# avishkarsaha/learning-adaptive-neighborhoods-for-gnns

Measured on AMD Instinct MI355X. Metric: DGG adj-build+SpMM fwd/bwd edges/sec & achieved HBM GB/s, N=100k d=128 k=32, higher is better.
Workload: dtype f32; 1 GPU; synthetic all-pairs DGG N=100000 d=128 h=64 k~32.3 K=64, u-v-dist/x/k_times_edge_prob, Gumbel(0,0.3) perturbation, + normalize + GCNConv(128,64), fwd+bwd; nodes=100000, feat=128, latent=64, parallelism=row-shard x1, rows_per_rank=100000, hipgraph=True, noise=ranked

## Files before the change

### include/dgg_hip.h

```cpp
#ifndef DGG_HIP_H
#define DGG_HIP_H
#include <stddef.h>
#include <stdint.h>

#ifdef __cplusplus
extern "C" {
#endif

#define DGG_OK 0
#define DGG_ERR_ARG 1
#define DGG_ERR_UNSUPPORTED 2
#define DGG_ERR_HIP 3

#define DGG_NOISE_NONE 0
#define DGG_NOISE_EXPLICIT 1
#define DGG_NOISE_HASH 2
#define DGG_NOISE_HASH_SYM 3
#define DGG_NOISE_RANKED 4
#define DGG_NOISE_RANKED_SYM 5

#define DGG_ACT_NONE 0
#define DGG_ACT_LEAKY 1
#define DGG_ACT_RELU 2

#define DGG_MODE_K_TIMES_EDGE_PROB 0
#define DGG_MODE_K_ONLY 1

const char *dgg_last_error(void);
int dgg_abi_version(void);

int dgg_linear_fwd(const float *x, int64_t N, int d, const float *W, const float *b, int out, int w_layout, int act,
                   float *y, void *stream);
size_t dgg_linear_bwd_ws_floats(int64_t N, int d, int out);
int dgg_linear_bwd(const float *x, int64_t N, int d, const float *W, int out, int w_layout, int act, const float *y,
                   const float *dy, float *dx, float *dW, float *db, float *ws, void *stream);
int dgg_linear_pack_weights(int nseg, const float *const *W, const float *const *b, const int *seg_out, const int *seg_layout, int d,
                            float *Wcat, float *bcat, void *stream);
int dgg_linear_fwd_multi(const float *x, int64_t N, int d, const float *Wcat, const float *bcat, int nseg, const int *seg_out,
                         const int *seg_act, float *const *y, void *stream);
size_t dgg_gemm_tn_multi_ws_floats(int64_t N, int M1_total, int M2);
int dgg_gemm_tn_multi(int nseg, const float *const *A, const int *M1, const float *const *Y, const int *act, const float *B,
                      int64_t N, int M2, float *const *C, const int *c_layout, float *const *colsum, float *ws, void *stream);
int dgg_gemm_tn_pairs(int npair, const float *const *A, const int *M1, const float *const *B, const int *M2, int64_t N, float *const *C,
                      float *const *colsum, float *ws, void *stream);
size_t dgg_gemm_tn_ws_floats(int64_t N, int M1, int M2);
int dgg_gemm_tn_acc(const float *A, const float *B, int64_t N, int M1, int M2, float *C, int c_layout, float *colsum,
                    float *ws, void *stream);

int dgg_degree_stats(const float *deg, int64_t N, float *mu_sd, void *ws, void *stream);
size_t dgg_degree_stats_ws_bytes(void);
int dgg_knet_x_fwd(const float *xk, int64_t N, int h, const float *deg, const float *mu_sd, const float *W1,
                   const float *b1, int h2, const float *Wmu, const float *bmu, int h4, const float *Wp, const float *bp,
                   float *k, float *z_save, float *u_save, float *feat_save, void *stream);
int dgg_knet_x_fwd_mfma(const float *xk, int64_t N, int h, const float *deg, const float *mu_sd, const float *W1, const float *b1,
                        const float *Wmu, const float *bmu, const float *Wp, const float *bp, float *k, float *u_save, void *stream);
size_t dgg_knet_x_bwd_ws_bytes(int64_t N, int h);
int dgg_knet_x_bwd_reg(const float *xk, int64_t N, int h, const float *deg, const float *mu_sd, const float *W1, const float *b1,
                       const float *Wmu, const float *bmu, const float *Wp, const float *u, const float *dk, float *dxk, float *gW1,
                       float *gb1, float *gWmu, float *gbmu, float *gWp, float *gbp, int out_act, void *ws, void *stream);
int dgg_knet_x_bwd_nodes(int64_t N, int h, const float *mu_sd, const float *W1, int h2, const float *Wmu, int h4,
                         const float *Wp, const float *bmu, const float *z, const float *u, const float *dk, float *dkp,
                         float *dm, float *dpre1, float *dxk, float *m_out, void *stream);
int dgg_knet_deg_fwd(const float *deg, int64_t N, const float *mu_sd, float dmean, float dstd, float eps, const float *Wd,
                     const float *bd, const float *Wmu, const float *bmu, int h4, const float *Wp, const float *bp, float *k,
                     float *u_save, void *stream);
int dgg_knet_feat(const float *xk, const float *deg, const float *mu_sd, int64_t N, int h, float *feat, void *stream);
int dgg_knet_out_fwd(const float *kp, const float *mu_sd, int64_t N, float *k, float *u, void *stream);
int dgg_knet_out_bwd(const float *u, const float *dk, const float *mu_sd, int64_t N, float *dkp, void *stream);
int dgg_knet_deg_bwd_sums(const float *deg, int64_t N, const float *mu_sd, float dmean, float dstd, float eps, const float *u,
                          const float *dk, float *S, void *stream);
int dgg_knet_input_deg_fwd(const float *deg, int64_t N, float dmean, float dstd, const float *Wd, const float *bd,
                           const float *Wmu, const float *bmu, int h4, const float *Wp, const float *bp, float *k,
                           void *stream);

int dgg_allpairs_topk(const float *xp, int64_t N, int h, int64_t row0, int64_t row1, float t, int noise_mode,
                      const float *G, int64_t ldG, uint32_t s0, uint32_t s1, int K, int32_t *idx, float *val,
                      const float *k_limit, int algo, void *workspace, size_t ws_bytes, void *stream);
int dgg_allpairs_ranked_probe(const float *xp, int64_t N, int h, int64_t row0, int64_t row1, float t, uint32_t s0, uint32_t s1,
                              const float *k_limit, int stride, int max_blocks, unsigned long long *probe, const float *lpub, void *stream);
int dgg_allpairs_topk_ranked_softk(const float *xp, int64_t N, int h, int64_t row0, int64_t row1, float t, uint32_t s0, uint32_t s1,
                                   const float *k, int mode, int32_t *idx, float *val, float *w, float *rs, void *stream);
int dgg_allpairs_topk_ranked_softk_dseed(const float *xp, int64_t N, int h, int64_t row0, int64_t row1, float t, const uint32_t *seed_dev,
                                         const float *k, int mode, int32_t *idx, float *val, float *w, float *rs, void *stream);
int dgg_allpairs_topk_ranked_softk_lp(const float *xp, int64_t N, int h, int64_t row0, int64_t row1, float t, uint32_t s0, uint32_t s1,
                                      const uint32_t *seed_dev, const float *lpub, const float *k, int mode, int32_t *idx, float *val, float *w,
                                      float *rs, void *stream);
int dgg_chunk_layout(const float *k, int64_t rows, int maxm, int64_t ccap, int32_t *cptr, int32_t *cnode, int32_t *meta, int32_t *sticky,
                     void *stream);
int dgg_allpairs_topk_ranked_wide(const float *xp, int64_t N, int h, int64_t row0, int64_t row1, float t, uint32_t s0, uint32_t s1,
                                  const uint32_t *seed_dev, const float *k, int mode, int maxm, const int32_t *cptr, int64_t ccap, int32_t *idx,
                                  float *val, float *w, float *rs, const float *lpub, void *stream);
size_t dgg_allpairs_anywide_ws_bytes(int64_t ccap, int64_t rows, int64_t N, int h);
int dgg_allpairs_topk_anywide(const float *xp, int64_t N, int h, int64_t row0, int64_t row1, float t, int noise_mode, uint32_t s0, uint32_t s1,
                              const uint32_t *seed_dev, const float *k, int mode, int maxm, int min_m, const int32_t *cptr, int64_t ccap,
                              int32_t *idx, float *val, float *w, float *rs, const float *lpub, void *workspace, size_t ws_bytes, void *stream);
size_t dgg_allpairs_rowmin_ws_bytes(int64_t rows, int64_t N, int h);
int dgg_allpairs_rowmin_bound(const float *xp, int64_t N, int h, int64_t row0, int64_t row1, float t, float *lpub, void *workspace, size_t ws_bytes,
                              void *stream);
size_t dgg_allpairs_workspace_bytes(int64_t N, int h, int noise_mode, int K);
size_t dgg_allpairs_sweep_ctl_offset_bytes(int64_t rows, int64_t N, int h);
size_t dgg_allpairs_rsym_ctl_offset_bytes(int64_t rows, int64_t N);
int dgg_literal_hard_fwd(const float *xp, int64_t N, int h, const int64_t *rowptr, const int32_t *col, float t, int noise_mode,
                         const float *G, int64_t ldG, uint32_t s0, uint32_t s1, const int32_t *idx, const float *w, int K, float threshold,
                         int32_t *hidx, float *hval, int32_t *hsrc, void *stream);
int dgg_literal_hard_bwd(const int32_t *hsrc, const float *g, int64_t N, int K, float *dw, void *stream);
int dgg_edgelist_topk(const float *xp, int64_t N, int h, const int64_t *rowptr, const int32_t *col, float t,
                      int noise_mode, const float *G, int64_t ldG, uint32_t s0, uint32_t s1, int K, int32_t *idx,
                      float *val, void *stream);
int dgg_edgelist_topk_softk(const float *xp, int64_t N, int h, const int64_t *rowptr, const int32_t *col, float t,
                            int noise_mode, const float *G, int64_t ldG, uint32_t s0, uint32_t s1, int K, const float *k,
                            int mode, int32_t *idx, float *val, float *w, float *rs, int32_t *overflow, void *stream);
int dgg_edgelist_topk_softk_rows(const float *xp, int64_t N, int h, int64_t row0, int64_t row1, const int64_t *rowptr, const int32_t *col,
                                 float t, int noise_mode, const float *G, int64_t ldG, uint32_t s0, uint32_t s1, int K, const float *k,
                                 int mode, int32_t *idx, float *val, float *w, float *rs, int32_t *overflow, void *stream);

int dgg_edge_mlp_fwd(const float *AB, const float *xp, int64_t N, int h, int hw, const int32_t *erow, const int32_t *col,
                     int64_t E, const float *deg, const float *ex_in, int ex_mode, float t_ex, const float *wdu,
                     const float *wdv, const float *wex, const float *b1, const float *w2, const float *b2, int act,
                     float *p_edge, float *ex_out, void *stream);
int dgg_edgelist_topk_p(const float *p_edge, int64_t N, const int64_t *rowptr, const int32_t *col, int noise_mode,
                        const float *G, int64_t ldG, uint32_t s0, uint32_t s1, int K, int32_t *idx, float *val, int32_t *eid,
                        void *stream);
int dgg_edgelist_topk_p_rows(const float *p_edge, int64_t N, int64_t row0, int64_t row1, const int64_t *rowptr, const int32_t *col,
                             int noise_mode, const float *G, int64_t ldG, uint32_t s0, uint32_t s1, int K, int32_t *idx, float *val,
                             int32_t *eid, void *stream);
// ... 193 lines not shown
```

### learning-adaptive-neighborhoods-for-gnns_amd/_lib.py

```python
import ctypes as C
import os

_HERE = os.path.dirname(os.path.abspath(__file__))
SO_PATH = os.environ.get("DGG_HIP_SO", os.path.join(_HERE, "libdgg_hip.so"))

_vp, _i64, _i32, _u32, _f32, _sz = C.c_void_p, C.c_int64, C.c_int, C.c_uint32, C.c_float, C.c_size_t

PROTOTYPES = {
    "dgg_linear_fwd": [_vp, _i64, _i32, _vp, _vp, _i32, _i32, _i32, _vp, _vp],
    "dgg_linear_bwd": [_vp, _i64, _i32, _vp, _i32, _i32, _i32, _vp, _vp, _vp, _vp, _vp, _vp, _vp],
    "dgg_gemm_tn_acc": [_vp, _vp, _i64, _i32, _i32, _vp, _i32, _vp, _vp, _vp],
    "dgg_gemm_tn_ws_floats": [_i64, _i32, _i32],
    "dgg_linear_pack_weights": [_i32, _vp, _vp, _vp, _vp, _i32, _vp, _vp, _vp],
    "dgg_linear_fwd_multi": [_vp, _i64, _i32, _vp, _vp, _i32, _vp, _vp, _vp, _vp],
    "dgg_gemm_tn_multi": [_i32, _vp, _vp, _vp, _vp, _vp, _i64, _i32, _vp, _vp, _vp, _vp, _vp],
    "dgg_gemm_tn_multi_ws_floats": [_i64, _i32, _i32],
    "dgg_gemm_tn_pairs": [_i32, _vp, _vp, _vp, _vp, _i64, _vp, _vp, _vp, _vp],
    "dgg_linear_bwd_ws_floats": [_i64, _i32, _i32],
    "dgg_degree_stats": [_vp, _i64, _vp, _vp, _vp],
    "dgg_degree_stats_ws_bytes": [],
    "dgg_knet_x_fwd": [_vp, _i64, _i32, _vp, _vp, _vp, _vp, _i32, _vp, _vp, _i32, _vp, _vp, _vp, _vp, _vp, _vp, _vp],
    "dgg_knet_x_fwd_mfma": [_vp, _i64, _i32] + [_vp] * 10 + [_vp],
    "dgg_knet_x_bwd_reg": [_vp, _i64, _i32] + [_vp] * 16 + [_i32, _vp, _vp],
    "dgg_knet_x_bwd_ws_bytes": [_i64, _i32],
    "dgg_knet_x_bwd_nodes": [_i64, _i32, _vp, _vp, _i32, _vp, _i32, _vp, _vp, _vp, _vp, _vp, _vp, _vp, _vp, _vp, _vp, _vp],
    "dgg_knet_input_deg_fwd": [_vp, _i64, _f32, _f32, _vp, _vp, _vp, _vp, _i32, _vp, _vp, _vp, _vp],
    "dgg_knet_feat": [_vp, _vp, _vp, _i64, _i32, _vp, _vp],
    "dgg_knet_out_fwd": [_vp, _vp, _i64, _vp, _vp, _vp],
    "dgg_knet_out_bwd": [_vp, _vp, _vp, _i64, _vp, _vp],
    "dgg_knet_deg_fwd": [_vp, _i64, _vp, _f32, _f32, _f32, _vp, _vp, _vp, _vp, _i32, _vp, _vp, _vp, _vp, _vp],
    "dgg_knet_deg_bwd_sums": [_vp, _i64, _vp, _f32, _f32, _f32, _vp, _vp, _vp, _vp],
    "dgg_allpairs_topk": [_vp, _i64, _i32, _i64, _i64, _f32, _i32, _vp, _i64, _u32, _u32, _i32, _vp, _vp, _vp, _i32, _vp, _sz, _vp],
    "dgg_allpairs_workspace_bytes": [_i64, _i32, _i32, _i32],
    "dgg_allpairs_sweep_ctl_offset_bytes": [_i64, _i64, _i32],
    "dgg_allpairs_rsym_ctl_offset_bytes": [_i64, _i64],
    "dgg_allpairs_ranked_probe": [_vp, _i64, _i32, _i64, _i64, _f32, _u32, _u32, _vp, _i32, _i32, _vp, _vp, _vp],
    "dgg_allpairs_topk_ranked_softk_lp": [_vp, _i64, _i32, _i64, _i64, _f32, _u32, _u32, _vp, _vp, _vp, _i32, _vp, _vp, _vp, _vp, _vp],
    "dgg_allpairs_topk_ranked_softk": [_vp, _i64, _i32, _i64, _i64, _f32, _u32, _u32, _vp, _i32, _vp, _vp, _vp, _vp, _vp],
    "dgg_literal_hard_fwd": [_vp, _i64, _i32, _vp, _vp, _f32, _i32, _vp, _i64, _u32, _u32, _vp, _vp, _i32, _f32, _vp, _vp, _vp, _vp],
    "dgg_literal_hard_bwd": [_vp, _vp, _i64, _i32, _vp, _vp],
    "dgg_allpairs_topk_ranked_softk_dseed": [_vp, _i64, _i32, _i64, _i64, _f32, _vp, _vp, _i32, _vp, _vp, _vp, _vp, _vp],
    "dgg_chunk_layout": [_vp, _i64, _i32, _i64, _vp, _vp, _vp, _vp, _vp],
    "dgg_allpairs_anywide_ws_bytes": [_i64, _i64, _i64, _i32],
    "dgg_allpairs_rowmin_ws_bytes": [_i64, _i64, _i32],
    "dgg_allpairs_rowmin_bound": [_vp, _i64, _i32, _i64, _i64, _f32, _vp, _vp, _sz, _vp],
    "dgg_allpairs_topk_anywide": [_vp, _i64, _i32, _i64, _i64, _f32, _i32, _u32, _u32, _vp, _vp, _i32, _i32, _i32, _vp, _i64, _vp, _vp, _vp, _vp, _vp,
                                  _vp, _sz, _vp],
    "dgg_allpairs_topk_ranked_wide": [_vp, _i64, _i32, _i64, _i64, _f32, _u32, _u32, _vp, _vp, _i32, _i32, _vp, _i64, _vp, _vp, _vp, _vp, _vp, _vp],
    "dgg_partp_build_chunked": [_vp, _vp, _vp, _vp, _i64, _vp, _i64, _vp, _vp, _vp, _i32, _vp],
    "dgg_ell_spmm_act_fwd_chunked": [_vp, _vp, _vp, _i64, _vp, _i32, _i32, _vp, _vp],
    "dgg_ell_conv_bwd_partp_chunked": [_vp, _vp, _i64, _i32, _vp, _i64, _vp, _vp, _vp, _vp, _vp, _vp, _vp],
    "dgg_softk_edge_bwd_partp_chunked": [_vp, _i64, _vp, _i64, _i32, _vp, _vp, _vp, _vp, _vp, _vp, _vp, _vp, _i64, _f32, _i32, _i32, _i32, _vp,
                                         _i64, _vp, _vp, _vp, _i32, _i32, _vp],
    "dgg_partp_gather_rec": [_vp, _i64, _i64, _vp, _vp, _vp],
    "dgg_edgelist_topk": [_vp, _i64, _i32, _vp, _vp, _f32, _i32, _vp, _i64, _u32, _u32, _i32, _vp, _vp, _vp],
    "dgg_edgelist_topk_softk": [_vp, _i64, _i32, _vp, _vp, _f32, _i32, _vp, _i64, _u32, _u32, _i32, _vp, _i32, _vp, _vp, _vp, _vp, _vp, _vp],
    "dgg_edgelist_topk_softk_rows": [_vp, _i64, _i32, _i64, _i64, _vp, _vp, _f32, _i32, _vp, _i64, _u32, _u32, _i32, _vp, _i32, _vp, _vp, _vp, _vp, _vp, _vp],
    "dgg_edge_mlp_fwd": [_vp, _vp, _i64, _i32, _i32, _vp, _vp, _i64, _vp, _vp, _i32, _f32, _vp, _vp, _vp, _vp, _vp, _vp, _i32, _vp, _vp, _vp],
    "dgg_edgelist_topk_p": [_vp, _i64, _vp, _vp, _i32, _vp, _i64, _u32, _u32, _i32, _vp, _vp, _vp, _vp],
    "dgg_edgelist_topk_p_rows": [_vp, _i64, _i64, _i64, _vp, _vp, _i32, _vp, _i64, _u32, _u32, _i32, _vp, _vp, _vp, _vp],
    "dgg_edge_mlp_bwd": [_vp, _i64, _i32, _vp, _vp, _vp, _vp, _vp, _i32, _vp, _vp, _vp, _vp, _vp, _vp, _vp, _vp, _i32, _i32, _vp, _vp, _vp, _vp],
    "dgg_edge_mlp_bwd_rows": [_vp, _i64, _i32, _i64, _i64, _vp, _vp, _vp, _vp, _vp, _i32, _vp, _vp, _vp, _vp, _vp, _vp, _vp, _vp, _i32, _i32, _vp, _vp, _vp, _vp],
    "dgg_edge_mlp_bwd_partp": [_vp, _i64, _i32, _vp, _vp, _vp, _vp, _vp, _i32, _vp, _vp, _vp, _vp, _vp, _vp, _vp, _vp, _i32, _i32, _vp, _i64, _vp, _i64, _vp, _vp, _vp, _vp],
    "dgg_edge_mlp_bwd_partp_rows": [_vp, _i64, _i32, _i64, _i64, _vp, _vp, _vp, _vp, _vp, _i32, _vp, _vp, _vp, _vp, _vp, _vp, _vp, _vp, _i32, _i32, _vp, _vp, _i64, _vp, _vp, _vp, _vp],
    "dgg_csr_softk_fwd": [_vp, _vp, _vp, _i64, _vp, _i32, _vp, _i64, _u32, _u32, _i32, _vp, _vp, _vp, _vp],
    "dgg_csr_softk_bwd": [_vp, _vp, _vp, _i64, _vp, _vp, _i32, _i32, _vp, _vp, _vp, _vp],
    "dgg_csr_softk_fwd_rows": [_vp, _vp, _vp, _i64, _i64, _i64, _vp, _i32, _u32, _u32, _i32, _vp, _vp, _vp, _vp],
    "dgg_csr_rank_ramp_fwd": [_vp, _vp, _vp, _i64, _vp, _vp, _vp, _vp, _vp, _vp, _vp],
    "dgg_csr_rank_ramp_bwd": [_vp, _vp, _i64, _vp, _vp, _vp, _vp, _vp, _vp, _vp, _vp, _vp],
    "dgg_csr_noisy_sigmoid_fwd": [_vp, _vp, _i64, _vp, _vp],
    "dgg_csr_noisy_sigmoid_bwd": [_vp, _vp, _i64, _vp, _vp],
    "dgg_csr_rank_cut_fwd": [_vp, _vp, _vp, _i64, _i32, _vp, _vp, _vp],
    "dgg_csr_rank_cut_bwd": [_vp, _vp, _i64, _i32, _vp, _vp],
    "dgg_dense_rows_fwd": [_vp, _i32, _i64, _i32, _vp, _f32, _i32, _vp, _i32, _f32, _f32, _i32, _vp, _vp, _vp, _vp],
    "dgg_dense_rows_bwd": [_vp, _i32, _i64, _i32, _vp, _f32, _i32, _vp, _f32, _f32, _vp, _vp, _vp, _vp, _vp, _vp, _vp],
    "dgg_dense_pairs_dx": [_vp, _i32, _i64, _i32, _vp, _vp, _vp],
    "dgg_feat_softmax_fwd": [_vp, _i64, _i32, _vp, _vp],
    "dgg_feat_softmax_bwd": [_vp, _vp, _i64, _i32, _vp, _vp],
    "dgg_csr_uvdist_fwd": [_vp, _vp, _vp, _i64, _i32, _f32, _vp, _vp],
    "dgg_csr_uvdist_bwd": [_vp, _vp, _vp, _i64, _i32, _f32, _vp, _vp, _vp, _vp],
    "dgg_csr_uvdist_fwd_rows": [_vp, _vp, _vp, _i64, _i64, _i64, _i32, _f32, _vp, _vp],
    "dgg_csr_uvdist_bwd_rows": [_vp, _vp, _vp, _i64, _i64, _i64, _i32, _f32, _vp, _vp, _vp, _vp],
    "dgg_csr_perturb_fwd": [_vp, _vp, _vp, _i64, _i64, _i32, _vp, _i64, _u32, _u32, _vp, _vp],
    "dgg_csr_perturb_bwd": [_vp, _vp, _vp, _i64, _vp, _vp],
    "dgg_csr_row_sum": [_vp, _vp, _i64, _vp, _vp],
    "dgg_csr_normalize_fwd": [_vp, _vp, _vp, _vp, _i64, _vp, _vp],
    "dgg_csr_norm_bwd": [_vp, _vp, _vp, _vp, _vp, _i64, _vp, _vp, _vp],
    "dgg_csr_normalize_fwd_rows": [_vp, _vp, _vp, _vp, _i64, _i64, _i64, _vp, _vp],
    "dgg_csr_norm_bwd_acc_rows": [_vp, _vp, _vp, _vp, _vp, _i64, _i64, _i64, _vp, _vp],
    "dgg_csr_norm_bwd_apply_rows": [_vp, _vp, _vp, _vp, _vp, _i64, _i64, _i64, _vp, _vp],
    "dgg_csr_spmm_fwd": [_vp, _vp, _vp, _vp, _i64, _i32, _vp, _vp],
    "dgg_csr_bg_softmax_fwd": [_vp, _vp, _i64, _vp, _vp, _vp],
    "dgg_csr_bg_softmax_bwd": [_vp, _vp, _vp, _i64, _vp, _vp, _vp, _vp],
    "dgg_masked_dense_sum": [_vp, _i64, _i32, _f32, _u32, _u32, _i32, _vp, _vp],
    "dgg_pair_keep": [_vp, _vp, _i64, _f32, _u32, _u32, _vp, _vp],
    "dgg_csr_spmm_bwd": [_vp, _vp, _vp, _vp, _vp, _i64, _i32, _vp, _vp, _vp],
    "dgg_select_scores": [_vp, _i64, _i64, _i32, _vp, _vp, _vp],
    "dgg_softk_fwd": [_vp, _vp, _vp, _i64, _i32, _i32, _vp, _vp, _vp],
# ... 89 lines not shown
```

### learning-adaptive-neighborhoods-for-gnns_amd/csrc/dgg_linear.hip

```cpp
#include "dgg_common.h"
#include "dgg_api_internal.h"

#include <cstdlib>

typedef float f32x16 __attribute__((ext_vector_type(16)));

namespace {

constexpr int LIN_BK(int nacc) { return 32; }

__device__ __forceinline__ float act_apply(float v, int act) {
    if (act == 1) return v > 0.0f ? v : __fmul_rn(0.01f, v);
    if (act == 2) return v > 0.0f ? v : 0.0f;
    return v;
}

struct LinSegs {
    float *y[8];
    int ld[8];
    int act[8];
};

template <int NACC, int WAVES, bool MULTI = false>
__global__ __launch_bounds__(64 * WAVES, NACC <= 2 ? 4 : 2) void linear_fwd_mfma(const float *__restrict__ x, int64_t N, int d,
                                                       const float *__restrict__ W, const float *__restrict__ b,
                                                       int out, int w_layout, int act, float *__restrict__ y, LinSegs segs) {
    constexpr int BN = 32 * NACC, BM = 32 * WAVES, NT = 64 * WAVES;
    constexpr int BK = LIN_BK(NACC), LDP = BK + 1, F4R = BK / 4;
    __shared__ float xs[BM * LDP];
    __shared__ float ws[BN * LDP];
    const int tid = threadIdx.x, lane = tid & 63, wave = dgg::wave_id();
    const int64_t m0 = (int64_t)blockIdx.x * BM;
    const int n0 = blockIdx.y * BN;
    f32x16 acc[NACC];
#pragma unroll
    for (int a = 0; a < NACC; a++)
#pragma unroll
        for (int r = 0; r < 16; r++) acc[a][r] = 0.0f;
    const int li = lane & 31, hh = lane >> 5;
    const bool vec4 = (d % 4 == 0) && ((reinterpret_cast<uintptr_t>(x) & 15) == 0);
    constexpr int XQ = BM * BK / 4 / NT;
    constexpr int WQ = BN * BK / NT;
    float4 xr[XQ];
    float wr[WQ];
    unsigned xm[XQ];
    auto load_block = [&](int k0) {
        if (vec4) {
#pragma unroll
            for (int q = 0; q < XQ; q++) {
                const int e = tid + q * NT, r = e / F4R, c4 = (e % F4R) * 4;
                const int64_t gi = m0 + r;
                const bool ok = gi < N && k0 + c4 < d;
                const int64_t gic = gi < N ? gi : N - 1;
                const int kc = k0 + c4 < d ? k0 + c4 : d - 4;
                xr[q] = *reinterpret_cast<const float4 *>(x + gic * d + kc);
                xm[q] = ok ? 15u : 0u;
            }
        } else {
#pragma unroll
            for (int q = 0; q < XQ; q++) {
                const int e = tid + q * NT, r = e / F4R, c4 = (e % F4R) * 4;
                const int64_t gi = m0 + r;
                const int64_t gic = gi < N ? gi : N - 1;
                float t[4];
                unsigned bits = 0;
#pragma unroll
                for (int u = 0; u < 4; u++) {
                    const int kk = k0 + c4 + u;
                    t[u] = x[gic * d + (kk < d ? kk : d - 1)];
                    bits |= (gi < N && kk < d) ? (1u << u) : 0u;
                }
                xr[q] = make_float4(t[0], t[1], t[2], t[3]);
                xm[q] = bits;
            }
        }
#pragma unroll
        for (int q = 0; q < WQ; q++) {
            const int e = tid + q * NT;
            const int j = w_layout == 0 ? e / BK : e % BN, c = w_layout == 0 ? e % BK : e / BN;
            const int gj = n0 + j, gk = k0 + c;
            const int gjc = gj < out ? gj : out - 1, gkc = gk < d ? gk : d - 1;
            wr[q] = W[w_layout == 0 ? (int64_t)gjc * d + gkc : (int64_t)gkc * out + gjc];
        }
    };
    float bj[NACC];
#pragma unroll
    for (int a = 0; a < NACC; a++) {
        const int gj = n0 + a * 32 + li;
        bj[a] = b ? b[gj < out ? gj : out - 1] : 0.0f;
    }
    load_block(0);
    for (int k0 = 0; k0 < d; k0 += BK) {
        __syncthreads();
#pragma unroll
        for (int q = 0; q < XQ; q++) {
            const int e = tid + q * NT, r = e / F4R, c4 = (e % F4R) * 4;
            float *dst = xs + r * LDP + c4;
            dst[0] = (xm[q] & 1u) ? xr[q].x : 0.0f; dst[1] = (xm[q] & 2u) ? xr[q].y : 0.0f;
            dst[2] = (xm[q] & 4u) ? xr[q].z : 0.0f; dst[3] = (xm[q] & 8u) ? xr[q].w : 0.0f;
        }
#pragma unroll
        for (int q = 0; q < WQ; q++) {
            const int e = tid + q * NT;
            const int j = w_layout == 0 ? e / BK : e % BN, c = w_layout == 0 ? e % BK : e / BN;
            ws[j * LDP + c] = (n0 + j < out && k0 + c < d) ? wr[q] : 0.0f;
        }
        __syncthreads();
        if (k0 + BK < d) load_block(k0 + BK);
        const float *xa = xs + (wave * 32 + li) * LDP + hh;
#pragma unroll
        for (int s = 0; s < BK / 2; s++) {
            float av = xa[2 * s];
#pragma unroll
            for (int a = 0; a < NACC; a++) {
                float bv = ws[(a * 32 + li) * LDP + 2 * s + hh];
                acc[a] = __builtin_amdgcn_mfma_f32_32x32x2f32(av, bv, acc[a], 0, 0, 0);
            }
        }
    }
    const bool hasb = b != nullptr;
    auto finish_act = [&](float v, float bias, int actv) {
        const float vb = __fadd_rn(v, bias);
        v = hasb ? vb : v;
        const float lk = v > 0.0f ? v : __fmul_rn(0.01f, v), rl = v > 0.0f ? v : 0.0f;
        return actv == 1 ? lk : (actv == 2 ? rl : v);
    };
    auto finish = [&](float v, float bias) { return finish_act(v, bias, act); };
    if constexpr (MULTI) {
        const bool full = m0 + BM <= N;
#pragma unroll
        for (int a = 0; a < NACC; a++) {
            const int cb = n0 / 32 + a;
            float *yb = segs.y[cb] + (m0 + wave * 32 + 4 * hh) * (int64_t)segs.ld[cb] + li;
            const int av = segs.act[cb];
#pragma unroll
            for (int r = 0; r < 16; r++) {
                const int row = (r & 3) + 8 * (r >> 2);
                if (full || m0 + wave * 32 + 4 * hh + row < N) yb[(int64_t)row * segs.ld[cb]] = finish_act(acc[a][r], bj[a], av);
            }
        }
        return;
    }
    if (m0 + BM <= N && n0 + BN <= out) {
        float *yb = y + (m0 + wave * 32 + 4 * hh) * out + n0 + li;
#pragma unroll
        for (int a = 0; a < NACC; a++)
#pragma unroll
            for (int r = 0; r < 16; r++) yb[(int64_t)((r & 3) + 8 * (r >> 2)) * out + a * 32] = finish(acc[a][r], bj[a]);
        return;
    }
#pragma unroll
    for (int a = 0; a < NACC; a++) {
        const int gj = n0 + a * 32 + li;
#pragma unroll
        for (int r = 0; r < 16; r++) {
            const int row = (r & 3) + 8 * (r >> 2) + 4 * hh;
            const int64_t gi = m0 + wave * 32 + row;
            const float v = finish(acc[a][r], bj[a]);
            if (gi < N && gj < out) y[gi * out + gj] = v;
        }
    }
}

template <int D, int NACC>
__global__ __launch_bounds__(256, 1) void linear_fwd_reg(const float *__restrict__ x, int64_t N, const float *__restrict__ W,
                                                         const float *__restrict__ b, LinSegs segs, int64_t nrb) {
    constexpr int S = D / 2, XR = D / 2;
    __shared__ float wsf[S * NACC * 64];
    const int tid = threadIdx.x, lane = tid & 63, wave = dgg::wave_id(), li = lane & 31, hh = lane >> 5;
    const int64_t nw = (int64_t)gridDim.x * 4, slot = (int64_t)blockIdx.x * 4 + wave;
    const int64_t nrbf = N / 32;
    const int64_t nmain = nrbf - nrbf % nw, nfull = nmain / nw;
    const int64_t R = nrb - nmain, nunits = nfull + (slot < R * NACC ? (R * NACC - slot + nw - 1) / nw : 0);
    auto unit_rb = [&](int64_t t) {
        if (t < nfull) return slot + t * nw;
        const int64_t u = slot + (t - nfull) * nw;
        return nmain + u % (R > 0 ? R : 1);
    };
    float xc[XR], xn[XR];
    auto load_rows = [&](int64_t rb, float(&dst)[XR]) {
        int64_t row = rb * 32 + li;
        row = row < N ? row : N - 1;
        const float4 *p = reinterpret_cast<const float4 *>(x + row * D + hh * (D / 2));
#pragma unroll
        for (int q = 0; q < XR / 4; q++) {
            const float4 v = p[q];
            dst[4 * q] = v.x; dst[4 * q + 1] = v.y; dst[4 * q + 2] = v.z; dst[4 * q + 3] = v.w;
        }
    };
    if (nunits > 0) load_rows(unit_rb(0), xc);
#pragma unroll
    for (int it = 0; it < NACC * 32 * (D / 4) / 256; it++) {
        const int e = tid + it * 256;
        const int j = e % (NACC * 32), q = e / (NACC * 32);
        const float4 v = *reinterpret_cast<const float4 *>(W + (int64_t)j * D + 4 * q);
        float *dst = wsf + ((2 * q) * NACC + (j >> 5)) * 64 + (j & 31);
        dst[0] = v.x; dst[32] = v.y; dst[NACC * 64] = v.z; dst[NACC * 64 + 32] = v.w;
    }
    const bool hasb = b != nullptr;
    float bj[NACC];
    int actv[NACC];
#pragma unroll
    for (int a = 0; a < NACC; a++) {
        bj[a] = hasb ? b[a * 32 + li] : 0.0f;
        actv[a] = segs.act[a];
    }
    __syncthreads();
    auto swap_rows = [&]() {
#pragma unroll
        for (int t = 0; t < XR / 2; t++) {
            const auto r = __builtin_amdgcn_permlane32_swap(__float_as_uint(xc[2 * t]), __float_as_uint(xc[2 * t + 1]), false, false);
            xc[2 * t] = __uint_as_float(r[0]);
            xc[2 * t + 1] = __uint_as_float(r[1]);
        }
    };
    auto act4 = [&](float4 v, int av) {
        if (av == 1) {
            v.x = fmaxf(v.x, __fmul_rn(0.01f, v.x)); v.y = fmaxf(v.y, __fmul_rn(0.01f, v.y));
            v.z = fmaxf(v.z, __fmul_rn(0.01f, v.z)); v.w = fmaxf(v.w, __fmul_rn(0.01f, v.w));
        } else if (av == 2) {
            v.x = fmaxf(v.x, 0.0f); v.y = fmaxf(v.y, 0.0f); v.z = fmaxf(v.z, 0.0f); v.w = fmaxf(v.w, 0.0f);
        }
        return v;
    };
    auto store_block = [&](const f32x16 &acc, int a, int64_t rb) {
        const int64_t n = rb * 32 + li;
        if (n >= N) return;
        const int av = actv[a];
        float *yb = segs.y[a] + n * (int64_t)segs.ld[a] + 4 * hh;
#pragma unroll
        for (int q = 0; q < 4; q++)
            *reinterpret_cast<float4 *>(yb + 8 * q) = act4(make_float4(acc[4 * q], acc[4 * q + 1], acc[4 * q + 2], acc[4 * q + 3]), av);
    };
    const float one_or_zero = hh == 0 ? 1.0f : 0.0f;
    auto main_block = [&](int64_t rb) {
        f32x16 acc[NACC];
#pragma unroll
        for (int a = 0; a < NACC; a++)
#pragma unroll
            for (int r = 0; r < 16; r++) acc[a][r] = 0.0f;
        constexpr int PD = NACC >= 4 ? 1 : (NACC >= 2 ? 2 : 4), RING = PD + 1;
        float bw[RING][NACC];
#pragma unroll
        for (int s = 0; s < PD; s++)
#pragma unroll
            for (int a = 0; a < NACC; a++) bw[s][a] = wsf[(s * NACC + a) * 64 + lane];
#pragma unroll
        for (int s = 0; s < S; s++) {
            if (s + PD < S) {
#pragma unroll
                for (int a = 0; a < NACC; a++) bw[(s + PD) % RING][a] = wsf[((s + PD) * NACC + a) * 64 + lane];
            }
            __builtin_amdgcn_sched_barrier(0);
            const float av = s < S / 2 ? xc[2 * s] : xc[2 * (s - S / 2) + 1];
#pragma unroll
            for (int a = 0; a < NACC; a++) acc[a] = __builtin_amdgcn_mfma_f32_32x32x2f32(bw[s % RING][a], av, acc[a], 0, 0, 0);
            __builtin_amdgcn_sched_barrier(0);
        }
        if (hasb) {
#pragma unroll
            for (int a = 0; a < NACC; a++) acc[a] = __builtin_amdgcn_mfma_f32_32x32x2f32(bj[a] * one_or_zero, one_or_zero, acc[a], 0, 0, 0);
        }
#pragma unroll
        for (int a = 0; a < NACC; a++) store_block(acc[a], a, rb);
    };
    int64_t t = 0;
    for (; t < nfull; t++) {
        load_rows(unit_rb(t + 1 < nunits ? t + 1 : t), xn);
        asm volatile("" ::: "memory");
        swap_rows();
        main_block(unit_rb(t));
#pragma unroll
        for (int q = 0; q < XR; q++) xc[q] = xn[q];
    }
    for (; t < nunits; t++) {
        const int64_t rb = unit_rb(t);
        load_rows(unit_rb(t + 1 < nunits ? t + 1 : t), xn);
        asm volatile("" ::: "memory");
        swap_rows();
        const int a = (int)((slot + (t - nfull) * nw) / R);
        f32x16 acc;
#pragma unroll
        for (int r = 0; r < 16; r++) acc[r] = 0.0f;
        const float *wa = wsf + a * 64 + lane;
#pragma unroll
        for (int s = 0; s < S; s++) {
            const float av = s < S / 2 ? xc[2 * s] : xc[2 * (s - S / 2) + 1];
            acc = __builtin_amdgcn_mfma_f32_32x32x2f32(wa[s * NACC * 64], av, acc, 0, 0, 0);
        }
        if (hasb) acc = __builtin_amdgcn_mfma_f32_32x32x2f32(b[a * 32 + li] * one_or_zero, one_or_zero, acc, 0, 0, 0);
        store_block(acc, a, rb);
#pragma unroll
        for (int q = 0; q < XR; q++) xc[q] = xn[q];
    }
}

__global__ void act_bwd_kernel(const float *__restrict__ y, const float *__restrict__ dy, int64_t n, int act,
                               float *__restrict__ dp) {
    int64_t i = (int64_t)blockIdx.x * blockDim.x + threadIdx.x;
    int64_t stride = (int64_t)gridDim.x * blockDim.x;
    for (; i < n; i += stride) {
        float g = dy[i], v = y[i];
        if (act == 1) g = v > 0.0f ? g : 0.01f * g;
        else if (act == 2) g = v > 0.0f ? g : 0.0f;
        dp[i] = g;
    }
}

constexpr int GT_GRID = 256, GT_PF = 8;
template <int MB, int NB, int PFK, bool ACT>
__global__ __launch_bounds__(256) void gemm_tn_persist(const float *__restrict__ A, const float *__restrict__ B, int64_t N,
                                                       int M1, int M2, int M1p, int M2p, float *__restrict__ slab,
                                                       float *__restrict__ cs_slab, const float *__restrict__ Yact, int act) {
    extern __shared__ float red[];
    const int lane = threadIdx.x & 63, wave = dgg::wave_id(), li = lane & 31, hh = lane >> 5;
    const int o0 = blockIdx.y * 32 * MB, c0 = blockIdx.z * 32 * NB;
    int64_t acol[MB], bcol[NB];
#pragma unroll
    for (int m = 0; m < MB; m++) acol[m] = o0 + m * 32 + li < M1 ? o0 + m * 32 + li : M1 - 1;
#pragma unroll
    for (int a = 0; a < NB; a++) bcol[a] = c0 + a * 32 + li < M2 ? c0 + a * 32 + li : M2 - 1;
    f32x16 acc[MB][NB];
#pragma unroll
    for (int m = 0; m < MB; m++)
#pragma unroll
        for (int a = 0; a < NB; a++)
#pragma unroll
            for (int r = 0; r < 16; r++) acc[m][a][r] = 0.0f;
    float csum[MB];
#pragma unroll
    for (int m = 0; m < MB; m++) csum[m] = 0.0f;
    constexpr int PF = PFK;
    const int64_t step = (int64_t)gridDim.x * 4 * 2 * PF;
    float av[2][PF][MB], bv[2][PF][NB], rmask[2][PF], yv[2][PF][MB];
    auto load = [&](int buf, int64_t base) {
#pragma unroll
        for (int u = 0; u < PF; u++) {
            const int64_t n = base + 2 * u + hh;
            const int64_t nc = n < N ? n : N - 1;
            rmask[buf][u] = n < N ? 1.0f : 0.0f;
#pragma unroll
            for (int m = 0; m < MB; m++) {
                av[buf][u][m] = A[nc * M1 + acol[m]];
                if (ACT) yv[buf][u][m] = Yact[nc * M1 + acol[m]];
            }
#pragma unroll
            for (int a = 0; a < NB; a++) bv[buf][u][a] = B[nc * M2 + bcol[a]];
        }
    };
    auto mma = [&](int buf) {
#pragma unroll
        for (int u = 0; u < PF; u++) {
#pragma unroll
            for (int m = 0; m < MB; m++) {
                float am = rmask[buf][u];
                if (ACT && act == 1) am = yv[buf][u][m] > 0.0f ? am : 0.01f * am;
                else if (ACT && act == 2) am = yv[buf][u][m] > 0.0f ? am : 0.0f;
                av[buf][u][m] *= am;
                csum[m] += av[buf][u][m];
#pragma unroll
                for (int a = 0; a < NB; a++)
                    acc[m][a] = __builtin_amdgcn_mfma_f32_32x32x2f32(av[buf][u][m], bv[buf][u][a], acc[m][a], 0, 0, 0);
            }
        }
    };
    int64_t base = ((int64_t)blockIdx.x * 4 + wave) * 2 * PF;
    if (base < N) load(0, base);
    while (base < N) {
        if (base + step < N) load(1, base + step);
        mma(0);
        base += step;
        if (base >= N) break;
        if (base + step < N) load(0, base + step);
// ... 263 lines not shown
                acc[m][a] = __builtin_amdgcn_mfma_f32_32x32x16_bf16(al[m], bh[a], acc[m][a], 0, 0, 0);
                acc[m][a] = __builtin_amdgcn_mfma_f32_32x32x16_bf16(ah[m], bl[a], acc[m][a], 0, 0, 0);
                acc[m][a] = __builtin_amdgcn_mfma_f32_32x32x16_bf16(ah[m], bh[a], acc[m][a], 0, 0, 0);
            }
    }
}

template <int PF, bool B3 = false, bool HASACT = true>
__global__ __launch_bounds__(256, 2) void gemm_tn_wide(TnSegs segs, const float *__restrict__ B, int64_t N, int G, int M2, int M2p, int ntile,
                                                       float *__restrict__ slab, float *__restrict__ cs_slab) {
    extern __shared__ float red[];
    const int lane = threadIdx.x & 63, wave = dgg::wave_id(), li = lane & 31, hh = lane >> 5;
    const int npair = segs.nyb / 2, nblk = npair * ntile;
    const int bid = blockIdx.x, tt = bid / (8 * nblk), rem = bid % (8 * nblk);
    const int yb = 2 * ((rem / 8) % npair), tile = (rem / 8) / npair;
    const int g = tt * 8 + (rem % 8);
    if (g >= G) return;
    const int col0 = tile * 128 + 4 * li, bcol = col0 + 4 <= M2 ? col0 : M2 - 4;
    const float *__restrict__ A = segs.A[yb];
    const float *__restrict__ Yact = segs.Y[yb];
    const int M1 = segs.ld[yb], act = Yact ? segs.act[yb] : 0, acol = segs.o0[yb] + 2 * li;
    f32x16 acc[2][4];
#pragma unroll
    for (int m = 0; m < 2; m++)
#pragma unroll
        for (int a = 0; a < 4; a++)
#pragma unroll
            for (int r = 0; r < 16; r++) acc[m][a][r] = 0.0f;
    float csum[2] = {0.0f, 0.0f};
    if constexpr (B3) {
        const int64_t base = ((int64_t)g * 4 + wave) * 16, stride = (int64_t)G * 4 * 16;
        if (HASACT && act != 0) tn_wide_stream_b3<true>(A, Yact, act, B, N, M1, acol, M2, bcol, hh, base, stride, acc, csum);
        else tn_wide_stream_b3<false>(A, Yact, act, B, N, M1, acol, M2, bcol, hh, base, stride, acc, csum);
    } else {
        const int64_t base = ((int64_t)g * 4 + wave) * 2 * PF, stride = (int64_t)G * 4 * 2 * PF;
        if (act != 0) tn_wide_stream<PF, true>(A, Yact, act, B, N, M1, acol, M2, bcol, hh, base, stride, acc, csum);
        else tn_wide_stream<PF, false>(A, Yact, act, B, N, M1, acol, M2, bcol, hh, base, stride, acc, csum);
    }
    float *cred = red + 8 * 16 * 64;
    for (int w = 1; w < 4; w++) {
        if (wave == w) {
#pragma unroll
            for (int q = 0; q < 8; q++)
#pragma unroll
                for (int r = 0; r < 16; r++) red[(q * 16 + r) * 64 + lane] = acc[q >> 2][q & 3][r];
            cred[lane] = csum[0];
            cred[64 + lane] = csum[1];
        }
        __syncthreads();
        if (wave == 0) {
#pragma unroll
            for (int q = 0; q < 8; q++)
#pragma unroll
                for (int r = 0; r < 16; r++) acc[q >> 2][q & 3][r] += red[(q * 16 + r) * 64 + lane];
            csum[0] += cred[lane];
            csum[1] += cred[64 + lane];
        }
        __syncthreads();
    }
    if (wave != 0) return;
    const int M1tp = segs.nyb * 32;
    float *sl = slab + ((int64_t)g * M1tp + yb * 32) * M2p + col0;
    if (col0 < M2p) {
#pragma unroll
        for (int m = 0; m < 2; m++)
#pragma unroll
            for (int r = 0; r < 16; r++) {
                const int go = (r & 3) + 8 * (r >> 2) + 4 * hh;
                *reinterpret_cast<float4 *>(sl + (int64_t)(2 * go + m) * M2p) = make_float4(acc[m][0][r], acc[m][1][r], acc[m][2][r], acc[m][3][r]);
            }
    }
    if (tile != 0) return;
#pragma unroll
    for (int m = 0; m < 2; m++) {
        const float t = csum[m] + __uint_as_float(dgg::xor_shfl<32>(__float_as_uint(csum[m]), lane));
        if (hh == 0) cs_slab[(int64_t)g * M1tp + yb * 32 + 2 * li + m] = t;
    }
}

struct RedSegs {
    float *C[8];
    float *colsum[8];
    int M1[8], M2[8], M1p[8], rowbase[8], c_layout[8];
};
__global__ __launch_bounds__(1024) void gemm_tn_reduce_multi(const float *__restrict__ slab, const float *__restrict__ cs_slab, int nchunks,
                                                             int M2p, int64_t chunk_stride, int64_t cs_stride, RedSegs rs) {
    __shared__ float part[16][64];
    const int sgi = blockIdx.z;
    const int M1 = rs.M1[sgi], M2 = rs.M2[sgi], M1p = rs.M1p[sgi];
    const int lane = threadIdx.x & 63, pw = threadIdx.x >> 6;
    const int e = blockIdx.x * 64 + lane;
    if (blockIdx.x * 64 >= M1p * M2p) return;
    auto total = [&](const float *base, int64_t stride, bool ok) {
        float acc[8];
#pragma unroll
        for (int j = 0; j < 8; j++) acc[j] = 0.0f;
        for (int k0 = pw; k0 < nchunks; k0 += 128) {
#pragma unroll
            for (int j = 0; j < 8; j++) {
                const int k = k0 + 16 * j;
                acc[j] += (ok && k < nchunks) ? base[(int64_t)k * stride] : 0.0f;
            }
        }
        part[pw][lane] = ((acc[0] + acc[1]) + (acc[2] + acc[3])) + ((acc[4] + acc[5]) + (acc[6] + acc[7]));
        __syncthreads();
        float v = 0.0f;
#pragma unroll
        for (int j = 0; j < 16; j++) v += part[j][lane];
        __syncthreads();
        return v;
    };
    const int o = e / M2p, c = e % M2p;
    const bool ok = e < M1p * M2p && o < M1 && c < M2;
    const float v = total(slab + (int64_t)rs.rowbase[sgi] * M2p + e, chunk_stride, ok);
    if (ok && pw == 0) {
        float *dst = rs.c_layout[sgi] == 0 ? rs.C[sgi] + (int64_t)o * M2 + c : rs.C[sgi] + (int64_t)c * M1 + o;
        *dst += v;
    }
    if (rs.colsum[sgi] && blockIdx.x * 64 < M1) {
        const bool okc = e < M1;
        const float cv = total(cs_slab + rs.rowbase[sgi] + e, cs_stride, okc);
        if (okc && pw == 0) rs.colsum[sgi][e] += cv;
    }
}

constexpr int GT_SPLIT = 32;
__global__ __launch_bounds__(256) void gemm_tn_reduce(const float *__restrict__ slab, const float *__restrict__ cs_slab,
                                                      int nchunks, int M1, int M2, int M1p, int M2p,
                                                      float *__restrict__ Cout, int c_layout, float *__restrict__ colsum,
                                                      int64_t chunk_stride, int64_t cs_stride) {
    const int e = blockIdx.x * 256 + threadIdx.x;
    const int per = (nchunks + (int)gridDim.y - 1) / (int)gridDim.y;
    const int k0 = blockIdx.y * per, k1 = k0 + per < nchunks ? k0 + per : nchunks;
    if (k0 >= k1) return;
    if (e < M1p * M2p) {
        const int o = e / M2p, c = e % M2p;
        if (o < M1 && c < M2) {
            float s = 0.0f;
            for (int k = k0; k < k1; k++) s += slab[(int64_t)k * chunk_stride + e];
            float *dst = c_layout == 0 ? Cout + (int64_t)o * M2 + c : Cout + (int64_t)c * M1 + o;
            atomicAdd(dst, s);
        }
    }
    if (colsum && cs_slab && e < M1) {
        float s = 0.0f;
        for (int k = k0; k < k1; k++) s += cs_slab[(int64_t)k * cs_stride + e];
        atomicAdd(colsum + e, s);
    }
}

template <int NACC>
void launch_linear_fwd_n(const float *x, int64_t N, int d, const float *W, const float *b, int out, int w_layout, int act, float *y,
                         hipStream_t st) {
    const unsigned gy = (unsigned)((out + 32 * NACC - 1) / (32 * NACC));
    hipLaunchKernelGGL((linear_fwd_mfma<NACC, 4>), dim3((unsigned)((N + 127) / 128), gy), dim3(256), 0, st, x, N, d, W, b, out, w_layout, act, y, LinSegs{});
}

int launch_linear_fwd(const float *x, int64_t N, int d, const float *W, const float *b, int out, int w_layout, int act,
                      float *y, hipStream_t st) {
    static const int nacc_env = [] { const char *e = getenv("DGG_LIN_NACC1"); return e ? atoi(e) : 0; }();
    const int64_t wg4 = ((N + 127) / 128) * ((out + 127) / 128);
    if (out <= 32) launch_linear_fwd_n<1>(x, N, d, W, b, out, w_layout, act, y, st);
    else if (out <= 64 || nacc_env == 2 || (nacc_env == 0 && wg4 < 256)) launch_linear_fwd_n<2>(x, N, d, W, b, out, w_layout, act, y, st);
    else launch_linear_fwd_n<4>(x, N, d, W, b, out, w_layout, act, y, st);
    return dgg_check_launch("linear_fwd");
}

template <int NACC>
void launch_linear_fwd_multi_n(const float *x, int64_t N, int d, const float *W, const float *b, int out, const LinSegs &segs, hipStream_t st) {
    hipLaunchKernelGGL((linear_fwd_mfma<NACC, 4, true>), dim3((unsigned)((N + 127) / 128), (unsigned)(out / (32 * NACC))), dim3(256), 0, st, x, N,
                       d, W, b, out, 0, 0, nullptr, segs);
}

inline void gemm_tn_shape(int M1p, int M2p, int &mb, int &nb) {
    mb = M1p / 32 >= 2 ? 2 : 1;
    nb = M2p / 32 >= 3 ? 4 : M2p / 32;
}
inline int gemm_tn_grid(int64_t N, int M1p, int M2p) {
    int mb, nb;
    gemm_tn_shape(M1p, M2p, mb, nb);
    const int64_t blocks = (int64_t)((M1p / 32 + mb - 1) / mb) * ((M2p / 32 + nb - 1) / nb);
    int64_t g = (4 * GT_GRID + blocks - 1) / blocks;
    if (g > GT_GRID) g = GT_GRID;
    const int64_t need = (N + 4 * 2 * GT_PF - 1) / (4 * 2 * GT_PF);
    if (g > need) g = need;
    int64_t cap = N * (int64_t)(M1p + M2p) / (4 * (int64_t)M1p * M2p);
    if (cap < 8) cap = 8;
    if (g > cap) g = cap;
    if (g > need) g = need;
    return (int)(g < 1 ? 1 : g);
}
size_t gemm_tn_ws_floats(int64_t N, int M1, int M2) {
    const size_t M1p = (size_t)(M1 + 31) / 32 * 32, M2p = (size_t)(M2 + 31) / 32 * 32;
    const size_t g = (size_t)gemm_tn_grid(N, (int)M1p, (int)M2p);
    return g * M1p * M2p + g * M1p;
}

template <int MB, int NB>
void launch_gemm_tn_persist(const float *A, const float *B, int64_t N, int M1, int M2, int M1p, int M2p, float *slab,
                            float *cs_slab, int g, const float *Yact, int act, hipStream_t st) {
    const unsigned gy = (unsigned)((M1p / 32 + MB - 1) / MB), gz = (unsigned)((M2p / 32 + NB - 1) / NB);
    const size_t lds = (size_t)(MB * NB * 16 * 64 + MB * 64) * sizeof(float);
    if (Yact)
        hipLaunchKernelGGL((gemm_tn_persist<MB, NB, GT_PF / 2, true>), dim3(g, gy, gz), dim3(256), lds, st, A, B, N, M1, M2, M1p, M2p, slab,
                           cs_slab, Yact, act);
    else
        hipLaunchKernelGGL((gemm_tn_persist<MB, NB, GT_PF, false>), dim3(g, gy, gz), dim3(256), lds, st, A, B, N, M1, M2, M1p, M2p, slab,
                           cs_slab, Yact, act);
}

int launch_gemm_tn(const float *A, const float *B, int64_t N, int M1, int M2, float *C, int c_layout, float *colsum,
                   float *ws, hipStream_t st, const float *Yact = nullptr, int act = 0) {
    if (!ws) return dgg_set_error(DGG_ERR_ARG, "gemm_tn: workspace is NULL (dgg_gemm_tn_ws_floats)");
    const int M1p = (M1 + 31) / 32 * 32, M2p = (M2 + 31) / 32 * 32;
    const int g = gemm_tn_grid(N, M1p, M2p);
    float *slab = ws, *cs_slab = ws + (size_t)g * M1p * M2p;
    float *csl = colsum ? cs_slab : nullptr;
    int mb, nb;
    gemm_tn_shape(M1p, M2p, mb, nb);
    if (Yact) mb = 1;
    if (mb == 2 && nb == 4) launch_gemm_tn_persist<2, 4>(A, B, N, M1, M2, M1p, M2p, slab, csl, g, Yact, act, st);
    else if (mb == 2 && nb == 2) launch_gemm_tn_persist<2, 2>(A, B, N, M1, M2, M1p, M2p, slab, csl, g, Yact, act, st);
    else if (mb == 2) launch_gemm_tn_persist<2, 1>(A, B, N, M1, M2, M1p, M2p, slab, csl, g, Yact, act, st);
    else if (nb == 4) launch_gemm_tn_persist<1, 4>(A, B, N, M1, M2, M1p, M2p, slab, csl, g, Yact, act, st);
    else if (nb == 2) launch_gemm_tn_persist<1, 2>(A, B, N, M1, M2, M1p, M2p, slab, csl, g, Yact, act, st);
    else launch_gemm_tn_persist<1, 1>(A, B, N, M1, M2, M1p, M2p, slab, csl, g, Yact, act, st);
    int split = (M1p * M2p >= 16384) ? (g + 7) / 8 : g;
    split = split < 1 ? 1 : (split > GT_SPLIT ? GT_SPLIT : split);
    hipLaunchKernelGGL(gemm_tn_reduce, dim3((unsigned)((M1p * M2p + 255) / 256), (unsigned)split), dim3(256), 0, st, slab, csl, g, M1,
                       M2, M1p, M2p, C, c_layout, colsum, (int64_t)M1p * M2p, (int64_t)M1p);
    return dgg_check_launch("gemm_tn");
}

}

extern "C" {

int dgg_linear_fwd(const float *x, int64_t N, int d, const float *W, const float *b, int out, int w_layout, int act,
                   float *y, void *stream) {
    if (N < 0 || d < 1 || out < 1) return dgg_set_error(DGG_ERR_ARG, "linear_fwd: bad shape");
    if (N == 0) return 0;
    return launch_linear_fwd(x, N, d, W, b, out, w_layout, act, y, (hipStream_t)stream);
}

struct PackSegs {
    const float *W[8];
    const float *b[8];
    int out[8], layout[8], first[8];
};
__global__ __launch_bounds__(256) void pack_weights_kernel(PackSegs sg, int nseg, int d, int total, float *__restrict__ Wcat,
                                                           float *__restrict__ bcat) {
    const int e = blockIdx.x * 256 + threadIdx.x;
    if (e >= total * (d + 1)) return;
    const int c = e / (d + 1), k = e % (d + 1);
    int s = 0;
#pragma unroll
    for (int q = 1; q < 8; q++)
        if (q < nseg && c >= sg.first[q]) s = q;
    const int lc = c - sg.first[s];
    if (k == d) { bcat[c] = sg.b[s] ? sg.b[s][lc] : 0.0f; return; }
    Wcat[(int64_t)c * d + k] = sg.layout[s] == 0 ? sg.W[s][(int64_t)lc * d + k] : sg.W[s][(int64_t)k * sg.out[s] + lc];
}

extern "C" int dgg_linear_pack_weights(int nseg, const float *const *W, const float *const *b, const int *seg_out, const int *seg_layout,
                                       int d, float *Wcat, float *bcat, void *stream) {
    if (nseg < 1 || nseg > 8 || d < 1) return dgg_set_error(DGG_ERR_ARG, "linear_pack_weights: 1..8 layers");
    PackSegs sg{};
    int total = 0;
    for (int s = 0; s < nseg; s++) {
        sg.W[s] = W[s]; sg.b[s] = b ? b[s] : nullptr; sg.out[s] = seg_out[s]; sg.layout[s] = seg_layout[s]; sg.first[s] = total;
        total += seg_out[s];
    }
    hipLaunchKernelGGL(pack_weights_kernel, dim3((unsigned)((total * (d + 1) + 255) / 256)), dim3(256), 0, (hipStream_t)stream, sg, nseg, d, total,
                       Wcat, bcat);
    return dgg_check_launch("linear_pack_weights");
}

int dgg_linear_fwd_multi(const float *x, int64_t N, int d, const float *Wcat, const float *bcat, int nseg, const int *seg_out,
                         const int *seg_act, float *const *y, void *stream) {
    if (N < 0 || d < 1 || nseg < 1 || nseg > 8) return dgg_set_error(DGG_ERR_ARG, "linear_fwd_multi: bad shape");
    LinSegs segs{};
    int cb = 0;
    for (int sgi = 0; sgi < nseg; sgi++) {
        if (seg_out[sgi] < 32 || seg_out[sgi] % 32 != 0 || cb + seg_out[sgi] / 32 > 8)
            return dgg_set_error(DGG_ERR_UNSUPPORTED, "linear_fwd_multi: layer widths must be multiples of 32 with a total of at most 256");
        for (int q = 0; q < seg_out[sgi] / 32; q++, cb++) {
            segs.y[cb] = y[sgi] + q * 32;
            segs.ld[cb] = seg_out[sgi];
            segs.act[cb] = seg_act[sgi];
        }
    }
    if (cb == 7) return dgg_set_error(DGG_ERR_UNSUPPORTED, "linear_fwd_multi: 7 column blocks (224 outputs) are not tiled");
    if (N == 0) return 0;
    const int out = cb * 32;
    hipStream_t st = (hipStream_t)stream;
    static const int forced = [] { const char *e = getenv("DGG_LINEAR_REG"); return e ? atoi(e) : -1; }();
    const bool aligned = (reinterpret_cast<uintptr_t>(x) % 16 == 0) && (reinterpret_cast<uintptr_t>(Wcat) % 16 == 0);
    if (d == 128 && aligned && cb <= 6 && (forced >= 0 ? forced != 0 : N >= 32768)) {
        const int64_t nrb = (N + 31) / 32;
        const unsigned grid = (unsigned)std::min<int64_t>(256, (nrb + 3) / 4);
        switch (cb) {
#define DGG_LIN_REG(NA) case NA: hipLaunchKernelGGL((linear_fwd_reg<128, NA>), dim3(grid), dim3(256), 0, st, x, N, Wcat, bcat, segs, nrb); break
            DGG_LIN_REG(1); DGG_LIN_REG(2); DGG_LIN_REG(3); DGG_LIN_REG(4); DGG_LIN_REG(5); DGG_LIN_REG(6);
#undef DGG_LIN_REG
        }
        return dgg_check_launch("linear_fwd_multi");
    }
    static const int nacc_env = [] { const char *e = getenv("DGG_LIN_NACC"); return e ? atoi(e) : 0; }();
    int nacc_small = 0;
    if ((N + 127) / 128 < 256 && cb > 2) nacc_small = cb % 2 == 0 ? 2 : 1;
    if (cb > 1 && ((N + 127) / 128) * ((cb + 1) / 2) < 128) nacc_small = 1;
    if (nacc_env > 0 && cb % nacc_env == 0) nacc_small = nacc_env;
    if (nacc_small > 0) {
        switch (nacc_small) {
            case 1: launch_linear_fwd_multi_n<1>(x, N, d, Wcat, bcat, out, segs, st); break;
            case 2: launch_linear_fwd_multi_n<2>(x, N, d, Wcat, bcat, out, segs, st); break;
            case 3: launch_linear_fwd_multi_n<3>(x, N, d, Wcat, bcat, out, segs, st); break;
            default: launch_linear_fwd_multi_n<4>(x, N, d, Wcat, bcat, out, segs, st); break;
        }
        return dgg_check_launch("linear_fwd_multi");
    }
    switch (cb) {
        case 1: launch_linear_fwd_multi_n<1>(x, N, d, Wcat, bcat, out, segs, st); break;
        case 2: launch_linear_fwd_multi_n<2>(x, N, d, Wcat, bcat, out, segs, st); break;
        case 3: launch_linear_fwd_multi_n<3>(x, N, d, Wcat, bcat, out, segs, st); break;
        case 4: launch_linear_fwd_multi_n<4>(x, N, d, Wcat, bcat, out, segs, st); break;
        case 5: launch_linear_fwd_multi_n<5>(x, N, d, Wcat, bcat, out, segs, st); break;
        case 6: launch_linear_fwd_multi_n<6>(x, N, d, Wcat, bcat, out, segs, st); break;
        default: launch_linear_fwd_multi_n<4>(x, N, d, Wcat, bcat, out, segs, st); break;
    }
    return dgg_check_launch("linear_fwd_multi");
}

size_t dgg_linear_bwd_ws_floats(int64_t N, int d, int out) { return (size_t)N * out + gemm_tn_ws_floats(N, out, d); }
size_t dgg_gemm_tn_ws_floats(int64_t N, int M1, int M2) { return gemm_tn_ws_floats(N, M1, M2); }

int dgg_linear_bwd(const float *x, int64_t N, int d, const float *W, int out, int w_layout, int act, const float *y,
                   const float *dy, float *dx, float *dW, float *db, float *ws, void *stream) {
    hipStream_t st = (hipStream_t)stream;
    if (N == 0) return 0;
    if (!ws) return dgg_set_error(DGG_ERR_ARG, "linear_bwd: workspace is NULL (dgg_linear_bwd_ws_floats)");
    const float *dp = dy;
    if (act != 0 && !dx && dW)
        return launch_gemm_tn(dy, x, N, out, d, dW, w_layout == 0 ? 0 : 1, db, ws + (size_t)N * out, st, y, act);
    if (act != 0) {
        int64_t n = N * out;
        unsigned blocks = (unsigned)((n + 255) / 256 < 4096 ? (n + 255) / 256 : 4096);
        hipLaunchKernelGGL(act_bwd_kernel, dim3(blocks), dim3(256), 0, st, y, dy, n, act, ws);
        dp = ws;
    }
    if (dx) {
        int rc = launch_linear_fwd(dp, N, out, W, nullptr, d, w_layout == 0 ? 1 : 0, 0, dx, st);
        if (rc != 0) return rc;
    }
    if (dW) return launch_gemm_tn(dp, x, N, out, d, dW, w_layout == 0 ? 0 : 1, db, ws + (size_t)N * out, st);
    return dgg_check_launch("linear_bwd");
}

int dgg_act_bwd(const float *y, const float *dy, int64_t n, int act, float *dp, void *stream) {
    if (n == 0) return 0;
    const unsigned blocks = (unsigned)((n + 255) / 256 < 8192 ? (n + 255) / 256 : 8192);
    hipLaunchKernelGGL(act_bwd_kernel, dim3(blocks), dim3(256), 0, (hipStream_t)stream, y, dy, n, act, dp);
    return dgg_check_launch("act_bwd");
}

size_t dgg_gemm_tn_multi_ws_floats(int64_t N, int M1_total, int M2) {
    const size_t M2p = (size_t)(M2 + 31) / 32 * 32;
    return (size_t)256 * ((size_t)M1_total * M2p + (size_t)M1_total);
}
int dgg_gemm_tn_multi(int nseg, const float *const *A, const int *M1, const float *const *Y, const int *act, const float *B, int64_t N,
                      int M2, float *const *C, const int *c_layout, float *const *colsum, float *ws, void *stream) {
    if (nseg < 1 || nseg > 8 || M2 < 1) return dgg_set_error(DGG_ERR_UNSUPPORTED, "gemm_tn_multi: 1..8 operands");
    if (!ws) return dgg_set_error(DGG_ERR_ARG, "gemm_tn_multi: workspace is NULL (dgg_gemm_tn_multi_ws_floats)");
    TnSegs segs{};
    int yb = 0;
    for (int sgi = 0; sgi < nseg; sgi++) {
        if (M1[sgi] < 32 || M1[sgi] % 32 != 0 || yb + M1[sgi] / 32 > 8)
            return dgg_set_error(DGG_ERR_UNSUPPORTED, "gemm_tn_multi: operand widths must be multiples of 32 with a total of at most 256");
        for (int q = 0; q < M1[sgi] / 32; q++, yb++) {
            segs.A[yb] = A[sgi];
            segs.Y[yb] = Y ? Y[sgi] : nullptr;
            segs.ld[yb] = M1[sgi];
            segs.o0[yb] = q * 32;
            segs.act[yb] = act ? act[sgi] : 0;
        }
    }
    segs.nyb = yb;
    if (N == 0) return 0;
    hipStream_t st = (hipStream_t)stream;
    const int M2p = (M2 + 31) / 32 * 32, M1tp = yb * 32;
    constexpr int PF = 4;
    int G = 128;
    const int64_t need = (N + 4 * 2 * PF - 1) / (4 * 2 * PF);
    while (G > 8 && G / 2 >= need) G /= 2;
    bool wide = (M2 == 128 || (M2 > 128 && M2 % 4 == 0)) && (N >= 4096 || M2 > 128) && reinterpret_cast<uintptr_t>(B) % 16 == 0;
    for (int sgi = 0; sgi < nseg; sgi++)
        wide = wide && M1[sgi] % 64 == 0 && reinterpret_cast<uintptr_t>(A[sgi]) % 8 == 0 && (!Y || !Y[sgi] || reinterpret_cast<uintptr_t>(Y[sgi]) % 8 == 0);
    static const int force_wide = [] { const char *e = getenv("DGG_TN_WIDE"); return e ? atoi(e) : -1; }();
    if (force_wide == 0 && M2 <= 128) wide = false;
    if (M2 > 128 && !wide)
        return dgg_set_error(DGG_ERR_UNSUPPORTED, "gemm_tn_multi: an input wider than 128 columns needs M2 % 4 == 0, operand widths in "
                                                  "multiples of 64 and 16-byte aligned rows");
    const int ntile = (M2 + 127) / 128;
    if (wide) {
        constexpr int PFW = 6;
        const int npair = yb / 2 * ntile;
        G = 512 / npair / 8 * 8;
        G = G < 8 ? 8 : G;
        G = G > 256 ? 256 : G;
        const int64_t needw = (N + 4 * 2 * PFW - 1) / (4 * 2 * PFW);
        while (G > 8 && G - 8 >= needw) G -= 8;
    }
    float *slab = ws, *cs_slab = ws + (size_t)G * M1tp * M2p;
    const unsigned grid = (unsigned)(G * yb);
    const int nb = M2p / 32 == 3 ? 4 : M2p / 32;
    const size_t lds = (size_t)(nb * 16 * 64 + 64) * sizeof(float);
    const size_t ldsw = (size_t)(8 * 16 * 64 + 128) * sizeof(float);
    const dim3 gridw((unsigned)(G * (yb / 2) * ntile));
    static const bool tn_b3 = [] { const char *e = getenv("DGG_TN_B3"); return !(e && atoi(e) == 0); }();
    bool hasact = false;
    for (int sgi = 0; sgi < nseg; sgi++) hasact = hasact || (Y && Y[sgi] && act && act[sgi] != 0);
    if (wide && tn_b3 && !hasact) hipLaunchKernelGGL((gemm_tn_wide<6, true, false>), gridw, dim3(256), ldsw, st, segs, B, N, G, M2, M2p, ntile, slab, cs_slab);
    else if (wide && tn_b3) hipLaunchKernelGGL((gemm_tn_wide<6, true, true>), gridw, dim3(256), ldsw, st, segs, B, N, G, M2, M2p, ntile, slab, cs_slab);
    else if (wide) hipLaunchKernelGGL((gemm_tn_wide<6>), gridw, dim3(256), ldsw, st, segs, B, N, G, M2, M2p, ntile, slab, cs_slab);
    else if (nb == 4) hipLaunchKernelGGL((gemm_tn_multi<4, PF>), dim3(grid), dim3(256), lds, st, segs, B, N, M2, M2p, G, slab, cs_slab);
    else if (nb == 2) hipLaunchKernelGGL((gemm_tn_multi<2, PF>), dim3(grid), dim3(256), lds, st, segs, B, N, M2, M2p, G, slab, cs_slab);
    else hipLaunchKernelGGL((gemm_tn_multi<1, PF>), dim3(grid), dim3(256), lds, st, segs, B, N, M2, M2p, G, slab, cs_slab);
    RedSegs rsg{};
    int rb = 0, m1max = 0;
    for (int sgi = 0; sgi < nseg; sgi++) {
        rsg.C[sgi] = C[sgi]; rsg.colsum[sgi] = colsum ? colsum[sgi] : nullptr; rsg.M1[sgi] = M1[sgi]; rsg.M2[sgi] = M2; rsg.M1p[sgi] = M1[sgi];
        rsg.rowbase[sgi] = rb; rsg.c_layout[sgi] = c_layout[sgi];
        rb += M1[sgi];
        m1max = M1[sgi] > m1max ? M1[sgi] : m1max;
    }
    hipLaunchKernelGGL(gemm_tn_reduce_multi, dim3((unsigned)((m1max * M2p + 63) / 64), 1, (unsigned)nseg), dim3(1024), 0, st,
                       slab, cs_slab, G, M2p, (int64_t)M1tp * M2p, (int64_t)M1tp, rsg);
    return dgg_check_launch("gemm_tn_multi");
}

int dgg_gemm_tn_pairs(int npair, const float *const *A, const int *M1, const float *const *B, const int *M2, int64_t N, float *const *C,
                      float *const *colsum, float *ws, void *stream) {
    if (npair < 1 || npair > 8) return dgg_set_error(DGG_ERR_UNSUPPORTED, "gemm_tn_pairs: 1..8 products");
    if (!ws) return dgg_set_error(DGG_ERR_ARG, "gemm_tn_pairs: workspace is NULL");
    TnSegs segs{};
    int yb = 0, rb[8], m2max = 1;
    for (int p = 0; p < npair; p++) {
        if (M1[p] < 1 || M2[p] < 1 || M2[p] > 128) return dgg_set_error(DGG_ERR_UNSUPPORTED, "gemm_tn_pairs: M2 <= 128");
        rb[p] = yb * 32;
        for (int q = 0; q < (M1[p] + 31) / 32; q++, yb++) {
            if (yb >= 8) return dgg_set_error(DGG_ERR_UNSUPPORTED, "gemm_tn_pairs: at most 256 (padded) rows of output in total");
            segs.A[yb] = A[p]; segs.Y[yb] = nullptr; segs.ld[yb] = M1[p]; segs.o0[yb] = q * 32; segs.act[yb] = 0;
            segs.Bp[yb] = B[p]; segs.m2[yb] = M2[p];
        }
        m2max = M2[p] > m2max ? M2[p] : m2max;
    }
    segs.nyb = yb;
    if (N == 0) return 0;
    hipStream_t st = (hipStream_t)stream;
    const int M2p = 128, M1tp = yb * 32;
    constexpr int PF = 4;
    int G = 256;
    const int64_t need = (N + 4 * 2 * PF - 1) / (4 * 2 * PF);
    while (G > 8 && G / 2 >= need) G /= 2;
    float *slab = ws, *cs_slab = ws + (size_t)G * M1tp * M2p;
    const size_t lds = (size_t)(4 * 16 * 64 + 64) * sizeof(float);
    hipLaunchKernelGGL((gemm_tn_multi<4, PF>), dim3((unsigned)(G * yb)), dim3(256), lds, st, segs, A[0], N, m2max, M2p, G, slab, cs_slab);
    RedSegs rsg{};
    int m1pmax = 0;
    for (int p = 0; p < npair; p++) {
        rsg.C[p] = C[p]; rsg.colsum[p] = colsum ? colsum[p] : nullptr; rsg.M1[p] = M1[p]; rsg.M2[p] = M2[p];
        rsg.M1p[p] = (M1[p] + 31) / 32 * 32; rsg.rowbase[p] = rb[p]; rsg.c_layout[p] = 0;
        m1pmax = rsg.M1p[p] > m1pmax ? rsg.M1p[p] : m1pmax;
    }
    hipLaunchKernelGGL(gemm_tn_reduce_multi, dim3((unsigned)((m1pmax * M2p + 63) / 64), 1, (unsigned)npair), dim3(1024), 0, st,
                       slab, cs_slab, G, M2p, (int64_t)M1tp * M2p, (int64_t)M1tp, rsg);
    return dgg_check_launch("gemm_tn_pairs");
}

int dgg_gemm_tn_acc(const float *A, const float *B, int64_t N, int M1, int M2, float *C, int c_layout, float *colsum,
                    float *ws, void *stream) {
    if (N == 0) return 0;
    return launch_gemm_tn(A, B, N, M1, M2, C, c_layout, colsum, ws, (hipStream_t)stream);
}

}
```

### learning-adaptive-neighborhoods-for-gnns_amd/csrc/dgg_scatter.hip

```cpp
#include "dgg_common.h"
#include "dgg_api_internal.h"

using namespace dgg;

namespace {

constexpr int BS = 128;
constexpr int PR = 256;

struct PartHdr {
    int *bstart, *cursor;
    int2 *tmp;
    int *slot;
    int2 *recs;
    int *cstart;
};
__host__ __device__ inline size_t align256(size_t x) { return (x + 255) / 256 * 256; }
inline PartHdr part_layout(void *ws, int64_t nb, int64_t nrec) {
    char *w = reinterpret_cast<char *>(ws);
    PartHdr p;
    p.bstart = reinterpret_cast<int *>(w);
    p.cursor = reinterpret_cast<int *>(w + align256((size_t)(nb + 1) * 4));
    p.tmp = reinterpret_cast<int2 *>(w + align256((size_t)(nb + 1) * 4) + align256((size_t)nb * 4));
    p.slot = reinterpret_cast<int *>(reinterpret_cast<char *>(p.tmp) + align256((size_t)nrec * sizeof(int2)));
// ... 59 lines not shown
            if (jj[u] >= 0) {
                const int b = jj[u] / BS;
                const int slot = base[b] + atomicAdd(&hist[b], 1);
                recs[slot] = make_int2((int)(i * 64 + lane), jj[u]);
            } else if (jj[u] == -1) {
                slotmap[i * K + lane] = -1;
            }
        }
    }
}

__global__ __launch_bounds__(1024) void part_sort(const int *__restrict__ bstart, const int2 *__restrict__ tmp, int K,
                                                 int2 *__restrict__ recs, int *__restrict__ slotmap) {
    __shared__ int cnt[BS], base[BS];
    const int tid = threadIdx.x, b = blockIdx.x;
    const int e0 = bstart[b], e1 = bstart[b + 1];
    if (tid < BS) cnt[tid] = 0;
    __syncthreads();
    for (int e = e0 + tid; e < e1; e += 1024) atomicAdd(&cnt[tmp[e].y - b * BS], 1);
    __syncthreads();
    if (tid < 64) {
        const int c0 = cnt[2 * tid], c1 = cnt[2 * tid + 1];
        int incl = c0 + c1;
#pragma unroll
        for (int off = 1; off < 64; off <<= 1) {
            const int v = __shfl_up(incl, off, 64);
            if (tid >= off) incl += v;
        }
        base[2 * tid] = incl - c0 - c1;
        base[2 * tid + 1] = incl - c1;
    }
    __syncthreads();
    if (tid < BS) cnt[tid] = 0;
    __syncthreads();
    for (int e = e0 + tid; e < e1; e += 1024) {
        const int2 rec = tmp[e];
        const int jl = rec.y - b * BS;
        const int pos = e0 + base[jl] + atomicAdd(&cnt[jl], 1);
        recs[pos] = rec;
        slotmap[(int64_t)(rec.x >> 6) * K + (rec.x & 63)] = pos;
    }
}

__global__ void part_chunk_starts(const int *__restrict__ bstart, int nb, const int2 *__restrict__ recs, int nchunks, int chunk,
                                  int *__restrict__ cstart) {
    const int c = blockIdx.x * blockDim.x + threadIdx.x;
    if (c > nchunks) return;
    const int nnz = bstart[nb];
    const int64_t x = (int64_t)c * chunk;
    int e = x < nnz ? (int)x : nnz;
    if (e > 0) {
        const int lim = e + 48 < nnz ? e + 48 : nnz;
        while (e < lim && recs[e].y == recs[e - 1].y) e++;
        if (e < nnz && recs[e].y == recs[e - 1].y) e = (int)x;
    }
    cstart[c] = e;
}

__global__ __launch_bounds__(1024) void part_scan(int *__restrict__ bstart, int *__restrict__ cursor, int nb) {
    __shared__ int part[1024];
    const int tid = threadIdx.x;
    const int per = (nb + 1023) / 1024;
    const int lo = tid * per, hi = lo + per < nb ? lo + per : nb;
    int s = 0;
    for (int b = lo; b < hi; b++) s += cursor[b];
    part[tid] = s;
    __syncthreads();
    for (int off = 1; off < 1024; off <<= 1) {
        int v = tid >= off ? part[tid - off] : 0;
        __syncthreads();
        part[tid] += v;
        __syncthreads();
    }
    int run = part[tid] - s;
    for (int b = lo; b < hi; b++) {
        const int c = cursor[b];
        bstart[b] = run;
        cursor[b] = run;
        run += c;
    }
    if (tid == 1023) bstart[nb] = part[1023];
}

struct SoftkArgs {
    const float *k, *rs, *dA, *da;
    int mode, normalized;
    float *dval_out, *dk;
    const float *ahat_rows;
    float4 *rowinfo;
    const int *recpos;
    const float *dA_rec;
};
template <int H, bool FUSE, bool PAY = false>
__global__ __launch_bounds__(256) void edge_bwd_rows(const float *__restrict__ xp, int64_t rows, const int32_t *__restrict__ idx,
                                                     const float *__restrict__ val, const float *__restrict__ dval, int K,
                                                     int64_t row0, float t, int perturb, const int *__restrict__ slotmap,
                                                     float *__restrict__ coef, float *__restrict__ dxp, SoftkArgs sk) {
    constexpr int LPR = H / 4;
    constexpr int NPI = 64 / LPR;
    const int lane = threadIdx.x & 63, c4 = lane % LPR, slot = lane / LPR;
    const int64_t i = (int64_t)blockIdx.x * 4 + dgg::wave_id();
    if (i >= rows) return;
    const int64_t gi = row0 + i;
    const int32_t jl = lane < K ? idx[i * K + lane] : -1;
    const float vl = lane < K ? val[i * K + lane] : 0.0f;
    float gl;
    if (FUSE) {
        const int lc = lane < K ? lane : K - 1;
        const bool viamap = PAY && sk.recpos != nullptr;
        float dw = viamap ? 0.0f : sk.dA[i * K + lc];
        const int rpos = viamap ? sk.recpos[i * 64 + lc] : 0;
        const bool live = lane < K && jl >= 0;
        if (sk.normalized) {
            const float rsi = sk.rs[gi];
            const float ai = __fdiv_rn(1.0f, c_sqrt(rsi)), aj = __fdiv_rn(1.0f, c_sqrt(sk.rs[jl >= 0 ? jl : gi]));
            float dai = sk.da[gi];
            if (sk.ahat_rows) {
                const float ah = lane < K ? sk.ahat_rows[i * K + lane] : 0.0f;
                if (viamap) dw = sk.dA_rec[ah != 0.0f ? rpos : 0];
                if (PAY && ah == 0.0f) dw = 0.0f;
                float rp = dw * ah;
                rp = wave_sum_dpp(rp, lane);
                dai += rp * sqrtf(rsi);
            }
            const float drs = -0.5f * dai * ai / rsi;
            dw = dw * ai * aj + drs;
            if (PAY && lane == 0) sk.rowinfo[i] = make_float4(ai, drs, sk.k[i], 0.0f);
        } else if (PAY && lane == 0) {
            sk.rowinfo[i] = make_float4(1.0f, 0.0f, sk.k[i], 0.0f);
        }
        const float th = c_tanh((float)lane - sk.k[i]);
        const float f = 1.0f - 0.5f * (1.0f + th);
        const float dfdk = 0.5f * (1.0f - th * th);
        gl = (live && sk.mode == 0) ? dw * f : 0.0f;
        float skp = live ? (sk.mode == 0 ? dw * vl * dfdk : dw * dfdk) : 0.0f;
#pragma unroll
        for (int off = 32; off >= 1; off >>= 1) skp += __shfl_xor(skp, off, 64);
        if (lane == 0) sk.dk[i] = skp;
        if (sk.dval_out && lane < K) sk.dval_out[i * K + lane] = gl;
    } else {
        gl = lane < K ? dval[i * K + lane] : 0.0f;
    }
    const float4 xi = *reinterpret_cast<const float4 *>(xp + gi * H + 4 * c4);
    float4 acc = make_float4(0.0f, 0.0f, 0.0f, 0.0f);
    float mycoef = 0.0f;
    constexpr int NBT = (32 / NPI) < 1 ? 1 : 32 / NPI;
    const bool myact = lane < K && jl >= 0 && gl != 0.0f;
    for (int r0 = 0; r0 < K; r0 += NBT * NPI) {
        const bool mine = lane >= r0 && lane < r0 + NBT * NPI;
        if (__ballot(mine && myact) == 0ull) continue;
        float4 xj[NBT];
#pragma unroll
        for (int b = 0; b < NBT; b++) {
            const int r = r0 + b * NPI + slot;
            const int rr = r < 64 ? r : 63;
            const int32_t jb = __shfl(jl, rr, 64);
            const bool ab = __shfl((int)myact, rr, 64) != 0 && r < K;
            xj[b] = *reinterpret_cast<const float4 *>(xp + (ab ? (int64_t)jb : gi) * H + 4 * c4);
        }
        float myd2 = 0.0f;
#pragma unroll
        for (int b = 0; b < NBT; b++) {
            const float4 d = make_float4(xi.x - xj[b].x, xi.y - xj[b].y, xi.z - xj[b].z, xi.w - xj[b].w);
            float d2 = d.x * d.x + d.y * d.y + d.z * d.z + d.w * d.w;
            if (LPR > 16) d2 += __uint_as_float(xor_shfl<16>(__float_as_uint(d2), lane));
            if (LPR > 8) d2 += __uint_as_float(xor_shfl<8>(__float_as_uint(d2), lane));
            if (LPR > 4) d2 += __uint_as_float(xor_shfl<4>(__float_as_uint(d2), lane));
            if (LPR > 2) d2 += __uint_as_float(xor_shfl<2>(__float_as_uint(d2), lane));
            d2 += __uint_as_float(xor_shfl<1>(__float_as_uint(d2), lane));
            const float tq = __shfl(d2, (lane % NPI) * LPR, 64);
            if ((lane - r0) / NPI == b && mine) myd2 = tq;
        }
        float mydd = 0.0f;
        if (mine && myact && myd2 != 0.0f) {
            const float dist = sqrtf(myd2);
            const float p = c_exp(t * dist);
            const float dp = perturb ? gl * vl / (p + 1e-8f) : gl;
            mydd = dp * t * p / dist;
        }
        if (!PAY && mine) mycoef = mydd;
#pragma unroll
        for (int b = 0; b < NBT; b++) {
            const int r = r0 + b * NPI + slot;
            const float dd = __shfl(mydd, r < 64 ? r : 63, 64);
            const float4 d = make_float4(xi.x - xj[b].x, xi.y - xj[b].y, xi.z - xj[b].z, xi.w - xj[b].w);
            acc.x += dd * d.x; acc.y += dd * d.y; acc.z += dd * d.z; acc.w += dd * d.w;
        }
    }
#pragma unroll
    for (int off = LPR; off < 64; off <<= 1) {
        acc.x += __shfl_xor(acc.x, off, 64); acc.y += __shfl_xor(acc.y, off, 64);
        acc.z += __shfl_xor(acc.z, off, 64); acc.w += __shfl_xor(acc.w, off, 64);
    }
    if (slot == 0) *reinterpret_cast<float4 *>(dxp + gi * H + 4 * c4) = acc;
    if (!PAY && lane < K) {
        const int sl = slotmap[i * K + lane];
        if (sl >= 0) coef[sl] = mycoef;
    }
}

template <int H>
__global__ __launch_bounds__(256) void edge_bwd_rows_chunked(const float *__restrict__ xp, int64_t rows, const int32_t *__restrict__ cptr,
                                                             const int32_t *__restrict__ idx, const float *__restrict__ val, int64_t row0,
                                                             float t, int perturb, float *__restrict__ dxp, SoftkArgs sk) {
    constexpr int LPR = H / 4;
    constexpr int NPI = 64 / LPR;
    constexpr int NBT = (32 / NPI) < 1 ? 1 : 32 / NPI;
    const int lane = threadIdx.x & 63, c4 = lane % LPR, slot = lane / LPR;
    const int64_t i = (int64_t)blockIdx.x * 4 + dgg::wave_id();
    if (i >= rows) return;
    const int64_t gi = row0 + i;
    const int cb = __builtin_amdgcn_readfirstlane(cptr[i]), ce = __builtin_amdgcn_readfirstlane(cptr[i + 1]);
    const float ki = sk.k[i];
    float ai = 1.0f, drs = 0.0f;
    if (sk.normalized) {
        const float rsi = sk.rs[gi];
        ai = __fdiv_rn(1.0f, c_sqrt(rsi));
        float dai = sk.da[gi];
        if (sk.ahat_rows) {
            float rp = 0.0f;
            for (int c = cb; c < ce; c++) {
                const float ah = sk.ahat_rows[(int64_t)c * 64 + lane];
                float dw = sk.dA[(int64_t)c * 64 + lane];
                if (ah == 0.0f) dw = 0.0f;
                rp += dw * ah;
            }
            rp = wave_sum_dpp(rp, lane);
            dai += rp * sqrtf(rsi);
        }
        drs = -0.5f * dai * ai / rsi;
    }
    const float4 xi = *reinterpret_cast<const float4 *>(xp + gi * H + 4 * c4);
    float4 acc = make_float4(0.0f, 0.0f, 0.0f, 0.0f);
    float skp = 0.0f;
    for (int c = cb; c < ce; c++) {
        const int64_t e = (int64_t)c * 64 + lane;
        const int32_t jl = idx[e];
        const float vl = val[e];
        const bool live = jl >= 0;
        float dw = sk.dA[e];
        const float kshift = ki - (float)(64 * (c - cb));
        if (sk.normalized) {
            const float aj = __fdiv_rn(1.0f, c_sqrt(sk.rs[live ? jl : gi]));
            if (sk.ahat_rows && sk.ahat_rows[e] == 0.0f) dw = 0.0f;
            dw = dw * ai * aj + drs;
        }
        if (lane == 0) sk.rowinfo[c] = make_float4(ai, drs, kshift, 0.0f);
        const float th = c_tanh((float)lane - kshift);
        const float f = 1.0f - 0.5f * (1.0f + th);
        const float dfdk = 0.5f * (1.0f - th * th);
        const float gl = (live && sk.mode == 0) ? dw * f : 0.0f;
        skp += live ? (sk.mode == 0 ? dw * vl * dfdk : dw * dfdk) : 0.0f;
        const bool myact = live && gl != 0.0f;
        if (__ballot(myact) == 0ull) continue;
        for (int r0 = 0; r0 < 64; r0 += NBT * NPI) {
            const bool mine = lane >= r0 && lane < r0 + NBT * NPI;
            if (__ballot(mine && myact) == 0ull) continue;
            float4 xj[NBT];
#pragma unroll
            for (int b = 0; b < NBT; b++) {
                const int r = r0 + b * NPI + slot;
                const int rr = r < 64 ? r : 63;
                const int32_t jb = __shfl(jl, rr, 64);
                const bool ab = __shfl((int)myact, rr, 64) != 0 && r < 64;
                xj[b] = *reinterpret_cast<const float4 *>(xp + (ab ? (int64_t)jb : gi) * H + 4 * c4);
            }
            float myd2 = 0.0f;
#pragma unroll
            for (int b = 0; b < NBT; b++) {
                const float4 d = make_float4(xi.x - xj[b].x, xi.y - xj[b].y, xi.z - xj[b].z, xi.w - xj[b].w);
                float d2 = d.x * d.x + d.y * d.y + d.z * d.z + d.w * d.w;
                if (LPR > 16) d2 += __uint_as_float(xor_shfl<16>(__float_as_uint(d2), lane));
                if (LPR > 8) d2 += __uint_as_float(xor_shfl<8>(__float_as_uint(d2), lane));
                if (LPR > 4) d2 += __uint_as_float(xor_shfl<4>(__float_as_uint(d2), lane));
                if (LPR > 2) d2 += __uint_as_float(xor_shfl<2>(__float_as_uint(d2), lane));
                d2 += __uint_as_float(xor_shfl<1>(__float_as_uint(d2), lane));
                const float tq = __shfl(d2, (lane % NPI) * LPR, 64);
                if ((lane - r0) / NPI == b && mine) myd2 = tq;
            }
            float mydd = 0.0f;
            if (mine && myact && myd2 != 0.0f) {
// ... 261 lines not shown
        float ext[NBT];
        if constexpr (EXT) {
#pragma unroll
            for (int b = 0; b < NBT; b++) ext[b] = src[b] >= 0 ? dA_ext[(int64_t)(src[b] >> 6) * K + (src[b] & 63)] : 0.0f;
        }
        float mydot = 0.0f;
#pragma unroll
        for (int b = 0; b < NBT; b++) {
            float dot = g[b].x * hj.x;
            dot = fmaf(g[b].y, hj.y, dot); dot = fmaf(g[b].z, hj.z, dot); dot = fmaf(g[b].w, hj.w, dot);
            if (LPR > 16) dot += __uint_as_float(xor_shfl<16>(__float_as_uint(dot), lane));
            if (LPR > 8) dot += __uint_as_float(xor_shfl<8>(__float_as_uint(dot), lane));
            if (LPR > 4) dot += __uint_as_float(xor_shfl<4>(__float_as_uint(dot), lane));
            dot += __uint_as_float(xor_shfl<2>(__float_as_uint(dot), lane));
            dot += __uint_as_float(xor_shfl<1>(__float_as_uint(dot), lane));
            if constexpr (EXT) dot += ext[b];
            if (dA && src[b] >= 0 && c4 == 0)
                __hip_atomic_store(&dA[(int64_t)(src[b] >> 6) * K + (src[b] & 63)], dot, __ATOMIC_RELAXED, __HIP_MEMORY_SCOPE_AGENT);
            if constexpr (ROWSHARE) {
                if (c4 == b) mydot = dot;
            } else {
                const float tq = __shfl(dot, (lane % NPI) * LPR, 64);
                if (lane / NPI == b) mydot = tq;
            }
            acc.x = fmaf(cf[b], g[b].x, acc.x); acc.y = fmaf(cf[b], g[b].y, acc.y);
            acc.z = fmaf(cf[b], g[b].z, acc.z); acc.w = fmaf(cf[b], g[b].w, acc.w);
            sda = fmaf(dot, cf[b], sda);
        }
        if (have) dA_rec[e0 + myq] = mydot;
    }
#pragma unroll
    for (int off = LPR; off < 64; off <<= 1) {
        acc.x += __shfl_xor(acc.x, off, 64); acc.y += __shfl_xor(acc.y, off, 64);
        acc.z += __shfl_xor(acc.z, off, 64); acc.w += __shfl_xor(acc.w, off, 64);
        sda += __shfl_xor(sda, off, 64);
    }
}

template <int F, bool EXT = false>
__global__ __launch_bounds__(256) void conv_bwd_node(const float *__restrict__ G, const float *__restrict__ Hm, int K, int64_t ncols,
                                                     const int *__restrict__ nodeptr, const int4 *__restrict__ recs,
                                                     const float *__restrict__ rs, float *__restrict__ dA, float *__restrict__ dA_rec,
                                                     float *__restrict__ dH, float *__restrict__ da, const float *__restrict__ dA_ext = nullptr,
                                                     unsigned nmain = 0, int wide = 0) {
    constexpr int LPR = F / 4, PER = 4 * (64 / LPR);
    __shared__ float4 part[4][LPR];
    __shared__ float parts[4];
    const int lane = threadIdx.x & 63, c4 = lane % LPR, slot = lane / LPR, wave = dgg::wave_id();
    const bool longmode = nmain != 0 && blockIdx.x >= nmain;
    const int64_t j = longmode ? (int64_t)(blockIdx.x - nmain) : (int64_t)blockIdx.x * 4 + wave;
    if (j >= ncols) return;
    const int p0 = nodeptr[j], p1 = nodeptr[j + 1];
    const bool islong = nmain != 0 && p1 - p0 > NODE_LONG;
    if (islong != longmode) return;
    const float4 hj = *reinterpret_cast<const float4 *>(Hm + j * F + 4 * c4);
    const float rsj = rs[j];
    const float aj = __fdiv_rn(1.0f, c_sqrt(rsj));
    float4 acc = make_float4(0.0f, 0.0f, 0.0f, 0.0f);
    float sda = 0.0f;
    if (!longmode) {
        conv_bwd_walk<F, EXT>(G, K, p0, p1, p1, recs, hj, aj, dA, dA_rec, dA_ext, lane, acc, sda, wide);
    } else {
        const int chunk = ((p1 - p0 + 4 * PER - 1) / (4 * PER)) * PER;
        const int pb = p0 + wave * chunk, pe = pb + chunk < p1 ? pb + chunk : p1;
        conv_bwd_walk<F, EXT>(G, K, pb < p1 ? pb : p1, pe, p1, recs, hj, aj, dA, dA_rec, dA_ext, lane, acc, sda, wide);
        if (slot == 0) part[wave][c4] = acc;
        if (lane == 0) parts[wave] = sda;
        __syncthreads();
        if (wave != 0) return;
        acc = part[0][c4];
        sda = parts[0];
#pragma unroll
        for (int w_ = 1; w_ < 4; w_++) {
            const float4 v = part[w_][c4];
            acc.x += v.x; acc.y += v.y; acc.z += v.z; acc.w += v.w;
            sda += parts[w_];
        }
    }
    if (slot == 0) *reinterpret_cast<float4 *>(dH + j * F + 4 * c4) = acc;
    if (da && lane == 0) da[j] = sda * sqrtf(rsj);
}

template <int H>
__device__ __forceinline__ void edge_bwd_walk(const float *__restrict__ xp, int64_t j, int pb, int pe, int p1, const int4 *__restrict__ recs,
                                              const float *__restrict__ dA_rec, const float4 *__restrict__ rowinfo, const float4 xj, const float aj,
                                              int64_t row0, float t, int perturb, int lane, float4 &acc, const int wide = 0) {
    constexpr int LPR = H / 4, NPI = 64 / LPR, NBT = (32 / NPI) < 1 ? 1 : 32 / NPI, PER = NBT * NPI;
    const int c4 = lane % LPR, slot = lane / LPR;
    for (int e0 = pb; e0 < pe; e0 += PER) {
        const bool have = lane < PER && e0 + lane < pe;
        const int ec = have ? e0 + lane : p1 - 1;
        int4 myrec = recs[ec];
        if (!have) myrec.y = -1;
        float mydval;
        {
            const float4 info = rowinfo[myrec.x >> 6];
            const float dw = dA_rec[ec] * info.x * aj + info.y;
            const float th = c_tanh((float)(myrec.x & 63) - info.z);
            mydval = have ? dw * (1.0f - 0.5f * (1.0f + th)) : 0.0f;
        }
        float4 xi[NBT];
#pragma unroll
        for (int b = 0; b < NBT; b++) {
            const int q = b * NPI + slot;
            const int src = __shfl(myrec.x, q, 64);
            const int dst = __shfl(myrec.y, q, 64);
            xi[b] = *reinterpret_cast<const float4 *>(xp + (dst >= 0 ? row0 + (wide ? dst : (src >> 6)) : j) * H + 4 * c4);
        }
        float myd2 = 0.0f;
#pragma unroll
        for (int b = 0; b < NBT; b++) {
            const float4 d = make_float4(xi[b].x - xj.x, xi[b].y - xj.y, xi[b].z - xj.z, xi[b].w - xj.w);
            float d2 = d.x * d.x + d.y * d.y + d.z * d.z + d.w * d.w;
            if (LPR > 16) d2 += __uint_as_float(xor_shfl<16>(__float_as_uint(d2), lane));
            if (LPR > 8) d2 += __uint_as_float(xor_shfl<8>(__float_as_uint(d2), lane));
            if (LPR > 4) d2 += __uint_as_float(xor_shfl<4>(__float_as_uint(d2), lane));
            d2 += __uint_as_float(xor_shfl<2>(__float_as_uint(d2), lane));
            d2 += __uint_as_float(xor_shfl<1>(__float_as_uint(d2), lane));
            const float tq = __shfl(d2, (lane % NPI) * LPR, 64);
            if (lane / NPI == b) myd2 = tq;
        }
        float mydd = 0.0f;
        if (mydval != 0.0f && myd2 != 0.0f) {
            const float dist = sqrtf(myd2);
            const float p = c_exp(t * dist);
            const float dp = perturb ? mydval * __int_as_float(myrec.w) / (p + 1e-8f) : mydval;
            mydd = dp * t * p / dist;
        }
#pragma unroll
        for (int b = 0; b < NBT; b++) {
            const float dd = __shfl(mydd, b * NPI + slot, 64);
            const float4 d = make_float4(xi[b].x - xj.x, xi[b].y - xj.y, xi[b].z - xj.z, xi[b].w - xj.w);
            acc.x -= dd * d.x; acc.y -= dd * d.y; acc.z -= dd * d.z; acc.w -= dd * d.w;
        }
    }
#pragma unroll
    for (int off = LPR; off < 64; off <<= 1) {
        acc.x += __shfl_xor(acc.x, off, 64); acc.y += __shfl_xor(acc.y, off, 64);
        acc.z += __shfl_xor(acc.z, off, 64); acc.w += __shfl_xor(acc.w, off, 64);
    }
}

template <int H>
__global__ __launch_bounds__(256) void edge_bwd_node(const float *__restrict__ xp, int64_t ncols, const int *__restrict__ nodeptr,
                                                     const int4 *__restrict__ recs, const float *__restrict__ dA_rec,
                                                     const float4 *__restrict__ rowinfo, const float *__restrict__ rs, int normalized,
                                                     int64_t row0, int64_t rows, float t, int perturb, float *__restrict__ dxp, int out_act,
                                                     unsigned nmain = 0, int wide = 0) {
    constexpr int LPR = H / 4, NPI = 64 / LPR, NBT = (32 / NPI) < 1 ? 1 : 32 / NPI, PER = NBT * NPI;
    __shared__ float4 part[4][LPR];
    const int lane = threadIdx.x & 63, c4 = lane % LPR, slot = lane / LPR, wave = dgg::wave_id();
    const bool longmode = nmain != 0 && blockIdx.x >= nmain;
    const int64_t j = longmode ? (int64_t)(blockIdx.x - nmain) : (int64_t)blockIdx.x * 4 + wave;
    if (j >= ncols) return;
    const int p0 = nodeptr[j], p1 = nodeptr[j + 1];
    const bool islong = nmain != 0 && p1 - p0 > NODE_LONG;
    if (islong != longmode) return;
    const float4 xj = *reinterpret_cast<const float4 *>(xp + j * H + 4 * c4);
    const float aj = normalized ? __fdiv_rn(1.0f, c_sqrt(rs[j])) : 1.0f;
    float4 acc = make_float4(0.0f, 0.0f, 0.0f, 0.0f);
    if (!longmode) {
        edge_bwd_walk<H>(xp, j, p0, p1, p1, recs, dA_rec, rowinfo, xj, aj, row0, t, perturb, lane, acc, wide);
    } else {
        const int chunk = ((p1 - p0 + 4 * PER - 1) / (4 * PER)) * PER;
        const int pb = p0 + wave * chunk, pe = pb + chunk < p1 ? pb + chunk : p1;
        edge_bwd_walk<H>(xp, j, pb < p1 ? pb : p1, pe, p1, recs, dA_rec, rowinfo, xj, aj, row0, t, perturb, lane, acc, wide);
        if (slot == 0) part[wave][c4] = acc;
        __syncthreads();
        if (wave != 0) return;
        acc = part[0][c4];
#pragma unroll
        for (int w_ = 1; w_ < 4; w_++) {
            const float4 v = part[w_][c4];
            acc.x += v.x; acc.y += v.y; acc.z += v.z; acc.w += v.w;
        }
    }
    if (slot == 0) {
        float4 *o = reinterpret_cast<float4 *>(dxp + j * H + 4 * c4);
        if (j >= row0 && j < row0 + rows) {
            float4 v = *o;
            acc.x += v.x; acc.y += v.y; acc.z += v.z; acc.w += v.w;
        }
        if (out_act == 1) {
            acc.x *= xj.x > 0.0f ? 1.0f : 0.01f; acc.y *= xj.y > 0.0f ? 1.0f : 0.01f;
            acc.z *= xj.z > 0.0f ? 1.0f : 0.01f; acc.w *= xj.w > 0.0f ? 1.0f : 0.01f;
        }
        *o = acc;
    }
}

template <int F, int NBT>
__global__ __launch_bounds__(256) void conv_bwd_nodeg(const float *__restrict__ G, const float *__restrict__ Hm, int K, int64_t ncols,
                                                      const int *__restrict__ nodeptr, const int4 *__restrict__ recs,
                                                      const float *__restrict__ rs, float *__restrict__ dA, float *__restrict__ dA_rec,
                                                      float *__restrict__ dH, float *__restrict__ da) {
    constexpr int LPR = F / 4, NPW = 64 / LPR;
    const int lane = threadIdx.x & 63, c4 = lane % LPR;
    const int64_t jraw = ((int64_t)blockIdx.x * 4 + dgg::wave_id()) * NPW + lane / LPR;
    const bool live = jraw < ncols;
    const int64_t j = live ? jraw : ncols - 1;
    const int p0 = nodeptr[j], p1 = live ? nodeptr[j + 1] : p0;
    const float4 hj = *reinterpret_cast<const float4 *>(Hm + j * F + 4 * c4);
    const float rsj = rs[j];
    const float aj = __fdiv_rn(1.0f, c_sqrt(rsj));
    float4 acc = make_float4(0.0f, 0.0f, 0.0f, 0.0f);
    float sda = 0.0f;
    int trips = (p1 - p0 + NBT - 1) / NBT;
#pragma unroll
    for (int off = LPR; off < 64; off <<= 1) trips = max(trips, __shfl_xor(trips, off, 64));
    for (int it = 0, e0 = p0; it < trips; it++, e0 += NBT) {
        int src[NBT];
        float cf[NBT];
        float4 g[NBT];
#pragma unroll
        for (int b = 0; b < NBT; b++) {
            const bool have = e0 + b < p1;
            const int4 r = recs[have ? e0 + b : (p1 > p0 ? p1 - 1 : 0)];
            src[b] = have ? r.x : -1;
            cf[b] = have ? __fmul_rn(__int_as_float(r.z), aj) : 0.0f;
            g[b] = *reinterpret_cast<const float4 *>(G + (int64_t)(have ? (r.x >> 6) : 0) * F + 4 * c4);
        }
#pragma unroll
        for (int b = 0; b < NBT; b++) {
            float dot = g[b].x * hj.x;
            dot = fmaf(g[b].y, hj.y, dot); dot = fmaf(g[b].z, hj.z, dot); dot = fmaf(g[b].w, hj.w, dot);
            if (LPR > 16) dot += __uint_as_float(xor_shfl<16>(__float_as_uint(dot), lane));
            if (LPR > 8) dot += __uint_as_float(xor_shfl<8>(__float_as_uint(dot), lane));
            if (LPR > 4) dot += __uint_as_float(xor_shfl<4>(__float_as_uint(dot), lane));
            dot += __uint_as_float(xor_shfl<2>(__float_as_uint(dot), lane));
            dot += __uint_as_float(xor_shfl<1>(__float_as_uint(dot), lane));
            if (src[b] >= 0 && c4 == (b % LPR)) {
                if (dA) __hip_atomic_store(&dA[(int64_t)(src[b] >> 6) * K + (src[b] & 63)], dot, __ATOMIC_RELAXED, __HIP_MEMORY_SCOPE_AGENT);
                dA_rec[e0 + b] = dot;
            }
            acc.x = fmaf(cf[b], g[b].x, acc.x); acc.y = fmaf(cf[b], g[b].y, acc.y);
            acc.z = fmaf(cf[b], g[b].z, acc.z); acc.w = fmaf(cf[b], g[b].w, acc.w);
            sda = fmaf(dot, cf[b], sda);
        }
    }
    if (!live) return;
    *reinterpret_cast<float4 *>(dH + j * F + 4 * c4) = acc;
    if (da && c4 == 0) da[j] = sda * sqrtf(rsj);
}

template <int H, int NBT>
__global__ __launch_bounds__(256) void edge_bwd_nodeg(const float *__restrict__ xp, int64_t ncols, const int *__restrict__ nodeptr,
                                                      const int4 *__restrict__ recs, const float *__restrict__ dA_rec,
                                                      const float4 *__restrict__ rowinfo, const float *__restrict__ rs, int normalized,
                                                      int64_t row0, int64_t rows, float t, int perturb, float *__restrict__ dxp, int out_act) {
// ... 74 lines not shown
    const int lane = threadIdx.x & 63;
    const int64_t i = (int64_t)blockIdx.x * 4 + dgg::wave_id();
    if (i >= rows) return;
    float rowpart = 0.0f, cf = 0.0f;
    if (lane < K) {
        const int32_t j = idx[i * K + lane];
        if (j >= 0) {
            const float g = dA[i * K + lane] * w[i * K + lane];
            if (g != 0.0f) {
                const float ai = 1.0f / sqrtf(rs[row0 + i]), aj = 1.0f / sqrtf(rs[j]);
                rowpart = g * aj;
                cf = g * ai;
            }
        }
        const int sl = slotmap[i * K + lane];
        if (sl >= 0) coef[sl] = cf;
    }
    rowpart = wave_sum_dpp(rowpart, lane);
    if (lane == 0) da[row0 + i] = rowpart;
}
__global__ __launch_bounds__(256) void norm_da_cols(int64_t ncols, const int *__restrict__ bstart, const int2 *__restrict__ recs,
                                                    const float *__restrict__ coef, float *__restrict__ da) {
    __shared__ float ssum[BS];
    const int tid = threadIdx.x, b = blockIdx.x;
    if (tid < BS) ssum[tid] = 0.0f;
    __syncthreads();
    const int e0 = bstart[b], e1 = bstart[b + 1], lane = tid & 63;
    for (int eb = e0 + (tid - lane); eb < e1; eb += 256) {
        const int e = eb + lane;
        const bool have = e < e1;
        const int dst = have ? recs[e].y : -1;
        float v = have ? coef[e] : 0.0f;
#pragma unroll
        for (int off = 1; off < 64; off <<= 1) {
            const float vo = __shfl_up(v, off, 64);
            const int dd = __shfl_up(dst, off, 64);
            if (lane >= off && dd == dst) v += vo;
        }
        const int dn = __shfl_down(dst, 1, 64);
        if (have && (lane == 63 || dn != dst) && v != 0.0f) atomicAdd(&ssum[dst - b * BS], v);
    }
    __syncthreads();
    if (tid < BS) {
        const int64_t j = (int64_t)b * BS + tid;
        if (j < ncols && ssum[tid] != 0.0f) da[j] += ssum[tid];
    }
}

inline int64_t nbuckets(int64_t ncols) { return (ncols + BS - 1) / BS; }

constexpr int PP_T = 1024;
constexpr int PP_RPT = 16;
constexpr int PP_UF = 8;
inline int pp_threads() {
    static const int t = [] { const char *e = getenv("DGG_PP_THREADS"); const int v = e ? atoi(e) : 0; return (v == 256 || v == 512 || v == 1024) ? v : 1024; }();
    return t;
}
inline int pp_width(int64_t rows, int K, int64_t ncols) {
    static const int forced = [] { const char *e = getenv("DGG_PP_WIDTH"); return e ? atoi(e) : 0; }();
    const double per_node = (double)rows * (0.7 * K) / (double)(ncols > 0 ? ncols : 1);
    int64_t wmax = (int64_t)(0.75 * PP_T * PP_RPT / (per_node > 1e-9 ? per_node : 1e-9));
    wmax = wmax < 32 ? 32 : (wmax > 4096 ? 4096 : wmax);
    int64_t w = wmax;
    for (int m = 1; m <= 16; m++) {
        const int64_t cand = (ncols + 256 * m - 1) / (256 * m);
        if (cand <= wmax) { w = cand < 32 ? 32 : cand; break; }
    }
    if (forced >= 32 && forced <= 4096) w = forced;
    while ((ncols + w - 1) / w > 4096) w *= 2;
    if ((double)ncols * (double)w >= 4.0e9) {
        int64_t p2 = 32;
        while (p2 < w) p2 *= 2;
        w = p2;
    }
    return (int)w;
}
inline uint32_t pp_recip(int width) { return (uint32_t)((((uint64_t)1 << 32) + (uint64_t)width - 1) / (uint64_t)width); }
__device__ __forceinline__ int pp_bucket(int j, uint32_t rcp) { return (int)__umulhi((uint32_t)j, rcp); }

struct PartP2 {
    int *bstart, *totals, *nodeptr, *T;
    int *recpos;
    float *ainv;
    int4 *tmp, *recs;
    int width;
    uint32_t rcp;
    int64_t nb, nwg;
};
static bool pp_builds_map(int64_t rows) {
    static const int forced = [] { const char *e = getenv("DGG_DA_MAP"); return e ? atoi(e) : -1; }();
    return forced >= 0 ? forced != 0 : rows * 64 * 4 <= (8 << 20);
}
inline size_t partp2_layout(PartP2 &p, void *ws, int64_t rows, int K, int64_t ncols) {
    p.width = pp_width(rows, K, ncols);
    p.rcp = pp_recip(p.width);
    p.nb = (ncols + p.width - 1) / p.width;
    p.nwg = (rows + pp_threads() / 4 - 1) / (pp_threads() / 4);
    char *w = reinterpret_cast<char *>(ws);
    size_t o = 0;
    p.bstart = reinterpret_cast<int *>(w + o); o += align256((size_t)(p.nb + 1) * 4);
    p.totals = reinterpret_cast<int *>(w + o); o += align256((size_t)p.nb * 4);
    p.nodeptr = reinterpret_cast<int *>(w + o); o += align256((size_t)(p.nb * p.width + 1) * 4);
    p.T = reinterpret_cast<int *>(w + o); o += align256((size_t)p.nwg * p.nb * 4);
    p.ainv = reinterpret_cast<float *>(w + o); o += align256((size_t)ncols * 4);
    p.tmp = reinterpret_cast<int4 *>(w + o); o += align256((size_t)rows * K * sizeof(int4));
    p.recs = reinterpret_cast<int4 *>(w + o); o += align256((size_t)rows * K * sizeof(int4));
    p.recpos = reinterpret_cast<int *>(w + o); o += (size_t)rows * 64 * sizeof(int);
    return o;
}

__device__ __forceinline__ void pp_load16(const int32_t *__restrict__ idx, const float *__restrict__ w, int64_t rows, int64_t r0, int lane,
                                          int4 (&ji)[4], float4 (&wv)[4]) {
#pragma unroll
    for (int u = 0; u < 4; u++) {
        const int64_t i = r0 + 4 * u + (lane >> 4);
        const int64_t e = (i < rows ? i : rows - 1) * 64 + 4 * (lane & 15);
        ji[u] = *reinterpret_cast<const int4 *>(idx + e);
        wv[u] = *reinterpret_cast<const float4 *>(w + e);
        if (i >= rows) ji[u] = make_int4(-1, -1, -1, -1);
    }
}
__device__ __forceinline__ int pp_get(const int4 &v, int c) { return c == 0 ? v.x : c == 1 ? v.y : c == 2 ? v.z : v.w; }
__device__ __forceinline__ float pp_getf(const float4 &v, int c) { return c == 0 ? v.x : c == 1 ? v.y : c == 2 ? v.z : v.w; }

template <int THREADS>
__global__ __launch_bounds__(THREADS) void pp_count(const int32_t *__restrict__ idx, const float *__restrict__ w, int64_t rows, int K, int nb,
                                                    uint32_t rcp, int *__restrict__ T, const float *__restrict__ rs_all, int64_t ncols,
                                                    float *__restrict__ ainv) {
    extern __shared__ int lds[];
    int *hist = lds;
    const int tid = threadIdx.x, lane = tid & 63, wave = dgg::wave_id();
    for (int b = tid; b < nb; b += THREADS) hist[b] = 0;
    if (rs_all) {
        const int64_t per = (ncols + gridDim.x - 1) / gridDim.x;
        const int64_t j1 = ((int64_t)blockIdx.x + 1) * per < ncols ? ((int64_t)blockIdx.x + 1) * per : ncols;
        for (int64_t j = (int64_t)blockIdx.x * per + tid; j < j1; j += THREADS) ainv[j] = __fdiv_rn(1.0f, c_sqrt(rs_all[j]));
    }
    __syncthreads();
    const int64_t r0 = (int64_t)blockIdx.x * (THREADS / 4) + wave * 16;
    if (K == 64) {
        int4 ji[4];
        float4 wv[4];
        pp_load16(idx, w, rows, r0, lane, ji, wv);
#pragma unroll
        for (int u = 0; u < 4; u++)
#pragma unroll
            for (int c = 0; c < 4; c++) {
                const int j = pp_get(ji[u], c);
                if (j >= 0 && pp_getf(wv[u], c) != 0.0f) atomicAdd(&hist[pp_bucket(j, rcp)], 1);
            }
    } else {
        for (int q = 0; q < 16; q++) {
            const int64_t i = r0 + q;
            if (i < rows && lane < K) {
                const int j = idx[i * K + lane];
                if (j >= 0 && w[i * K + lane] != 0.0f) atomicAdd(&hist[pp_bucket(j, rcp)], 1);
            }
        }
    }
    __syncthreads();
    int *row = T + (int64_t)blockIdx.x * nb;
    for (int b = tid; b < nb; b += THREADS) row[b] = hist[b];
}

__global__ __launch_bounds__(1024) void pp_scan(int *__restrict__ T, int nwg, int nb, int *__restrict__ totals) {
    __shared__ int part[32][33];
    const int c = threadIdx.x & 31, s = threadIdx.x >> 5;
    const int b = blockIdx.x * 32 + c;
    const int per = (nwg + 31) / 32;
    const int lo = s * per, hi = lo + per < nwg ? lo + per : nwg;
    constexpr int CHK = 16;
    int v[CHK];
    int sum = 0;
    for (int g0 = lo; g0 < hi; g0 += CHK) {
#pragma unroll
        for (int q = 0; q < CHK; q++) v[q] = (b < nb && g0 + q < hi) ? T[(int64_t)(g0 + q) * nb + b] : 0;
#pragma unroll
        for (int q = 0; q < CHK; q++) sum += v[q];
    }
    part[s][c] = sum;
    __syncthreads();
    int run = 0, tot = 0;
#pragma unroll
    for (int q = 0; q < 32; q++) {
        const int pv = part[q][c];
        if (q < s) run += pv;
        tot += pv;
    }
    if (b < nb && s == 0) totals[b] = tot;
    for (int g0 = lo; g0 < hi; g0 += CHK) {
        if (per > CHK) {
#pragma unroll
            for (int q = 0; q < CHK; q++) v[q] = (b < nb && g0 + q < hi) ? T[(int64_t)(g0 + q) * nb + b] : 0;
        }
#pragma unroll
        for (int q = 0; q < CHK; q++) {
            if (b < nb && g0 + q < hi) T[(int64_t)(g0 + q) * nb + b] = run;
            run += v[q];
        }
    }
}

template <int THREADS>
__device__ __forceinline__ int pp_block_scan(const int *__restrict__ in_g, int *__restrict__ out, int nb, int *__restrict__ scratch) {
    const int tid = threadIdx.x;
    const int per = (nb + THREADS - 1) / THREADS;
    const int lo = tid * per, hi = lo + per < nb ? lo + per : nb;
    int s = 0;
    for (int b = lo; b < hi; b++) s += in_g[b];
    int incl = s;
#pragma unroll
    for (int off = 1; off < 64; off <<= 1) {
        const int v = __shfl_up(incl, off, 64);
        if ((tid & 63) >= off) incl += v;
    }
// ... 273 lines not shown
                       static_cast<const void *>(dY), F, p.cstart, (int)ngroups, p.recs, a, K, dX);
    return dgg_check_launch("ell_spmm_t_part");
}
int dgg_ell_spmm_t_part_b16(const float *a, const void *dYb, int64_t rows, int K, int F, const void *part_ws, int64_t ncols, float *dX,
                            void *stream) {
    if (F % 64 != 0 || (reinterpret_cast<uintptr_t>(dYb) % 8) != 0)
        return dgg_set_error(DGG_ERR_UNSUPPORTED, "ell_spmm_t_part_b16: feature width must be a multiple of 64 (8-byte aligned rows)");
    if (rows == 0) return 0;
    const int64_t nb = nbuckets(ncols);
    PartHdr p = part_layout(const_cast<void *>(part_ws), nb, rows * K);
    const int64_t ngroups = (rows * K + CH - 1) / CH;
    hipLaunchKernelGGL(spmm_t_cols<true>, dim3((unsigned)((ngroups * 16 + 255) / 256), (unsigned)(F / 64)), dim3(256), 0, (hipStream_t)stream, dYb,
                       F, p.cstart, (int)ngroups, p.recs, a, K, dX);
    return dgg_check_launch("ell_spmm_t_part_b16");
}

int dgg_ell_conv_bwd_part(const float *G, const float *H, const float *ahat, int64_t rows, int K, int F, const void *part_ws,
                          int64_t ncols, const float *rs, float *dA, float *dH, float *da, void *stream) {
    if ((F != 16 && F != 32 && F != 64 && F != 128) || (reinterpret_cast<uintptr_t>(G) % 16) || (reinterpret_cast<uintptr_t>(H) % 16) ||
        (reinterpret_cast<uintptr_t>(dH) % 16))
        return dgg_set_error(DGG_ERR_UNSUPPORTED, "ell_conv_bwd_part: feature width must be 16, 32, 64 or 128 (16-byte aligned rows)");
    if (da && !rs) return dgg_set_error(DGG_ERR_ARG, "ell_conv_bwd_part: da needs the row sums");
    if (!dgg_part_slotmap(part_ws, rows, K, ncols)) return dgg_set_error(DGG_ERR_ARG, "ell_conv_bwd_part: no partition");
    if (rows == 0) return 0;
    const int64_t nb = nbuckets(ncols);
    PartHdr p = part_layout(const_cast<void *>(part_ws), nb, rows * K);
    const int64_t ngroups = (rows * K + CH - 1) / CH;
    hipStream_t st = (hipStream_t)stream;
#define DGG_CONV_COLS(FF)                                                                                                  \
    hipLaunchKernelGGL(conv_bwd_cols<FF>, dim3((unsigned)((ngroups * (FF / 4) + 255) / 256)), dim3(256), 0, st, G, H, ahat, K, \
                       p.bstart, (int)nb, p.recs, rs, dA, dH, da)
    switch (F) {
        case 16: DGG_CONV_COLS(16); break;
        case 32: DGG_CONV_COLS(32); break;
        case 64: DGG_CONV_COLS(64); break;
        default: DGG_CONV_COLS(128); break;
    }
#undef DGG_CONV_COLS
    return dgg_check_launch("ell_conv_bwd_part");
}

int dgg_partp_build_norm(const int32_t *idx, const float *w, const float *val, const float *rs_rows, int64_t rows, int K, int64_t ncols,
                         const float *rs_all, float *ahat, void *ws, void *stream);
int dgg_partp_build_phase(const int32_t *idx, const float *w, const float *val, const float *rs_rows, int64_t rows, int K, int64_t ncols,
                          const float *rs_all, float *ahat, void *ws, int phase, void *stream);
size_t dgg_partp_ws_bytes(int64_t rows, int K, int64_t ncols) {
    if (K > 64 || K < 1 || rows * 64 >= ((int64_t)1 << 31) || ncols < 1) return 0;
    PartP2 p;
    const size_t bytes = partp2_layout(p, nullptr, rows, K, ncols);
    if (p.nb > 4096 || p.width > 4096) return 0;
    return bytes;
}

int dgg_partp_build(const int32_t *idx, const float *w, const float *val, const float *rs_rows, int64_t rows, int K, int64_t ncols,
                    void *ws, void *stream) {
    return dgg_partp_build_norm(idx, w, val, rs_rows, rows, K, ncols, nullptr, nullptr, ws, stream);
}

int dgg_partp_build_norm(const int32_t *idx, const float *w, const float *val, const float *rs_rows, int64_t rows, int K, int64_t ncols,
                         const float *rs_all, float *ahat, void *ws, void *stream) {
    return dgg_partp_build_phase(idx, w, val, rs_rows, rows, K, ncols, rs_all, ahat, ws, 0, stream);
}

int dgg_partp_build_phase(const int32_t *idx, const float *w, const float *val, const float *rs_rows, int64_t rows, int K, int64_t ncols,
                          const float *rs_all, float *ahat, void *ws, int phase, void *stream) {
    hipStream_t st = (hipStream_t)stream;
    if (phase < 0 || phase > 2) return dgg_set_error(DGG_ERR_ARG, "partp_build_phase: phase is 0 (all), 1 (count + fill) or 2 (sort)");
    if (dgg_partp_ws_bytes(rows, K, ncols) == 0 || !ws) return dgg_set_error(DGG_ERR_UNSUPPORTED, "partp_build: unsupported size or NULL workspace");
    if (!val || !rs_rows) return dgg_set_error(DGG_ERR_ARG, "partp_build: the payload needs the scores and the row sums");
    if ((rs_all == nullptr) != (ahat == nullptr)) return dgg_set_error(DGG_ERR_ARG, "partp_build_norm: rs_all and ahat go together");
    if (K == 64 && ((reinterpret_cast<uintptr_t>(idx) | reinterpret_cast<uintptr_t>(w) | reinterpret_cast<uintptr_t>(val) |
                     reinterpret_cast<uintptr_t>(ahat)) % 16))
        return dgg_set_error(DGG_ERR_ARG, "partp_build: idx / w / val / ahat must be 16-byte aligned");
    if (rows == 0) return 0;
    PartP2 p;
    partp2_layout(p, ws, rows, K, ncols);
    const int nb = (int)p.nb, nwg = (int)p.nwg, pbs = p.width;
    if (phase == 2) {
        hipLaunchKernelGGL(pp_sort<false>, dim3((unsigned)nb), dim3(PP_T), (size_t)(2 * pbs + 16) * 4, st, p.bstart, p.tmp, p.recs, p.nodeptr, pp_builds_map(rows) ? p.recpos : nullptr, nb, pbs, (const int32_t *)nullptr);
        return dgg_check_launch("partp_build");
    }
#define DGG_PP_PASS(TT)                                                                                                      \
    hipLaunchKernelGGL(pp_count<TT>, dim3((unsigned)nwg), dim3(TT), (size_t)nb * 4, st, idx, w, rows, K, nb, p.rcp, p.T, rs_all, ncols, \
                       p.ainv);                                                                                              \
    hipLaunchKernelGGL(pp_scan, dim3((unsigned)((nb + 31) / 32)), dim3(1024), 0, st, p.T, nwg, nb, p.totals);                \
    hipLaunchKernelGGL(pp_fill<TT>, dim3((unsigned)nwg), dim3(TT), (size_t)(2 * nb + 16) * 4, st, idx, w, val, rs_rows, rows, K, nb, p.rcp, \
                       p.T, p.totals, p.bstart, p.tmp, p.ainv, ahat)
    switch (pp_threads()) {
        case 256: DGG_PP_PASS(256); break;
        case 512: DGG_PP_PASS(512); break;
        default: DGG_PP_PASS(1024); break;
    }
#undef DGG_PP_PASS
    if (phase == 1) return dgg_check_launch("partp_build");
    hipLaunchKernelGGL(pp_sort<false>, dim3((unsigned)nb), dim3(PP_T), (size_t)(2 * pbs + 16) * 4, st, p.bstart, p.tmp, p.recs, p.nodeptr, pp_builds_map(rows) ? p.recpos : nullptr, nb, pbs, (const int32_t *)nullptr);
    return dgg_check_launch("partp_build");
}

int dgg_partp_has_map(int64_t rows) { return pp_builds_map(rows) ? 1 : 0; }

}
int dgg_partp_internal_ptrs(const void *partp_ws, int64_t rows, int K, int64_t ncols, const int **nodeptr, const int **recpos) {
    if (!partp_ws || dgg_partp_ws_bytes(rows, K, ncols) == 0 || !pp_builds_map(rows)) return 1;
    PartP2 p;
    partp2_layout(p, const_cast<void *>(partp_ws), rows, K, ncols);
    *nodeptr = p.nodeptr;
    *recpos = p.recpos;
    return 0;
}
extern "C" {
int dgg_partp_describe(int64_t rows, int K, int64_t ncols, int64_t *out6) {
    if (!out6 || dgg_partp_ws_bytes(rows, K, ncols) == 0) return dgg_set_error(DGG_ERR_UNSUPPORTED, "partp_describe: no payload partition for this shape");
    PartP2 p;
    partp2_layout(p, nullptr, rows, K, ncols);
    out6[0] = reinterpret_cast<char *>(p.bstart) - static_cast<char *>(nullptr);
    out6[1] = reinterpret_cast<char *>(p.nodeptr) - static_cast<char *>(nullptr);
    out6[2] = reinterpret_cast<char *>(p.recs) - static_cast<char *>(nullptr);
    out6[3] = p.nb;
    out6[4] = p.width;
    out6[5] = pp_threads() / 4;
    return 0;
}

static bool node_split(int64_t ncols) {
    static const int forced = [] { const char *e = getenv("DGG_NODE_SPLIT"); return e ? atoi(e) : -1; }();
    return forced >= 0 ? forced != 0 : ncols <= NODE_SPLIT_MAX;
}
static bool node_groups(int64_t nrec, int64_t ncols) {
    static const int forced = [] { const char *e = getenv("DGG_NODE_GROUPS"); return e ? atoi(e) : -1; }();
    return forced >= 0 ? forced != 0 : nrec < 16 * ncols;
}

int dgg_ell_conv_bwd_partp_ext(const float *G, const float *H, int64_t rows, int K, int F, const void *partp_ws, int64_t ncols,
                               const float *rs, const float *dA_ext, float *dA, float *dA_rec, float *dH, float *da, void *stream);
int dgg_ell_conv_bwd_partp(const float *G, const float *H, int64_t rows, int K, int F, const void *partp_ws, int64_t ncols,
                           const float *rs, float *dA, float *dA_rec, float *dH, float *da, void *stream) {
    return dgg_ell_conv_bwd_partp_ext(G, H, rows, K, F, partp_ws, ncols, rs, nullptr, dA, dA_rec, dH, da, stream);
}
int dgg_ell_conv_bwd_partp_ext(const float *G, const float *H, int64_t rows, int K, int F, const void *partp_ws, int64_t ncols,
                               const float *rs, const float *dA_ext, float *dA, float *dA_rec, float *dH, float *da, void *stream) {
    if ((F != 16 && F != 32 && F != 64 && F != 128) || (reinterpret_cast<uintptr_t>(G) % 16) || (reinterpret_cast<uintptr_t>(H) % 16) ||
        (reinterpret_cast<uintptr_t>(dH) % 16))
        return dgg_set_error(DGG_ERR_UNSUPPORTED, "ell_conv_bwd_partp: feature width must be 16, 32, 64 or 128 (16-byte aligned rows)");
    if (!rs || !partp_ws || !dA_rec || dgg_partp_ws_bytes(rows, K, ncols) == 0) return dgg_set_error(DGG_ERR_ARG, "ell_conv_bwd_partp: missing operand");
    if (rows == 0) return 0;
    PartP2 p;
    partp2_layout(p, const_cast<void *>(partp_ws), rows, K, ncols);
    hipStream_t st = (hipStream_t)stream;
    const bool grouped = !dA_ext && node_groups(rows * K, ncols);
    const unsigned nmain = (unsigned)((ncols + 3) / 4);
    const bool split = node_split(ncols);
    const dim3 gridn(split ? nmain + (unsigned)ncols : nmain);
#define DGG_CONV_COLS_P(FF)                                                                                                \
    if (dA_ext)                                                                                                            \
        hipLaunchKernelGGL((conv_bwd_node<FF, true>), gridn, dim3(256), 0, st, G, H, K, ncols, p.nodeptr, p.recs,          \
                           rs, dA, dA_rec, dH, da, dA_ext, split ? nmain : 0u);                                            \
    else if (grouped)                                                                                                      \
        hipLaunchKernelGGL((conv_bwd_nodeg<FF, 4>), dim3((unsigned)((ncols + 4 * (256 / FF) - 1) / (4 * (256 / FF)))), dim3(256), 0, st, G, H, K, \
                           ncols, p.nodeptr, p.recs, rs, dA, dA_rec, dH, da);                                              \
    else                                                                                                                   \
        hipLaunchKernelGGL((conv_bwd_node<FF, false>), gridn, dim3(256), 0, st, G, H, K, ncols, p.nodeptr, p.recs,         \
                           rs, dA, dA_rec, dH, da, (const float *)nullptr, split ? nmain : 0u)
    switch (F) {
        case 16: DGG_CONV_COLS_P(16); break;
        case 32: DGG_CONV_COLS_P(32); break;
        case 64: DGG_CONV_COLS_P(64); break;
        default: DGG_CONV_COLS_P(128); break;
    }
#undef DGG_CONV_COLS_P
    return dgg_check_launch("ell_conv_bwd_partp");
}

int dgg_softk_edge_bwd_partp_phase(const float *xp, int64_t rows, int h, const int32_t *idx, const float *val, const float *k, const float *rs,
                                   const float *dA, const float *dA_rec, const float *da, const float *ahat_rows, int K, int64_t row0, float t,
                                   int perturb, int mode, int normalized, const void *partp_ws, int64_t ncols, float *rowinfo_ws, float *dk,
                                   float *dxp, int out_act, int phase, void *stream);
int dgg_softk_edge_bwd_partp(const float *xp, int64_t rows, int h, const int32_t *idx, const float *val, const float *k, const float *rs,
                             const float *dA, const float *dA_rec, const float *da, const float *ahat_rows, int K, int64_t row0, float t,
                             int perturb, int mode, int normalized, const void *partp_ws, int64_t ncols, float *rowinfo_ws, float *dk,
                             float *dxp, int out_act, void *stream) {
    return dgg_softk_edge_bwd_partp_phase(xp, rows, h, idx, val, k, rs, dA, dA_rec, da, ahat_rows, K, row0, t, perturb, mode, normalized,
                                          partp_ws, ncols, rowinfo_ws, dk, dxp, out_act, 0, stream);
}

int dgg_softk_edge_bwd_partp_phase(const float *xp, int64_t rows, int h, const int32_t *idx, const float *val, const float *k, const float *rs,
                                   const float *dA, const float *dA_rec, const float *da, const float *ahat_rows, int K, int64_t row0, float t,
                                   int perturb, int mode, int normalized, const void *partp_ws, int64_t ncols, float *rowinfo_ws, float *dk,
                                   float *dxp, int out_act, int phase, void *stream) {
    if (phase < 0 || phase > 2) return dgg_set_error(DGG_ERR_ARG, "softk_edge_bwd_partp_phase: phase is 0 (all), 1 (rows) or 2 (nodes)");
    if (mode != 0 && mode != 1) return dgg_set_error(DGG_ERR_ARG, "softk_edge_bwd_partp: mode must be 0 (k_times) or 1 (k_only)");
    if (out_act != 0 && (out_act != 1 || mode != 0))
        return dgg_set_error(DGG_ERR_ARG, "softk_edge_bwd_partp: out_act is 0 or 1 (LeakyReLU), mode 0 only");
    if (!k || !dA_rec || !dk || !rowinfo_ws || (normalized && (!rs || !da))) return dgg_set_error(DGG_ERR_ARG, "softk_edge_bwd_partp: missing operand");
    if (!dA && !(normalized && ahat_rows))
        return dgg_set_error(DGG_ERR_ARG, "softk_edge_bwd_partp: dA may be NULL only in the normalised form with ahat_rows");
    if (!dA && !pp_builds_map(rows))
        return dgg_set_error(DGG_ERR_ARG, "softk_edge_bwd_partp: dA is NULL but the partition of a block this large carries no slot -> record "
                                          "map (dgg_partp_has_map)");
    if (ahat_rows && !normalized) return dgg_set_error(DGG_ERR_ARG, "softk_edge_bwd_partp: ahat_rows is an operand of the normalised form");
    if (!partp_ws || dgg_partp_ws_bytes(rows, K, ncols) == 0) return dgg_set_error(DGG_ERR_ARG, "softk_edge_bwd_partp: no partition");
    if (rows == 0) return 0;
    hipStream_t st = (hipStream_t)stream;
    PartP2 p;
    partp2_layout(p, const_cast<void *>(partp_ws), rows, K, ncols);
    const SoftkArgs sk{k, rs, dA, da, mode, normalized, nullptr, dk, ahat_rows, reinterpret_cast<float4 *>(rowinfo_ws),
                       dA ? nullptr : p.recpos, dA_rec};
    const unsigned gr = (unsigned)((rows + 3) / 4);
    const bool grouped = node_groups(rows * K, ncols);
    const unsigned nmain = (unsigned)((ncols + 3) / 4);
    const bool split = node_split(ncols);
#define DGG_EDGE_PARTP(HH)                                                                                                  \
    if (phase != 2)                                                                                                          \
        hipLaunchKernelGGL((edge_bwd_rows<HH, true, true>), dim3(gr), dim3(256), 0, st, xp, rows, idx, val, nullptr, K, row0, t, perturb, nullptr, \
                           nullptr, dxp, sk);                                                                                \
    if (phase == 1) {                                                                                                        \
    } else if (mode == 0 && grouped)                                                                                         \
        hipLaunchKernelGGL((edge_bwd_nodeg<HH, 4>), dim3((unsigned)((ncols + 4 * (256 / HH) - 1) / (4 * (256 / HH)))), dim3(256), 0, st, xp, \
                           ncols, p.nodeptr, p.recs, dA_rec, reinterpret_cast<const float4 *>(rowinfo_ws), rs, normalized, row0, rows, t, \
                           perturb, dxp, out_act);                                                                           \
    else if (mode == 0)                                                                                                      \
        hipLaunchKernelGGL(edge_bwd_node<HH>, dim3(split ? nmain + (unsigned)ncols : nmain), dim3(256), 0, st, xp, ncols, p.nodeptr, p.recs, \
                           dA_rec, reinterpret_cast<const float4 *>(rowinfo_ws), rs, normalized, row0, rows, t, perturb, dxp, out_act,  \
                           split ? nmain : 0u)
    switch (h) {
        case 16: DGG_EDGE_PARTP(16); break;
        case 32: DGG_EDGE_PARTP(32); break;
        case 64: DGG_EDGE_PARTP(64); break;
        case 128: DGG_EDGE_PARTP(128); break;
        default: return dgg_set_error(DGG_ERR_UNSUPPORTED, "softk_edge_bwd_partp supports latent_dim in {16,32,64,128}");
    }
#undef DGG_EDGE_PARTP
    return dgg_check_launch("softk_edge_bwd_partp");
}

int dgg_partp_build_chunked(const int32_t *idx, const float *w, const float *val, const float *rs_nodes, int64_t chunks, const int32_t *cnode,
                            int64_t ncols, const float *rs_all, float *ahat, void *ws, int phase, void *stream) {
    hipStream_t st = (hipStream_t)stream;
    const int K = 64;
    if (phase < 0 || phase > 2) return dgg_set_error(DGG_ERR_ARG, "partp_build_chunked: phase is 0 (all), 1 (count + fill) or 2 (sort)");
    if (dgg_partp_ws_bytes(chunks, K, ncols) == 0 || !ws) return dgg_set_error(DGG_ERR_UNSUPPORTED, "partp_build_chunked: unsupported size or NULL workspace");
    if (!val || !rs_nodes || !cnode) return dgg_set_error(DGG_ERR_ARG, "partp_build_chunked: the payload needs the scores, the row sums and the chunk nodes");
    if ((rs_all == nullptr) != (ahat == nullptr)) return dgg_set_error(DGG_ERR_ARG, "partp_build_chunked: rs_all and ahat go together");
    if ((reinterpret_cast<uintptr_t>(idx) | reinterpret_cast<uintptr_t>(w) | reinterpret_cast<uintptr_t>(val) | reinterpret_cast<uintptr_t>(ahat)) % 16)
        return dgg_set_error(DGG_ERR_ARG, "partp_build_chunked: idx / w / val / ahat must be 16-byte aligned");
    if (chunks == 0) return 0;
    PartP2 p;
    partp2_layout(p, ws, chunks, K, ncols);
    const int nb = (int)p.nb, nwg = (int)p.nwg, pbs = p.width;
    if (phase != 2) {
#define DGG_PP_PASS(TT)                                                                                                      \
    hipLaunchKernelGGL(pp_count<TT>, dim3((unsigned)nwg), dim3(TT), (size_t)nb * 4, st, idx, w, chunks, K, nb, p.rcp, p.T, rs_all, ncols, \
                       p.ainv);                                                                                              \
    hipLaunchKernelGGL(pp_scan, dim3((unsigned)((nb + 31) / 32)), dim3(1024), 0, st, p.T, nwg, nb, p.totals);                \
    hipLaunchKernelGGL(pp_fill<TT>, dim3((unsigned)nwg), dim3(TT), (size_t)(2 * nb + 16) * 4, st, idx, w, val, rs_nodes, chunks, K, nb, p.rcp, \
                       p.T, p.totals, p.bstart, p.tmp, p.ainv, ahat, cnode)
        switch (pp_threads()) {
            case 256: DGG_PP_PASS(256); break;
            case 512: DGG_PP_PASS(512); break;
            default: DGG_PP_PASS(1024); break;
        }
#undef DGG_PP_PASS
    }
    if (phase != 1)
        hipLaunchKernelGGL(pp_sort<true>, dim3((unsigned)nb), dim3(PP_T), (size_t)(2 * pbs + 16) * 4, st, p.bstart, p.tmp, p.recs, p.nodeptr,
                           (int *)nullptr, nb, pbs, cnode);
    return dgg_check_launch("partp_build_chunked");
}

int dgg_ell_conv_bwd_partp_chunked(const float *G, const float *H, int64_t chunks, int F, const void *partp_ws, int64_t ncols, const float *rs,
                                   const float *dA_ext, float *dA, float *dA_rec, float *dH, float *da, void *stream) {
    const int K = 64;
    if ((F != 16 && F != 32 && F != 64 && F != 128) || (reinterpret_cast<uintptr_t>(G) % 16) || (reinterpret_cast<uintptr_t>(H) % 16) ||
        (reinterpret_cast<uintptr_t>(dH) % 16))
        return dgg_set_error(DGG_ERR_UNSUPPORTED, "ell_conv_bwd_partp_chunked: feature width must be 16, 32, 64 or 128 (16-byte aligned rows)");
    if (!rs || !partp_ws || !dA_rec || !dA || dgg_partp_ws_bytes(chunks, K, ncols) == 0) return dgg_set_error(DGG_ERR_ARG, "ell_conv_bwd_partp_chunked: missing operand");
    if (chunks == 0) return 0;
    PartP2 p;
    partp2_layout(p, const_cast<void *>(partp_ws), chunks, K, ncols);
    hipStream_t st = (hipStream_t)stream;
    const unsigned nmain = (unsigned)((ncols + 3) / 4);
    const bool split = node_split(ncols);
    const dim3 gridn(split ? nmain + (unsigned)ncols : nmain);
#define DGG_CONV_COLS_C(FF)                                                                                                \
    if (dA_ext)                                                                                                            \
        hipLaunchKernelGGL((conv_bwd_node<FF, true>), gridn, dim3(256), 0, st, G, H, K, ncols, p.nodeptr, p.recs,          \
                           rs, dA, dA_rec, dH, da, dA_ext, split ? nmain : 0u, 1);                                         \
    else                                                                                                                   \
        hipLaunchKernelGGL((conv_bwd_node<FF, false>), gridn, dim3(256), 0, st, G, H, K, ncols, p.nodeptr, p.recs,         \
                           rs, dA, dA_rec, dH, da, (const float *)nullptr, split ? nmain : 0u, 1)
    switch (F) {
        case 16: DGG_CONV_COLS_C(16); break;
        case 32: DGG_CONV_COLS_C(32); break;
        case 64: DGG_CONV_COLS_C(64); break;
        default: DGG_CONV_COLS_C(128); break;
    }
#undef DGG_CONV_COLS_C
    return dgg_check_launch("ell_conv_bwd_partp_chunked");
}

int dgg_softk_edge_bwd_partp_chunked(const float *xp, int64_t rows, const int32_t *cptr, int64_t chunks, int h, const int32_t *idx, const float *val,
                                     const float *k, const float *rs, const float *dA, const float *dA_rec, const float *da, const float *ahat_rows,
                                     int64_t row0, float t, int perturb, int mode, int normalized, const void *partp_ws, int64_t ncols,
                                     float *rowinfo_ws, float *dk, float *dxp, int out_act, int phase, void *stream) {
    const int K = 64;
    if (phase < 0 || phase > 2) return dgg_set_error(DGG_ERR_ARG, "softk_edge_bwd_partp_chunked: phase is 0 (all), 1 (rows) or 2 (nodes)");
    if (mode != 0 && mode != 1) return dgg_set_error(DGG_ERR_ARG, "softk_edge_bwd_partp_chunked: mode must be 0 (k_times) or 1 (k_only)");
    if (out_act != 0 && (out_act != 1 || mode != 0)) return dgg_set_error(DGG_ERR_ARG, "softk_edge_bwd_partp_chunked: out_act is 0 or 1 (LeakyReLU), mode 0 only");
    if (!k || !cptr || !dA || !dA_rec || !dk || !rowinfo_ws || (normalized && (!rs || !da)))
        return dgg_set_error(DGG_ERR_ARG, "softk_edge_bwd_partp_chunked: missing operand");
    if (ahat_rows && !normalized) return dgg_set_error(DGG_ERR_ARG, "softk_edge_bwd_partp_chunked: ahat_rows is an operand of the normalised form");
    if (!partp_ws || dgg_partp_ws_bytes(chunks, K, ncols) == 0) return dgg_set_error(DGG_ERR_ARG, "softk_edge_bwd_partp_chunked: no partition");
    if (rows == 0) return 0;
    hipStream_t st = (hipStream_t)stream;
    PartP2 p;
    partp2_layout(p, const_cast<void *>(partp_ws), chunks, K, ncols);
    const SoftkArgs sk{k, rs, dA, da, mode, normalized, nullptr, dk, ahat_rows, reinterpret_cast<float4 *>(rowinfo_ws), nullptr, dA_rec};
    const unsigned gr = (unsigned)((rows + 3) / 4);
    const unsigned nmain = (unsigned)((ncols + 3) / 4);
    const bool split = node_split(ncols);
#define DGG_EDGE_PARTC(HH)                                                                                                   \
    if (phase != 2)                                                                                                          \
        hipLaunchKernelGGL((edge_bwd_rows_chunked<HH>), dim3(gr), dim3(256), 0, st, xp, rows, cptr, idx, val, row0, t, perturb, dxp, sk); \
    if (phase != 1 && mode == 0)                                                                                             \
        hipLaunchKernelGGL(edge_bwd_node<HH>, dim3(split ? nmain + (unsigned)ncols : nmain), dim3(256), 0, st, xp, ncols, p.nodeptr, p.recs, \
                           dA_rec, reinterpret_cast<const float4 *>(rowinfo_ws), rs, normalized, row0, rows, t, perturb, dxp, out_act,  \
                           split ? nmain : 0u, 1)
    switch (h) {
        case 16: DGG_EDGE_PARTC(16); break;
        case 32: DGG_EDGE_PARTC(32); break;
        case 64: DGG_EDGE_PARTC(64); break;
        case 128: DGG_EDGE_PARTC(128); break;
        default: return dgg_set_error(DGG_ERR_UNSUPPORTED, "softk_edge_bwd_partp_chunked supports latent_dim in {16,32,64,128}");
    }
#undef DGG_EDGE_PARTC
    return dgg_check_launch("softk_edge_bwd_partp_chunked");
}

int dgg_partp_gather_rec(const float *dA, int64_t rows, int64_t ncols, const void *partp_ws, float *dA_rec, void *stream) {
    if (!dA || !dA_rec || !partp_ws || dgg_partp_ws_bytes(rows, 64, ncols) == 0) return dgg_set_error(DGG_ERR_ARG, "partp_gather_rec: missing operand or no partition");
    if (rows == 0) return 0;
    PartP2 p;
    partp2_layout(p, const_cast<void *>(partp_ws), rows, 64, ncols);
    hipLaunchKernelGGL(pp_gather_rec, dim3((unsigned)((rows * 64 + 255) / 256)), dim3(256), 0, (hipStream_t)stream, p.bstart, (int)p.nb, p.recs, dA, dA_rec);
    return dgg_check_launch("partp_gather_rec");
}

int dgg_norm_bwd_da_part(const int32_t *idx, const float *w, const float *rs, const float *dA, int64_t rows, int K, int64_t row0,
                         const void *part_ws, int64_t ncols, float *coef_ws, float *da, void *stream) {
    hipStream_t st = (hipStream_t)stream;
    if (rows == 0) return 0;
    const int64_t nb = nbuckets(ncols);
    PartHdr p = part_layout(const_cast<void *>(part_ws), nb, rows * K);
    hipLaunchKernelGGL(norm_da_rows, dim3((unsigned)((rows + 3) / 4)), dim3(256), 0, st, idx, w, rs, dA, rows, K, row0, p.slot, coef_ws, da);
    hipLaunchKernelGGL(norm_da_cols, dim3((unsigned)nb), dim3(256), 0, st, ncols, p.bstart, p.recs, coef_ws, da);
    return dgg_check_launch("norm_bwd_da_part");
}

}
```

### learning-adaptive-neighborhoods-for-gnns_amd/ops.py

```python
import collections
import math
import os
import ctypes as C

import torch

from . import _lib

NOISE_NONE, NOISE_EXPLICIT, NOISE_HASH, NOISE_HASH_SYM, NOISE_RANKED, NOISE_RANKED_SYM = 0, 1, 2, 3, 4, 5
RSYM_WIDTHS = (8, 16, 32, 64, 128)
ACT_NONE, ACT_LEAKY, ACT_RELU = 0, 1, 2
MODE_K_TIMES_EDGE_PROB, MODE_K_ONLY = 0, 1
MODE_HARD_ST = 3
DEFAULT_K = 64
T_DIST = -0.05

PROBE = None



_POOL = None


class zero_pool:
# ... 43 lines not shown
        e1 = torch.cuda.Event(enable_timing=True)
        e1.record()
        PROBE.setdefault(name, []).append((e0, e1))


def _ptr(t):
    return None if t is None else C.c_void_p(t.data_ptr())


def _stream():
    return C.c_void_p(torch.cuda.current_stream().cuda_stream)


def backward_will_follow(*tensors):
    return torch.is_grad_enabled() and any(torch.is_tensor(t) and t.requires_grad for t in tensors)


_KEEP = collections.deque(maxlen=64)


def _chk(t, dtype=torch.float32):
    assert t.is_cuda, "dgg ops run on the GPU only (no CPU fallback)"
    assert t.dtype == dtype, f"expected {dtype}, got {t.dtype}"
    if t.is_contiguous():
        return t
    c = t.contiguous()
    _KEEP.append(c)
    return c


def linear_fwd(x, W, b=None, act=ACT_NONE, w_layout=0):
    x, W = _chk(x), _chk(W)
    N, d = x.shape
    out = W.shape[0] if w_layout == 0 else W.shape[1]
    assert (W.shape[1] if w_layout == 0 else W.shape[0]) == d
    y = torch.empty((N, out), device=x.device, dtype=torch.float32)
    bb = _chk(b) if b is not None else None
    pe = _probe_begin()
    _lib.check(_lib.lib().dgg_linear_fwd(_ptr(x), N, d, _ptr(W), _ptr(bb), out, w_layout, act, _ptr(y), _stream()), "linear_fwd")
    _probe_end("linear_fwd", pe)
    return y


def linear_bwd(x, W, y, dy, act=ACT_NONE, w_layout=0, need_dx=True, need_db=True):
    x, W, dy = _chk(x), _chk(W), _chk(dy)
    N, d = x.shape
    out = W.shape[0] if w_layout == 0 else W.shape[1]
    dx = torch.empty_like(x) if need_dx else None
    zz = _zeros((W.numel() + (out if need_db else 0),), x.device)
    dW = zz[:W.numel()].view(W.shape)
    db = zz[W.numel():] if need_db else None
    ws = torch.empty((int(_lib.lib().dgg_linear_bwd_ws_floats(N, d, out)),), device=x.device, dtype=torch.float32)
    yy = _chk(y) if act != ACT_NONE else None
    pe = _probe_begin()
    _lib.check(_lib.lib().dgg_linear_bwd(_ptr(x), N, d, _ptr(W), out, w_layout, act, _ptr(yy), _ptr(dy), _ptr(dx), _ptr(dW),
                                         _ptr(db), _ptr(ws), _stream()), "linear_bwd")
    _probe_end("linear_bwd", pe)
    return dx, dW, db


def _ptr_array(ts):
    return (C.c_void_p * len(ts))(*[None if t is None else t.data_ptr() for t in ts])


def _int_array(vs):
    return (C.c_int * len(vs))(*[int(v) for v in vs])


def linear_fwd_multi(x, layers):
    x = _chk(x)
    N, d = x.shape
    outs = [(W.shape[0] if lay == 0 else W.shape[1]) for W, _, _, lay in layers]
    if len(layers) > 1 and sum(outs) > 256 and not any(o % 32 for o in outs) and max(outs) <= 256:
        res, grp, tot = [], [], 0
        for lay_, o in zip(layers, outs):
            if grp and tot + o > 256:
                res += linear_fwd_multi(x, grp)
                grp, tot = [], 0
            grp.append(lay_)
            tot += o
        return res + linear_fwd_multi(x, grp)
    if len(layers) > 8 or any(o % 32 for o in outs) or sum(outs) > 256 or sum(outs) == 224:
        return [linear_fwd(x, W, b, act, lay) for W, b, act, lay in layers]
    Wcat = torch.empty((sum(outs), d), device=x.device, dtype=torch.float32)
    bcat = torch.empty((sum(outs),), device=x.device, dtype=torch.float32)
    _lib.check(_lib.lib().dgg_linear_pack_weights(len(layers), _ptr_array([_chk(W) for W, *_ in layers]),
                                                  _ptr_array([None if b is None else _chk(b) for _, b, _, _ in layers]), _int_array(outs),
                                                  _int_array([lay for *_, lay in layers]), d, _ptr(Wcat), _ptr(bcat), _stream()),
               "linear_pack_weights")
    ys = [torch.empty((N, o), device=x.device, dtype=torch.float32) for o in outs]
    _lib.check(_lib.lib().dgg_linear_fwd_multi(_ptr(x), N, d, _ptr(Wcat), _ptr(bcat), len(layers), _int_array(outs),
                                               _int_array([a for _, _, a, _ in layers]), _ptr_array(ys), _stream()), "linear_fwd_multi")
    return ys


def linear_bwd_multi(x, layers):
    x = _chk(x)
    N, d = x.shape
    outs = [(W.shape[0] if lay == 0 else W.shape[1]) for W, _, _, _, lay, _ in layers]
    if len(layers) > 1 and sum(outs) > 256 and d <= 128 and not any(o % 32 for o in outs) and max(outs) <= 256:
        res, grp, tot = [], [], 0
        for lay_, o in zip(layers, outs):
            if grp and tot + o > 256:
                res += linear_bwd_multi(x, grp)
                grp, tot = [], 0
            grp.append(lay_)
            tot += o
        return res + linear_bwd_multi(x, grp)
    wide_in = d > 128 and d % 4 == 0 and not any(o % 64 for o in outs) and x.data_ptr() % 16 == 0
    if len(layers) > 8 or any(o % 32 for o in outs) or sum(outs) > 256 or (d > 128 and not wide_in):
        res = []
        for W, y, dy, act, lay, need_db in layers:
            _, dW, db = linear_bwd(x, W, y, dy, act, lay, need_dx=False, need_db=need_db)
            res.append((dW, db))
        return res
    nW = [int(W.numel()) for W, *_ in layers]
    zz = _zeros((sum(nW) + sum(o for o, l_ in zip(outs, layers) if l_[5]),), x.device)
    dWs, dbs, o_ = [], [], 0
    for (W, *_), n_ in zip(layers, nW):
        dWs.append(zz[o_:o_ + n_].view(W.shape))
        o_ += n_
    for (_, _, _, _, _, need_db), o in zip(layers, outs):
        dbs.append(zz[o_:o_ + o] if need_db else None)
        o_ += o if need_db else 0
    ws = torch.empty((int(_lib.lib().dgg_gemm_tn_multi_ws_floats(N, sum(outs), d)),), device=x.device, dtype=torch.float32)
    dys = [_chk(l_[2]) for l_ in layers]
    ysv = [(_chk(l_[1]) if (l_[1] is not None and l_[3] != ACT_NONE) else None) for l_ in layers]
    _lib.check(_lib.lib().dgg_gemm_tn_multi(len(layers), _ptr_array(dys), _int_array(outs), _ptr_array(ysv),
                                            _int_array([l_[3] for l_ in layers]), _ptr(x), N, d, _ptr_array(dWs),
                                            _int_array([0 if l_[4] == 0 else 1 for l_ in layers]), _ptr_array(dbs), _ptr(ws), _stream()),
               "gemm_tn_multi")
    return list(zip(dWs, dbs))


def gemm_tn(A, B, colsum=False):
    A, B = _chk(A), _chk(B)
    N, M1 = A.shape
    M2 = B.shape[1]
    zz = _zeros((M1 * M2 + (M1 if colsum else 0),), A.device)
    Cm = zz[:M1 * M2].view(M1, M2)
    cs = zz[M1 * M2:] if colsum else None
    ws = torch.empty((int(_lib.lib().dgg_gemm_tn_ws_floats(N, M1, M2)),), device=A.device, dtype=torch.float32)
    _lib.check(_lib.lib().dgg_gemm_tn_acc(_ptr(A), _ptr(B), N, M1, M2, _ptr(Cm), 0, _ptr(cs), _ptr(ws), _stream()), "gemm_tn_acc")
    return (Cm, cs) if colsum else Cm


def gemm_tn_pairs(pairs):
    As, Bs = [_chk(a) for a, _ in pairs], [_chk(b) for _, b in pairs]
    N = As[0].shape[0]
    M1s, M2s = [a.shape[1] for a in As], [b.shape[1] for b in Bs]
    tot = sum((m + 31) // 32 * 32 for m in M1s)
    if len(pairs) > 8 or tot > 256 or max(M2s) > 128:
        return [gemm_tn(a, b, colsum=True) for a, b in zip(As, Bs)]
    zz = _zeros((sum(m1 * m2 + m1 for m1, m2 in zip(M1s, M2s)),), As[0].device)
    Cs, css, o = [], [], 0
    for m1, m2 in zip(M1s, M2s):
        Cs.append(zz[o:o + m1 * m2].view(m1, m2))
        css.append(zz[o + m1 * m2:o + m1 * m2 + m1])
        o += m1 * m2 + m1
    ws = torch.empty((int(_lib.lib().dgg_gemm_tn_multi_ws_floats(N, tot, 128)),), device=As[0].device, dtype=torch.float32)
    _lib.check(_lib.lib().dgg_gemm_tn_pairs(len(pairs), _ptr_array(As), _int_array(M1s), _ptr_array(Bs), _int_array(M2s), N, _ptr_array(Cs),
                                            _ptr_array(css), _ptr(ws), _stream()), "gemm_tn_pairs")
    return list(zip(Cs, css))


_DEGSTAT_CACHE = {}


def degree_stats(deg):
    import weakref
    key = id(deg)
    ent = _DEGSTAT_CACHE.get(key)
    if ent is not None and ent[0]() is deg and ent[1] == deg._version:
        return ent[2]
    degc = _chk(deg)
    out = torch.empty((2,), device=degc.device, dtype=torch.float32)
    ws = torch.empty((int(_lib.lib().dgg_degree_stats_ws_bytes()),), device=degc.device, dtype=torch.uint8)
    _lib.check(_lib.lib().dgg_degree_stats(_ptr(degc), degc.shape[0], _ptr(out), _ptr(ws), _stream()), "degree_stats")
    if not torch.cuda.is_current_stream_capturing() and not deg.requires_grad:
        for k_ in [k_ for k_, v in _DEGSTAT_CACHE.items() if v[0]() is None]:
            del _DEGSTAT_CACHE[k_]
        _DEGSTAT_CACHE[key] = (weakref.ref(deg), deg._version, out)
    return out


def allpairs_topk(xp, K=DEFAULT_K, t=T_DIST, noise_mode=NOISE_NONE, G=None, seed=(0, 0), rows=None, algo=0,
                  return_ws=False, k_limit=None, status=None):
    xp = _chk(xp)
    N, h = xp.shape
    r0, r1 = (0, N) if rows is None else rows
    idx = torch.empty((r1 - r0, K), device=xp.device, dtype=torch.int32)
    val = torch.empty((r1 - r0, K), device=xp.device, dtype=torch.float32)
    ldG = 0
    if G is not None:
        G = _chk(G)
        assert G.shape[-1] == N and G.shape[0] == N, "explicit noise must be [N, N]"
        ldG = N
    ws, ws_bytes = None, 0
    if algo != 1 or noise_mode == NOISE_RANKED_SYM:
        ws_bytes = int(_lib.lib().dgg_allpairs_workspace_bytes(N, h, noise_mode, K))
        if ws_bytes:
            ws = torch.empty((ws_bytes,), device=xp.device, dtype=torch.uint8)
    pe = _probe_begin()
    _lib.check(_lib.lib().dgg_allpairs_topk(_ptr(xp), N, h, r0, r1, t, noise_mode, _ptr(G), ldG, seed[0], seed[1], K,
                                            _ptr(idx), _ptr(val), _ptr(None if k_limit is None else _chk(k_limit)), algo, _ptr(ws),
                                            ws_bytes, _stream()), "allpairs_topk")
    _probe_end("allpairs_topk", pe)
    if status is not None and noise_mode == NOISE_RANKED_SYM and ws is not None:
        off = int(_lib.lib().dgg_allpairs_rsym_ctl_offset_bytes(r1 - r0, N))
        ctl = ws[off:off + 32].view(torch.int32)
        if status.get("sym_fallback") and not torch.cuda.is_current_stream_capturing() and bool(ctl[4].item()):
            status["rsym_fell_back"] = True
            status["rsym_err"] = None
# ... 1641 lines not shown
```

### learning-adaptive-neighborhoods-for-gnns_amd/parallel.py

```python
import os
import weakref

import torch
import torch.distributed as dist


def shard_bounds(N, world, rank):
    per = (N + world - 1) // world
    r0 = min(rank * per, N)
    return r0, min(r0 + per, N), per


def csr_rows(rowptr, col, rows):
    r0, r1 = int(rows[0]), int(rows[1])
    e0, e1 = (int(v) for v in rowptr[[r0, r1]].tolist())
    return (rowptr[r0:r1 + 1] - e0).contiguous(), col[e0:e1], (e0, e1)


class _Gather:

    def __init__(self, t_local, N, per, group, async_op, bufs=None, key=None):
        world = dist.get_world_size(group)
        tail = tuple(t_local.shape[1:])
        n_loc = t_local.shape[0]
# ... 236 lines not shown
            lp = self._row_bound(xp, s["k"])
            if lp is not None:
                lkw_["lpub"] = lp
            if lay is not None:
                s["idx"], s["val"], s["w"], rs_local = kern.allpairs_topk_wide(xp, s["k"], lay, self.mode, self.t, self.seed, rows=(self.r0, self.r1), **lkw_)
            else:
                s["idx"], s["val"], s["w"], rs_local = kern.allpairs_topk_softk(xp, s["k"], self.mode, self.t, self.seed, rows=(self.r0, self.r1), **lkw_)
        else:
            lay = self._chunk_layout(s["k"]) if (xp.shape[1] in (16, 32, 64, 128) and self.mode in (0, 1)) else None
            s["layout"] = lay
            if lay is not None:
                s["idx"], s["val"], s["w"], rs_local = kern.allpairs_topk_wide(xp, s["k"], lay, self.mode, self.t, self.seed, rows=(self.r0, self.r1),
                                                                             noise_mode=self.WIDE_NOISE[self.noise_mode])
            else:
                nm = 3 if (self.noise_mode == 5 and self.sym_hash) else self.noise_mode
                if nm == 5 and not hasattr(kern, "rsym_status"):
                    st = None
                else:
                    st = {"sym_fallback": self.sym_fallback and self.world == 1} if nm == 5 else None
                kw = {} if st is None else {"status": st}
                s["idx"], s["val"] = kern.allpairs_topk(xp, self.K, self.t, nm, None, self.seed,
                                                        rows=(self.r0, self.r1), algo=self.algo, k_limit=s["k"], **kw)
                if st and st.get("rsym_fell_back"):
                    self.sym_hash = True
                if st and st.get("rsym_err") is not None:
                    self.rsym_err = st["rsym_err"] if getattr(self, "rsym_err", None) is None else (self.rsym_err | st["rsym_err"])
                    self.rsym_last = st
                s["w"], rs_local = kern.softk_fwd(s["idx"], s["val"], s["k"], self.mode)
        s["rs"] = rs = _all_gather_rows(rs_local, self.N, self.per, self.group, self.bufs, "rs") if self.coll else rs_local
        if self.emulate is not None:
            s["rs"] = rs = rs_local.repeat(self.world)[:self.N].contiguous()
        use_p = hasattr(kern, "partp_build") and xp.shape[1] in (16, 32, 64, 128) and H.shape[1] in (16, 32, 64, 128) and self.mode in (0, 1)
        ov = use_p and self.overlap and self.overlap_sort and s["idx"].is_cuda
        nobwd = use_p and not getattr(self, "want_backward", True)
        lay = s.get("layout")
        lkw = {} if lay is None else {"layout": lay}
        assert lay is None or use_p, "chunked rows run on the payload partition (latent / conv widths 16, 32, 64, 128; soft modes)"
        got = (kern.partp_build(s["idx"], s["w"], s["val"], rs_local, self.N, rs, phase=1, **lkw) if (ov or nobwd) else
               kern.partp_build(s["idx"], s["w"], s["val"], rs_local, self.N, rs, **lkw)) if use_p else None
        s["partp"], s["ahat"] = got if got is not None else (None, None)
        s["side_join"] = False
        s["partp_sorted"] = not nobwd
        if nobwd and got is not None:
            s["partp"].args = None
        elif ov and got is not None:
            main, side = torch.cuda.current_stream(), self._side_stream()
            side.wait_stream(main)
            with torch.cuda.stream(side):
                kern.partp_sort(s["partp"])
            if not torch.cuda.is_current_stream_capturing():
                s["partp"].ws.record_stream(side)
            s["side_join"] = True
        s["part"] = kern.part_build(s["idx"], s["w"], self.N) if (s["partp"] is None and hasattr(kern, "part_build")) else None
        if s["ahat"] is None:
            s["ahat"] = kern.normalize_fwd(s["idx"], s["w"], rs, self.r0)
        if self.coll and (not repl or hyb):
            H = g_H.get()
        elif hyb:
            Hf = _Gather._buf(self.bufs, ("H", "emu"), (self.N, H.shape[1]), H)
            if not self.bufs.get(("H", "emu_init")):
                Hf.copy_(H.repeat((self.N + H.shape[0] - 1) // H.shape[0], 1)[:self.N])
                self.bufs[("H", "emu_init")] = True
            Hf[self.r0:self.r1].copy_(H)
            H = Hf
        s["H"] = H
        s["Z"] = kern.spmm_fwd(s["idx"], s["ahat"], H, 2, **lkw)
        s["gen"] = self._fwd_gen
        self.saved = s
        return s["Z"]

    def backward(self, dZ, x_local, P, dA_ext=None):
        kern, s = self.kern, self.saved
        assert s.get("gen") == getattr(self, "_fwd_gen", None), "ShardedDGGConv: backward() must follow the forward() it differentiates " \
            "(a second forward has overwritten the gathered buffers)"
        assert s.get("partp_sorted", True), "ShardedDGGConv: this forward ran with want_backward = False (its partition was not sorted)"
        if hasattr(kern, "zero_pool"):
            ncols, h, F = s["xp"].shape[0], s["xp"].shape[1], s["H"].shape[1]
            rows = s["idx"].shape[0]
            need = 3 * sum(int(v.numel()) for v in P.values()) + 65536
            if s.get("partp") is None:
                need += rows * self.K + ncols * (h + F + 2)
            if self.scorer is not None:
                need += rows * self.K + ncols * (2 * self.scorer["Wcat"].shape[0] + h) + 4 * int(self.scorer["Wcat"].numel()) + 4096
            with kern.zero_pool(s["xp"].device, need):
                return self._backward(dZ, x_local, P, dA_ext)
        return self._backward(dZ, x_local, P, dA_ext)

    def _reduce_scatter_rows(self, t, key, async_op=False):
        pad = self.world * self.per - self.N
        src = t
        if pad:
            src = _Gather._buf(self.bufs, (key, "rs_src"), (self.world * self.per, t.shape[1]), t)
            src[:self.N].copy_(t)
            src[self.N:].zero_()
        out = _Gather._buf(self.bufs, (key, "rs_out"), (self.per, t.shape[1]), t)
        src = src.contiguous()
        work = dist.reduce_scatter_tensor(out, src, group=self.group, async_op=async_op)
        if not async_op:
            return out[: self.r1 - self.r0]

        def get(_keep=src):
            work.wait()
            return out[: self.r1 - self.r0]
        return get

    def _backward(self, dZ, x_local, P, dA_ext=None):
        kern, s = self.kern, self.saved
        g = {}
        repl = self.x_full is not None
        part = s.get("part")
        G = kern.act_bwd(s["Z"], dZ, 2)
        partp = s.get("partp")
        if partp is not None:
            if s.get("side_join"):
                torch.cuda.current_stream().wait_stream(self._side_stream())
                s["side_join"] = False
            use_map = getattr(kern, "DA_MAP", False) and kern.partp_has_map(s["idx"].shape[0]) and self.scorer is None and s.get("layout") is None
            kw = {"want_dA": False} if use_map else {}
            if dA_ext is not None:
                kw["dA_ext"] = dA_ext
            pc = kern.conv_bwd_cols_p(s["idx"], s["H"], G, partp, s["rs"], zero_dA=self.scorer is not None, **kw)
            assert pc is not None
            dA, dA_rec, dH, da = pc
            if self.scorer is not None:
                return self._scorer_backward(g, dA, dH, da, x_local, P, cols_only=True)
            if self.coll:
                dist.all_reduce(da, group=self.group)
            if self._hyb() and self.coll:
                dH = self._reduce_scatter_rows(dH, "dH", async_op=True)
            pre = self._premask(x_local)
            if self.overlap and self.overlap_knet and self.mode == 0 and s["z"] is None and s["idx"].is_cuda:
                dxp, dk, st = kern.softk_edge_bwd_p(s["xp"], s["idx"], s["val"], s["k"], dA, dA_rec, s["rs"], da, self.r0, self.t,
                                                    self.noise_mode != 0, self.mode, True, partp, ahat_rows=s["ahat"],
                                                    out_act=1 if pre else 0, phase=1)
                main, side = torch.cuda.current_stream(), self._side_stream()
                side.wait_stream(main)
                with torch.cuda.stream(side):
                    kn = kern.knet_x_bwd_fused(s["xk"], s["deg_local"], s["mu_sd"], P["W1"], P["b1"], P["Wmu"], P["bmu"],
                                               P["Wp"].reshape(-1), s["u"], dk, out_act=1 if pre else 0)
                kern.softk_edge_bwd_p(s["xp"], s["idx"], s["val"], s["k"], dA, dA_rec, s["rs"], da, self.r0, self.t,
                                      self.noise_mode != 0, self.mode, True, partp, ahat_rows=s["ahat"], out_act=1 if pre else 0,
                                      phase=2, state=st)
                main.wait_stream(side)
                if not torch.cuda.is_current_stream_capturing():
                    dk.record_stream(side)
                    for t_ in kn:
                        t_.record_stream(main)
                return self._weight_grads(g, dxp, dH, dk, x_local, P, premasked=pre, knet=kn)
            dxp, dk = kern.softk_edge_bwd_p(s["xp"], s["idx"], s["val"], s["k"], dA, dA_rec, s["rs"], da, self.r0, self.t,
                                            self.noise_mode != 0, self.mode, True, partp, ahat_rows=s["ahat"], out_act=1 if pre else 0)
            return self._weight_grads(g, dxp, dH, dk, x_local, P, premasked=pre)
        cols = None
        if self.scorer is None and dA_ext is None and part is not None and hasattr(kern, "conv_bwd_cols") and hasattr(kern, "softk_edge_bwd") and \
                s["xp"].shape[1] in (16, 32, 64, 128) and self.mode in (0, 1):
            cols = kern.conv_bwd_cols(s["idx"], s["ahat"], s["H"], G, part, s["rs"], True)
        if cols is not None:
            dA, dH, da = cols
            ahat_rows = s["ahat"]
        else:
            dA, dH = kern.spmm_bwd(s["idx"], s["ahat"], s["H"], G, True, True)
            if dA_ext is not None:
                dA = dA + torch.where(s["idx"] >= 0, dA_ext, torch.zeros_like(dA_ext))
            da = kern.norm_bwd_da(s["idx"], s["w"], s["rs"], dA, self.r0, part) if part is not None else \
                kern.norm_bwd_da(s["idx"], s["w"], s["rs"], dA, self.r0)
            ahat_rows = None
        if self.scorer is not None:
# ... 117 lines not shown
```

Before: 2.650 billion edges/s.

## Skip weight packing, store gemm_tn results directly, and add live/ainv edge paths

Adds an unpacked multi-segment linear forward that reads each segment's weights directly into shared memory, so the separate pack-weights kernel and concatenated buffers are no longer needed. Adds a store mode to the TN gemm reduction so gradient buffers are written instead of accumulated, which removes the zero-fill and lets the backward pass skip the zero pool. Also changes the edge backward kernels: a new payload row kernel, a 'live' flag, and precomputed ainv inputs, all on by default through environment variables. This spreads several unrelated changes across the forward linear, the weight-gradient GEMM and the edge backward, and adds new code paths with more complex layout handling.

```diff
diff --git a/include/dgg_hip.h b/include/dgg_hip.h
--- a/include/dgg_hip.h
+++ b/include/dgg_hip.h
@@ -38,9 +38,15 @@
                             float *Wcat, float *bcat, void *stream);
 int dgg_linear_fwd_multi(const float *x, int64_t N, int d, const float *Wcat, const float *bcat, int nseg, const int *seg_out,
                          const int *seg_act, float *const *y, void *stream);
+int dgg_linear_fwd_multi_unpacked_ok(const float *x, int64_t N, int d, int nseg, const float *const *W, const int *seg_out,
+                                     const int *seg_layout);
+int dgg_linear_fwd_multi_unpacked(const float *x, int64_t N, int d, int nseg, const float *const *W, const float *const *b,
+                                  const int *seg_out, const int *seg_layout, const int *seg_act, float *const *y, void *stream);
 size_t dgg_gemm_tn_multi_ws_floats(int64_t N, int M1_total, int M2);
 int dgg_gemm_tn_multi(int nseg, const float *const *A, const int *M1, const float *const *Y, const int *act, const float *B,
                       int64_t N, int M2, float *const *C, const int *c_layout, float *const *colsum, float *ws, void *stream);
+int dgg_gemm_tn_multi_store(int nseg, const float *const *A, const int *M1, const float *const *Y, const int *act, const float *B,
+                            int64_t N, int M2, float *const *C, const int *c_layout, float *const *colsum, float *ws, void *stream);
 int dgg_gemm_tn_pairs(int npair, const float *const *A, const int *M1, const float *const *B, const int *M2, int64_t N, float *const *C,
                       float *const *colsum, float *ws, void *stream);
 size_t dgg_gemm_tn_ws_floats(int64_t N, int M1, int M2);
diff --git a/learning-adaptive-neighborhoods-for-gnns_amd/_lib.py b/learning-adaptive-neighborhoods-for-gnns_amd/_lib.py
--- a/learning-adaptive-neighborhoods-for-gnns_amd/_lib.py
+++ b/learning-adaptive-neighborhoods-for-gnns_amd/_lib.py
@@ -13,7 +13,10 @@
     "dgg_gemm_tn_ws_floats": [_i64, _i32, _i32],
     "dgg_linear_pack_weights": [_i32, _vp, _vp, _vp, _vp, _i32, _vp, _vp, _vp],
     "dgg_linear_fwd_multi": [_vp, _i64, _i32, _vp, _vp, _i32, _vp, _vp, _vp, _vp],
+    "dgg_linear_fwd_multi_unpacked_ok": [_vp, _i64, _i32, _i32, _vp, _vp, _vp],
+    "dgg_linear_fwd_multi_unpacked": [_vp, _i64, _i32, _i32, _vp, _vp, _vp, _vp, _vp, _vp, _vp],
     "dgg_gemm_tn_multi": [_i32, _vp, _vp, _vp, _vp, _vp, _i64, _i32, _vp, _vp, _vp, _vp, _vp],
+    "dgg_gemm_tn_multi_store": [_i32, _vp, _vp, _vp, _vp, _vp, _i64, _i32, _vp, _vp, _vp, _vp, _vp],
     "dgg_gemm_tn_multi_ws_floats": [_i64, _i32, _i32],
     "dgg_gemm_tn_pairs": [_i32, _vp, _vp, _vp, _vp, _i64, _vp, _vp, _vp, _vp],
     "dgg_linear_bwd_ws_floats": [_i64, _i32, _i32],
diff --git a/learning-adaptive-neighborhoods-for-gnns_amd/csrc/dgg_linear.hip b/learning-adaptive-neighborhoods-for-gnns_amd/csrc/dgg_linear.hip
--- a/learning-adaptive-neighborhoods-for-gnns_amd/csrc/dgg_linear.hip
+++ b/learning-adaptive-neighborhoods-for-gnns_amd/csrc/dgg_linear.hip
@@ -19,6 +19,11 @@
     float *y[8];
     int ld[8];
     int act[8];
+};
+struct LinBlkW {
+    const float *W[8];
+    const float *b[8];
+    int layout[8];
 };
 
 template <int NACC, int WAVES, bool MULTI = false>
@@ -162,9 +167,9 @@
     }
 }
 
-template <int D, int NACC>
+template <int D, int NACC, bool UNP = false>
 __global__ __launch_bounds__(256, 1) void linear_fwd_reg(const float *__restrict__ x, int64_t N, const float *__restrict__ W,
-                                                         const float *__restrict__ b, LinSegs segs, int64_t nrb) {
+                                                         const float *__restrict__ b, LinSegs segs, int64_t nrb, LinBlkW wu = LinBlkW{}) {
     constexpr int S = D / 2, XR = D / 2;
     __shared__ float wsf[S * NACC * 64];
     const int tid = threadIdx.x, lane = tid & 63, wave = dgg::wave_id(), li = lane & 31, hh = lane >> 5;
@@ -189,20 +194,57 @@
         }
     };
     if (nunits > 0) load_rows(unit_rb(0), xc);
-#pragma unroll
-    for (int it = 0; it < NACC * 32 * (D / 4) / 256; it++) {
-        const int e = tid + it * 256;
-        const int j = e % (NACC * 32), q = e / (NACC * 32);
-        const float4 v = *reinterpret_cast<const float4 *>(W + (int64_t)j * D + 4 * q);
-        float *dst = wsf + ((2 * q) * NACC + (j >> 5)) * 64 + (j & 31);
-        dst[0] = v.x; dst[32] = v.y; dst[NACC * 64] = v.z; dst[NACC * 64 + 32] = v.w;
-    }
-    const bool hasb = b != nullptr;
+    if constexpr (!UNP) {
+#pragma unroll
+        for (int it = 0; it < NACC * 32 * (D / 4) / 256; it++) {
+            const int e = tid + it * 256;
+            const int j = e % (NACC * 32), q = e / (NACC * 32);
+            const float4 v = *reinterpret_cast<const float4 *>(W + (int64_t)j * D + 4 * q);
+            float *dst = wsf + ((2 * q) * NACC + (j >> 5)) * 64 + (j & 31);
+            dst[0] = v.x; dst[32] = v.y; dst[NACC * 64] = v.z; dst[NACC * 64 + 32] = v.w;
+        }
+    } else {
+        constexpr int NU = 2 * NACC, UI = (NU + 3) / 4, LPU = D / 16;
+        float4 v[UI][LPU];
+#pragma unroll
+        for (int ui = 0; ui < UI; ui++) {
+            const int u = wave + 4 * ui < NU ? wave + 4 * ui : NU - 1, a = u >> 1;
+            const bool t1 = wu.layout[a] != 0;
+            const int64_t stride = t1 ? segs.ld[a] : D;
+            const int r0 = t1 ? lane >> 3 : li, dr = t1 ? 8 : 0, c0 = t1 ? lane & 7 : hh, dc = t1 ? 0 : 2;
+#pragma unroll
+            for (int i = 0; i < LPU; i++) {
+                const int ii = (u & 1) * LPU + i;
+                v[ui][i] = *reinterpret_cast<const float4 *>(wu.W[a] + (r0 + dr * ii) * stride + 4 * (c0 + dc * ii));
+            }
+        }
+#pragma unroll
+        for (int ui = 0; ui < UI; ui++) {
+            const int u = wave + 4 * ui, a = u >> 1;
+            if (u >= NU) break;
+            const bool t1 = wu.layout[a] != 0;
+#pragma unroll
+            for (int i = 0; i < LPU; i++) {
+                const int ii = (u & 1) * LPU + i;
+                const float4 w4 = v[ui][i];
+                if (!t1) {
+                    const int q = hh + 2 * ii;
+                    float *dst = wsf + ((2 * q) * NACC + a) * 64 + li;
+                    dst[0] = w4.x; dst[32] = w4.y; dst[NACC * 64] = w4.z; dst[NACC * 64 + 32] = w4.w;
+                } else {
+                    const int k = (lane >> 3) + 8 * ii;
+                    *reinterpret_cast<float4 *>(wsf + ((k >> 1) * NACC + a) * 64 + (k & 1) * 32 + 4 * (lane & 7)) = w4;
+                }
+            }
+        }
+    }
+    const bool hasb = UNP || b != nullptr;
     float bj[NACC];
     int actv[NACC];
 #pragma unroll
     for (int a = 0; a < NACC; a++) {
-        bj[a] = hasb ? b[a * 32 + li] : 0.0f;
+        if constexpr (UNP) bj[a] = wu.b[a] ? wu.b[a][li] : 0.0f;
+        else bj[a] = hasb ? b[a * 32 + li] : 0.0f;
         actv[a] = segs.act[a];
     }
     __syncthreads();
@@ -288,7 +330,15 @@
             const float av = s < S / 2 ? xc[2 * s] : xc[2 * (s - S / 2) + 1];
             acc = __builtin_amdgcn_mfma_f32_32x32x2f32(wa[s * NACC * 64], av, acc, 0, 0, 0);
         }
-        if (hasb) acc = __builtin_amdgcn_mfma_f32_32x32x2f32(b[a * 32 + li] * one_or_zero, one_or_zero, acc, 0, 0, 0);
+        if constexpr (UNP) {
+            float ba = bj[0];
+#pragma unroll
+            for (int a2 = 1; a2 < NACC; a2++)
+                if (a == a2) ba = bj[a2];
+            acc = __builtin_amdgcn_mfma_f32_32x32x2f32(ba * one_or_zero, one_or_zero, acc, 0, 0, 0);
+        } else if (hasb) {
+            acc = __builtin_amdgcn_mfma_f32_32x32x2f32(b[a * 32 + li] * one_or_zero, one_or_zero, acc, 0, 0, 0);
+        }
         store_block(acc, a, rb);
 #pragma unroll
         for (int q = 0; q < XR; q++) xc[q] = xn[q];
@@ -718,6 +768,7 @@
     float *C[8];
     float *colsum[8];
     int M1[8], M2[8], M1p[8], rowbase[8], c_layout[8];
+    int store;
 };
 __global__ __launch_bounds__(1024) void gemm_tn_reduce_multi(const float *__restrict__ slab, const float *__restrict__ cs_slab, int nchunks,
                                                              int M2p, int64_t chunk_stride, int64_t cs_stride, RedSegs rs) {
@@ -751,12 +802,12 @@
     const float v = total(slab + (int64_t)rs.rowbase[sgi] * M2p + e, chunk_stride, ok);
     if (ok && pw == 0) {
         float *dst = rs.c_layout[sgi] == 0 ? rs.C[sgi] + (int64_t)o * M2 + c : rs.C[sgi] + (int64_t)c * M1 + o;
-        *dst += v;
+        *dst = rs.store ? v : *dst + v;
     }
     if (rs.colsum[sgi] && blockIdx.x * 64 < M1) {
         const bool okc = e < M1;
         const float cv = total(cs_slab + rs.rowbase[sgi] + e, cs_stride, okc);
-        if (okc && pw == 0) rs.colsum[sgi][e] += cv;
+        if (okc && pw == 0) rs.colsum[sgi][e] = rs.store ? cv : rs.colsum[sgi][e] + cv;
     }
 }
 
@@ -912,6 +963,59 @@
     return dgg_check_launch("linear_pack_weights");
 }
 
+static bool lin_unpacked() { const char *e = getenv("DGG_LIN_UNPACKED"); return e ? atoi(e) != 0 : true; }
+static int lin_reg_forced() { static const int forced = [] { const char *e = getenv("DGG_LINEAR_REG"); return e ? atoi(e) : -1; }(); return forced; }
+static int lin_multi_blocks(int nseg, const int *seg_out) {
+    int cb = 0;
+    for (int s = 0; s < nseg; s++) {
+        if (seg_out[s] < 32 || seg_out[s] % 32 != 0 || cb + seg_out[s] / 32 > 8) return -1;
+        cb += seg_out[s] / 32;
+    }
+    return cb;
+}
+
+int dgg_linear_fwd_multi_unpacked_ok(const float *x, int64_t N, int d, int nseg, const float *const *W, const int *seg_out, const int *seg_layout) {
+    if (!lin_unpacked() || !x || !W || !seg_out || !seg_layout || nseg < 1 || nseg > 8 || d != 128 || N < 1) return 0;
+    const int cb = lin_multi_blocks(nseg, seg_out);
+    if (cb < 1 || cb > 6) return 0;
+    if (reinterpret_cast<uintptr_t>(x) % 16) return 0;
+    for (int s = 0; s < nseg; s++) {
+        if (!W[s] || (seg_layout[s] != 0 && seg_layout[s] != 1)) return 0;
+        if (reinterpret_cast<uintptr_t>(W[s]) % 16) return 0;
+    }
+    const int forced = lin_reg_forced();
+    return (forced >= 0 ? forced != 0 : N >= 32768) ? 1 : 0;
+}
+
+int dgg_linear_fwd_multi_unpacked(const float *x, int64_t N, int d, int nseg, const float *const *W, const float *const *b, const int *seg_out,
+                                  const int *seg_layout, const int *seg_act, float *const *y, void *stream) {
+    if (!seg_act || !y) return dgg_set_error(DGG_ERR_ARG, "linear_fwd_multi_unpacked: missing operand");
+    if (!dgg_linear_fwd_multi_unpacked_ok(x, N, d, nseg, W, seg_out, seg_layout))
+        return dgg_set_error(DGG_ERR_UNSUPPORTED, "linear_fwd_multi_unpacked: shape outside the persistent kernel's range "
+                                                  "(dgg_linear_fwd_multi_unpacked_ok)");
+    LinSegs segs{};
+    LinBlkW wu{};
+    int cb = 0;
+    for (int s = 0; s < nseg; s++)
+        for (int q = 0; q < seg_out[s] / 32; q++, cb++) {
+            segs.y[cb] = y[s] + q * 32;
+            segs.ld[cb] = seg_out[s];
+            segs.act[cb] = seg_act[s];
+            wu.W[cb] = seg_layout[s] == 0 ? W[s] + (int64_t)q * 32 * d : W[s] + q * 32;
+            wu.b[cb] = (b && b[s]) ? b[s] + q * 32 : nullptr;
+            wu.layout[cb] = seg_layout[s];
+        }
+    const int64_t nrb = (N + 31) / 32;
+    const unsigned grid = (unsigned)std::min<int64_t>(256, (nrb + 3) / 4);
+    hipStream_t st = (hipStream_t)stream;
+    switch (cb) {
+#define DGG_LIN_REG_U(NA) case NA: hipLaunchKernelGGL((linear_fwd_reg<128, NA, true>), dim3(grid), dim3(256), 0, st, x, N, (const float *)nullptr, (const float *)nullptr, segs, nrb, wu); break
+        DGG_LIN_REG_U(1); DGG_LIN_REG_U(2); DGG_LIN_REG_U(3); DGG_LIN_REG_U(4); DGG_LIN_REG_U(5); DGG_LIN_REG_U(6);
+#undef DGG_LIN_REG_U
+    }
+    return dgg_check_launch("linear_fwd_multi_unpacked");
+}
+
 int dgg_linear_fwd_multi(const float *x, int64_t N, int d, const float *Wcat, const float *bcat, int nseg, const int *seg_out,
                          const int *seg_act, float *const *y, void *stream) {
     if (N < 0 || d < 1 || nseg < 1 || nseg > 8) return dgg_set_error(DGG_ERR_ARG, "linear_fwd_multi: bad shape");
@@ -930,13 +1034,13 @@
     if (N == 0) return 0;
     const int out = cb * 32;
     hipStream_t st = (hipStream_t)stream;
-    static const int forced = [] { const char *e = getenv("DGG_LINEAR_REG"); return e ? atoi(e) : -1; }();
+    const int forced = lin_reg_forced();
     const bool aligned = (reinterpret_cast<uintptr_t>(x) % 16 == 0) && (reinterpret_cast<uintptr_t>(Wcat) % 16 == 0);
     if (d == 128 && aligned && cb <= 6 && (forced >= 0 ? forced != 0 : N >= 32768)) {
         const int64_t nrb = (N + 31) / 32;
         const unsigned grid = (unsigned)std::min<int64_t>(256, (nrb + 3) / 4);
         switch (cb) {
-#define DGG_LIN_REG(NA) case NA: hipLaunchKernelGGL((linear_fwd_reg<128, NA>), dim3(grid), dim3(256), 0, st, x, N, Wcat, bcat, segs, nrb); break
+#define DGG_LIN_REG(NA) case NA: hipLaunchKernelGGL((linear_fwd_reg<128, NA, false>), dim3(grid), dim3(256), 0, st, x, N, Wcat, bcat, segs, nrb, LinBlkW{}); break
             DGG_LIN_REG(1); DGG_LIN_REG(2); DGG_LIN_REG(3); DGG_LIN_REG(4); DGG_LIN_REG(5); DGG_LIN_REG(6);
 #undef DGG_LIN_REG
         }
@@ -1004,8 +1108,18 @@
     const size_t M2p = (size_t)(M2 + 31) / 32 * 32;
     return (size_t)256 * ((size_t)M1_total * M2p + (size_t)M1_total);
 }
+static int gemm_tn_multi_impl(int nseg, const float *const *A, const int *M1, const float *const *Y, const int *act, const float *B, int64_t N,
+                             int M2, float *const *C, const int *c_layout, float *const *colsum, float *ws, int store, void *stream);
 int dgg_gemm_tn_multi(int nseg, const float *const *A, const int *M1, const float *const *Y, const int *act, const float *B, int64_t N,
                       int M2, float *const *C, const int *c_layout, float *const *colsum, float *ws, void *stream) {
+    return gemm_tn_multi_impl(nseg, A, M1, Y, act, B, N, M2, C, c_layout, colsum, ws, 0, stream);
+}
+int dgg_gemm_tn_multi_store(int nseg, const float *const *A, const int *M1, const float *const *Y, const int *act, const float *B, int64_t N,
+                            int M2, float *const *C, const int *c_layout, float *const *colsum, float *ws, void *stream) {
+    return gemm_tn_multi_impl(nseg, A, M1, Y, act, B, N, M2, C, c_layout, colsum, ws, 1, stream);
+}
+static int gemm_tn_multi_impl(int nseg, const float *const *A, const int *M1, const float *const *Y, const int *act, const float *B, int64_t N,
+                              int M2, float *const *C, const int *c_layout, float *const *colsum, float *ws, int store, void *stream) {
     if (nseg < 1 || nseg > 8 || M2 < 1) return dgg_set_error(DGG_ERR_UNSUPPORTED, "gemm_tn_multi: 1..8 operands");
     if (!ws) return dgg_set_error(DGG_ERR_ARG, "gemm_tn_multi: workspace is NULL (dgg_gemm_tn_multi_ws_floats)");
     TnSegs segs{};
@@ -1022,8 +1136,16 @@
         }
     }
     segs.nyb = yb;
+    hipStream_t st = (hipStream_t)stream;
+    if (N == 0 && store) {
+        for (int sgi = 0; sgi < nseg; sgi++) {
+            if (dgg_check_hip(hipMemsetAsync(C[sgi], 0, (size_t)M1[sgi] * M2 * sizeof(float), st), "gemm_tn_multi memset") != 0) return DGG_ERR_HIP;
+            if (colsum && colsum[sgi] && dgg_check_hip(hipMemsetAsync(colsum[sgi], 0, (size_t)M1[sgi] * sizeof(float), st), "gemm_tn_multi memset") != 0)
+                return DGG_ERR_HIP;
+        }
+        return 0;
+    }
     if (N == 0) return 0;
-    hipStream_t st = (hipStream_t)stream;
     const int M2p = (M2 + 31) / 32 * 32, M1tp = yb * 32;
     constexpr int PF = 4;
     int G = 128;
@@ -1070,6 +1192,7 @@
         rb += M1[sgi];
         m1max = M1[sgi] > m1max ? M1[sgi] : m1max;
     }
+    rsg.store = store;
     hipLaunchKernelGGL(gemm_tn_reduce_multi, dim3((unsigned)((m1max * M2p + 63) / 64), 1, (unsigned)nseg), dim3(1024), 0, st,
                        slab, cs_slab, G, M2p, (int64_t)M1tp * M2p, (int64_t)M1tp, rsg);
     return dgg_check_launch("gemm_tn_multi");
diff --git a/learning-adaptive-neighborhoods-for-gnns_amd/csrc/dgg_scatter.hip b/learning-adaptive-neighborhoods-for-gnns_amd/csrc/dgg_scatter.hip
--- a/learning-adaptive-neighborhoods-for-gnns_amd/csrc/dgg_scatter.hip
+++ b/learning-adaptive-neighborhoods-for-gnns_amd/csrc/dgg_scatter.hip
@@ -165,6 +165,9 @@
     if (tid == 1023) bstart[nb] = part[1023];
 }
 
+static int edge_live() { const char *e = getenv("DGG_EDGE_LIVE"); return e ? atoi(e) != 0 : 1; }
+static int edge_ainv() { const char *e = getenv("DGG_EDGE_AINV"); return e ? atoi(e) != 0 : 1; }
+
 struct SoftkArgs {
     const float *k, *rs, *dA, *da;
     int mode, normalized;
@@ -173,7 +176,71 @@
     float4 *rowinfo;
     const int *recpos;
     const float *dA_rec;
+    const float *ainv;
+    const int *ainv_ok;
+    int live;
 };
+
+template <int H>
+__device__ __forceinline__ void edge_rows_group(const float *__restrict__ xp, int64_t gi, int r0, int K, bool mine, int32_t jl, bool myact,
+                                                 float gl, float vl, const float4 xi, float t, int perturb, int lane, int nbl, float4 &acc) {
+    constexpr int LPR = H / 4, NPI = 64 / LPR, NBT = (32 / NPI) < 1 ? 1 : 32 / NPI;
+    constexpr int Q = NBT >= 2 ? NBT / 2 : NBT;
+    const int c4 = lane % LPR, slot = lane / LPR;
+    const bool run1 = nbl > Q;
+    float4 xj[NBT];
+    float myd2 = 0.0f, mydd = 0.0f;
+    auto gather = [&](auto B0, auto B1) {
+#pragma unroll
+        for (int b = B0; b < B1; b++) {
+            const int r = r0 + b * NPI + slot;
+            const int rr = r < 64 ? r : 63;
+            const int32_t jb = __shfl(jl, rr, 64);
+            const bool ab = __shfl((int)myact, rr, 64) != 0 && r < K;
+            xj[b] = *reinterpret_cast<const float4 *>(xp + (ab ? (int64_t)jb : gi) * H + 4 * c4);
+        }
+    };
+    auto dist2 = [&](auto B0, auto B1) {
+#pragma unroll
+        for (int b = B0; b < B1; b++) {
+            const float4 d = make_float4(xi.x - xj[b].x, xi.y - xj[b].y, xi.z - xj[b].z, xi.w - xj[b].w);
+            float d2 = d.x * d.x + d.y * d.y + d.z * d.z + d.w * d.w;
+            if (LPR > 16) d2 += __uint_as_float(xor_shfl<16>(__float_as_uint(d2), lane));
+            if (LPR > 8) d2 += __uint_as_float(xor_shfl<8>(__float_as_uint(d2), lane));
+            if (LPR > 4) d2 += __uint_as_float(xor_shfl<4>(__float_as_uint(d2), lane));
+            if (LPR > 2) d2 += __uint_as_float(xor_shfl<2>(__float_as_uint(d2), lane));
+            d2 += __uint_as_float(xor_shfl<1>(__float_as_uint(d2), lane));
+            const float tq = __shfl(d2, (lane % NPI) * LPR, 64);
+            if ((lane - r0) / NPI == b && mine) myd2 = tq;
+        }
+    };
+    auto accum = [&](auto B0, auto B1) {
+#pragma unroll
+        for (int b = B0; b < B1; b++) {
+            const int r = r0 + b * NPI + slot;
+            const float dd = __shfl(mydd, r < 64 ? r : 63, 64);
+            const float4 d = make_float4(xi.x - xj[b].x, xi.y - xj[b].y, xi.z - xj[b].z, xi.w - xj[b].w);
+            acc.x += dd * d.x; acc.y += dd * d.y; acc.z += dd * d.z; acc.w += dd * d.w;
+        }
+    };
+    using std::integral_constant;
+    constexpr integral_constant<int, 0> c0{};
+    constexpr integral_constant<int, Q> c1{};
+    constexpr integral_constant<int, NBT> c2{};
+    if (run1) gather(c1, c2);
+    gather(c0, c1);
+    if (run1) dist2(c1, c2);
+    dist2(c0, c1);
+    if (mine && myact && myd2 != 0.0f) {
+        const float dist = sqrtf(myd2);
+        const float p = c_exp(t * dist);
+        const float dp = perturb ? gl * vl / (p + 1e-8f) : gl;
+        mydd = dp * t * p / dist;
+    }
+    accum(c0, c1);
+    if (run1) accum(c1, c2);
+}
+
 template <int H, bool FUSE, bool PAY = false>
 __global__ __launch_bounds__(256) void edge_bwd_rows(const float *__restrict__ xp, int64_t rows, const int32_t *__restrict__ idx,
                                                      const float *__restrict__ val, const float *__restrict__ dval, int K,
@@ -280,6 +347,75 @@
         const int sl = slotmap[i * K + lane];
         if (sl >= 0) coef[sl] = mycoef;
     }
+}
+
+template <int H>
+__global__ __launch_bounds__(256) __attribute__((amdgpu_waves_per_eu(H == 64 ? 7 : (H == 128 ? 4 : 8))))
+void edge_bwd_rows_pay(const float *__restrict__ xp, int64_t rows, const int32_t *__restrict__ idx, const float *__restrict__ val, int K,
+                       int64_t row0, float t, int perturb, float *__restrict__ dxp, SoftkArgs sk) {
+    constexpr int LPR = H / 4;
+    constexpr int NPI = 64 / LPR;
+    const int lane = threadIdx.x & 63, c4 = lane % LPR, slot = lane / LPR;
+    const int64_t i = (int64_t)blockIdx.x * 4 + dgg::wave_id();
+    if (i >= rows) return;
+    const int64_t gi = row0 + i;
+    const int32_t jl = lane < K ? idx[i * K + lane] : -1;
+    const float vl = lane < K ? val[i * K + lane] : 0.0f;
+    float gl;
+    {
+        const int lc = lane < K ? lane : K - 1;
+        const bool viamap = sk.recpos != nullptr;
+        float dw = viamap ? 0.0f : sk.dA[i * K + lc];
+        const int rpos = viamap ? sk.recpos[i * 64 + lc] : 0;
+        const bool live = lane < K && jl >= 0;
+        if (sk.normalized) {
+            const float rsi = sk.rs[gi];
+            const float ai = __fdiv_rn(1.0f, c_sqrt(rsi));
+            const bool tab = sk.ainv != nullptr && *sk.ainv_ok != 0;
+            const int64_t jj = jl >= 0 ? jl : gi;
+            const float aj = tab ? sk.ainv[jj] : __fdiv_rn(1.0f, c_sqrt(sk.rs[jj]));
+            float dai = sk.da[gi];
+            if (sk.ahat_rows) {
+                const float ah = lane < K ? sk.ahat_rows[i * K + lane] : 0.0f;
+                if (viamap) dw = sk.dA_rec[ah != 0.0f ? rpos : 0];
+                if (ah == 0.0f) dw = 0.0f;
+                float rp = dw * ah;
+                rp = wave_sum_dpp(rp, lane);
+                dai += rp * sqrtf(rsi);
+            }
+            const float drs = -0.5f * dai * ai / rsi;
+            dw = dw * ai * aj + drs;
+            if (lane == 0) sk.rowinfo[i] = make_float4(ai, drs, sk.k[i], 0.0f);
+        } else if (lane == 0) {
+            sk.rowinfo[i] = make_float4(1.0f, 0.0f, sk.k[i], 0.0f);
+        }
+        const float th = c_tanh((float)lane - sk.k[i]);
+        const float f = 1.0f - 0.5f * (1.0f + th);
+        const float dfdk = 0.5f * (1.0f - th * th);
+        gl = (live && sk.mode == 0) ? dw * f : 0.0f;
+        float skp = live ? (sk.mode == 0 ? dw * vl * dfdk : dw * dfdk) : 0.0f;
+#pragma unroll
+        for (int off = 32; off >= 1; off >>= 1) skp += __shfl_xor(skp, off, 64);
+        if (lane == 0) sk.dk[i] = skp;
+        if (sk.dval_out && lane < K) sk.dval_out[i * K + lane] = gl;
+    }
+    const float4 xi = *reinterpret_cast<const float4 *>(xp + gi * H + 4 * c4);
+    float4 acc = make_float4(0.0f, 0.0f, 0.0f, 0.0f);
+    constexpr int NBT = (32 / NPI) < 1 ? 1 : 32 / NPI;
+    const bool myact = lane < K && jl >= 0 && gl != 0.0f;
+    for (int r0 = 0; r0 < K; r0 += NBT * NPI) {
+        const bool mine = lane >= r0 && lane < r0 + NBT * NPI;
+        const unsigned long long actm = __ballot(mine && myact);
+        if (actm == 0ull) continue;
+        const int nbl = sk.live ? (63 - __clzll((long long)actm) - r0) / NPI + 1 : NBT;
+        edge_rows_group<H>(xp, gi, r0, K, mine, jl, myact, gl, vl, xi, t, perturb, lane, nbl, acc);
+    }
+#pragma unroll
+    for (int off = LPR; off < 64; off <<= 1) {
+        acc.x += __shfl_xor(acc.x, off, 64); acc.y += __shfl_xor(acc.y, off, 64);
+        acc.z += __shfl_xor(acc.z, off, 64); acc.w += __shfl_xor(acc.w, off, 64);
+    }
+    if (slot == 0) *reinterpret_cast<float4 *>(dxp + gi * H + 4 * c4) = acc;
 }
 
 template <int H>
@@ -707,11 +843,68 @@
 }
 
 template <int H>
+__device__ __forceinline__ void edge_walk_group(const float *__restrict__ xp, int64_t j, const int4 myrec, const float mydval, const float4 xj,
+                                                int64_t row0, float t, int perturb, int lane, int nbl, float4 &acc, const int wide) {
+    constexpr int LPR = H / 4, NPI = 64 / LPR, NBT = (32 / NPI) < 1 ? 1 : 32 / NPI;
+    constexpr int Q = NBT >= 2 ? NBT / 2 : NBT;
+    const int c4 = lane % LPR, slot = lane / LPR;
+    const bool run1 = nbl > Q;
+    float4 xi[NBT];
+    float myd2 = 0.0f, mydd = 0.0f;
+    auto gather = [&](auto B0, auto B1) {
+#pragma unroll
+        for (int b = B0; b < B1; b++) {
+            const int q = b * NPI + slot;
+            const int src = __shfl(myrec.x, q, 64);
+            const int dst = __shfl(myrec.y, q, 64);
+            xi[b] = *reinterpret_cast<const float4 *>(xp + (dst >= 0 ? row0 + (wide ? dst : (src >> 6)) : j) * H + 4 * c4);
+        }
+    };
+    auto dist2 = [&](auto B0, auto B1) {
+#pragma unroll
+        for (int b = B0; b < B1; b++) {
+            const float4 d = make_float4(xi[b].x - xj.x, xi[b].y - xj.y, xi[b].z - xj.z, xi[b].w - xj.w);
+            float d2 = d.x * d.x + d.y * d.y + d.z * d.z + d.w * d.w;
+            if (LPR > 16) d2 += __uint_as_float(xor_shfl<16>(__float_as_uint(d2), lane));
+            if (LPR > 8) d2 += __uint_as_float(xor_shfl<8>(__float_as_uint(d2), lane));
+            if (LPR > 4) d2 += __uint_as_float(xor_shfl<4>(__float_as_uint(d2), lane));
+            d2 += __uint_as_float(xor_shfl<2>(__float_as_uint(d2), lane));
+            d2 += __uint_as_float(xor_shfl<1>(__float_as_uint(d2), lane));
+            const float tq = __shfl(d2, (lane % NPI) * LPR, 64);
+            if (lane / NPI == b) myd2 = tq;
+        }
+    };
+    auto accum = [&](auto B0, auto B1) {
+#pragma unroll
+        for (int b = B0; b < B1; b++) {
+            const float dd = __shfl(mydd, b * NPI + slot, 64);
+            const float4 d = make_float4(xi[b].x - xj.x, xi[b].y - xj.y, xi[b].z - xj.z, xi[b].w - xj.w);
+            acc.x -= dd * d.x; acc.y -= dd * d.y; acc.z -= dd * d.z; acc.w -= dd * d.w;
+        }
+    };
+    using std::integral_constant;
+    constexpr integral_constant<int, 0> c0{};
+    constexpr integral_constant<int, Q> c1{};
+    constexpr integral_constant<int, NBT> c2{};
+    if (run1) gather(c1, c2);
+    gather(c0, c1);
+    if (run1) dist2(c1, c2);
+    dist2(c0, c1);
+    if (mydval != 0.0f && myd2 != 0.0f) {
+        const float dist = sqrtf(myd2);
+        const float p = c_exp(t * dist);
+        const float dp = perturb ? mydval * __int_as_float(myrec.w) / (p + 1e-8f) : mydval;
+        mydd = dp * t * p / dist;
+    }
+    accum(c0, c1);
+    if (run1) accum(c1, c2);
+}
+
+template <int H>
 __device__ __forceinline__ void edge_bwd_walk(const float *__restrict__ xp, int64_t j, int pb, int pe, int p1, const int4 *__restrict__ recs,
                                               const float *__restrict__ dA_rec, const float4 *__restrict__ rowinfo, const float4 xj, const float aj,
-                                              int64_t row0, float t, int perturb, int lane, float4 &acc, const int wide = 0) {
+                                              int64_t row0, float t, int perturb, int lane, float4 &acc, const int wide = 0, const int live = 0) {
     constexpr int LPR = H / 4, NPI = 64 / LPR, NBT = (32 / NPI) < 1 ? 1 : 32 / NPI, PER = NBT * NPI;
-    const int c4 = lane % LPR, slot = lane / LPR;
     for (int e0 = pb; e0 < pe; e0 += PER) {
         const bool have = lane < PER && e0 + lane < pe;
         const int ec = have ? e0 + lane : p1 - 1;
@@ -724,40 +917,9 @@
             const float th = c_tanh((float)(myrec.x & 63) - info.z);
             mydval = have ? dw * (1.0f - 0.5f * (1.0f + th)) : 0.0f;
         }
-        float4 xi[NBT];
-#pragma unroll
-        for (int b = 0; b < NBT; b++) {
-            const int q = b * NPI + slot;
-            const int src = __shfl(myrec.x, q, 64);
-            const int dst = __shfl(myrec.y, q, 64);
-            xi[b] = *reinterpret_cast<const float4 *>(xp + (dst >= 0 ? row0 + (wide ? dst : (src >> 6)) : j) * H + 4 * c4);
-        }
-        float myd2 = 0.0f;
-#pragma unroll
-        for (int b = 0; b < NBT; b++) {
-            const float4 d = make_float4(xi[b].x - xj.x, xi[b].y - xj.y, xi[b].z - xj.z, xi[b].w - xj.w);
-            float d2 = d.x * d.x + d.y * d.y + d.z * d.z + d.w * d.w;
-            if (LPR > 16) d2 += __uint_as_float(xor_shfl<16>(__float_as_uint(d2), lane));
-            if (LPR > 8) d2 += __uint_as_float(xor_shfl<8>(__float_as_uint(d2), lane));
-            if (LPR > 4) d2 += __uint_as_float(xor_shfl<4>(__float_as_uint(d2), lane));
-            d2 += __uint_as_float(xor_shfl<2>(__float_as_uint(d2), lane));
-            d2 += __uint_as_float(xor_shfl<1>(__float_as_uint(d2), lane));
-            const float tq = __shfl(d2, (lane % NPI) * LPR, 64);
-            if (lane / NPI == b) myd2 = tq;
-        }
-        float mydd = 0.0f;
-        if (mydval != 0.0f && myd2 != 0.0f) {
-            const float dist = sqrtf(myd2);
-            const float p = c_exp(t * dist);
-            const float dp = perturb ? mydval * __int_as_float(myrec.w) / (p + 1e-8f) : mydval;
-            mydd = dp * t * p / dist;
-        }
-#pragma unroll
-        for (int b = 0; b < NBT; b++) {
-            const float dd = __shfl(mydd, b * NPI + slot, 64);
-            const float4 d = make_float4(xi[b].x - xj.x, xi[b].y - xj.y, xi[b].z - xj.z, xi[b].w - xj.w);
-            acc.x -= dd * d.x; acc.y -= dd * d.y; acc.z -= dd * d.z; acc.w -= dd * d.w;
-        }
+        const int left = __builtin_amdgcn_readfirstlane(pe - e0);
+        const int nbl = live && left < PER ? (left + NPI - 1) / NPI : NBT;
+        edge_walk_group<H>(xp, j, myrec, mydval, xj, row0, t, perturb, lane, nbl, acc, wide);
     }
 #pragma unroll
     for (int off = LPR; off < 64; off <<= 1) {
@@ -767,11 +929,11 @@
 }
 
 template <int H>
-__global__ __launch_bounds__(256) void edge_bwd_node(const float *__restrict__ xp, int64_t ncols, const int *__restrict__ nodeptr,
+__global__ __launch_bounds__(256) __attribute__((amdgpu_waves_per_eu(H == 64 ? 6 : (H == 128 ? 3 : 8)))) void edge_bwd_node(const float *__restrict__ xp, int64_t ncols, const int *__restrict__ nodeptr,
                                                      const int4 *__restrict__ recs, const float *__restrict__ dA_rec,
                                                      const float4 *__restrict__ rowinfo, const float *__restrict__ rs, int normalized,
                                                      int64_t row0, int64_t rows, float t, int perturb, float *__restrict__ dxp, int out_act,
-                                                     unsigned nmain = 0, int wide = 0) {
+                                                     unsigned nmain = 0, int wide = 0, int live = 0) {
     constexpr int LPR = H / 4, NPI = 64 / LPR, NBT = (32 / NPI) < 1 ? 1 : 32 / NPI, PER = NBT * NPI;
     __shared__ float4 part[4][LPR];
     const int lane = threadIdx.x & 63, c4 = lane % LPR, slot = lane / LPR, wave = dgg::wave_id();
@@ -785,11 +947,11 @@
     const float aj = normalized ? __fdiv_rn(1.0f, c_sqrt(rs[j])) : 1.0f;
     float4 acc = make_float4(0.0f, 0.0f, 0.0f, 0.0f);
     if (!longmode) {
-        edge_bwd_walk<H>(xp, j, p0, p1, p1, recs, dA_rec, rowinfo, xj, aj, row0, t, perturb, lane, acc, wide);
+        edge_bwd_walk<H>(xp, j, p0, p1, p1, recs, dA_rec, rowinfo, xj, aj, row0, t, perturb, lane, acc, wide, live);
     } else {
         const int chunk = ((p1 - p0 + 4 * PER - 1) / (4 * PER)) * PER;
         const int pb = p0 + wave * chunk, pe = pb + chunk < p1 ? pb + chunk : p1;
-        edge_bwd_walk<H>(xp, j, pb < p1 ? pb : p1, pe, p1, recs, dA_rec, rowinfo, xj, aj, row0, t, perturb, lane, acc, wide);
+        edge_bwd_walk<H>(xp, j, pb < p1 ? pb : p1, pe, p1, recs, dA_rec, rowinfo, xj, aj, row0, t, perturb, lane, acc, wide, live);
         if (slot == 0) part[wave][c4] = acc;
         __syncthreads();
         if (wave != 0) return;
@@ -1030,6 +1192,7 @@
     int *bstart, *totals, *nodeptr, *T;
     int *recpos;
     float *ainv;
+    int *ainv_ok;
     int4 *tmp, *recs;
     int width;
     uint32_t rcp;
@@ -1053,7 +1216,8 @@
     p.ainv = reinterpret_cast<float *>(w + o); o += align256((size_t)ncols * 4);
     p.tmp = reinterpret_cast<int4 *>(w + o); o += align256((size_t)rows * K * sizeof(int4));
     p.recs = reinterpret_cast<int4 *>(w + o); o += align256((size_t)rows * K * sizeof(int4));
-    p.recpos = reinterpret_cast<int *>(w + o); o += (size_t)rows * 64 * sizeof(int);
+    p.recpos = reinterpret_cast<int *>(w + o); o += align256((size_t)rows * 64 * sizeof(int));
+    p.ainv_ok = reinterpret_cast<int *>(w + o); o += 256;
     return o;
 }
 
@@ -1074,11 +1238,12 @@
 template <int THREADS>
 __global__ __launch_bounds__(THREADS) void pp_count(const int32_t *__restrict__ idx, const float *__restrict__ w, int64_t rows, int K, int nb,
                                                     uint32_t rcp, int *__restrict__ T, const float *__restrict__ rs_all, int64_t ncols,
-                                                    float *__restrict__ ainv) {
+                                                    float *__restrict__ ainv, int *__restrict__ ainv_ok) {
     extern __shared__ int lds[];
     int *hist = lds;
     const int tid = threadIdx.x, lane = tid & 63, wave = dgg::wave_id();
     for (int b = tid; b < nb; b += THREADS) hist[b] = 0;
+    if (blockIdx.x == 0 && tid == 0) *ainv_ok = rs_all ? 1 : 0;
     if (rs_all) {
         const int64_t per = (ncols + gridDim.x - 1) / gridDim.x;
         const int64_t j1 = ((int64_t)blockIdx.x + 1) * per < ncols ? ((int64_t)blockIdx.x + 1) * per : ncols;
@@ -1518,7 +1683,7 @@
     }
 #define DGG_PP_PASS(TT)                                                                                                      \
     hipLaunchKernelGGL(pp_count<TT>, dim3((unsigned)nwg), dim3(TT), (size_t)nb * 4, st, idx, w, rows, K, nb, p.rcp, p.T, rs_all, ncols, \
-                       p.ainv);                                                                                              \
+                       p.ainv, p.ainv_ok);                                                                                   \
     hipLaunchKernelGGL(pp_scan, dim3((unsigned)((nb + 31) / 32)), dim3(1024), 0, st, p.T, nwg, nb, p.totals);                \
     hipLaunchKernelGGL(pp_fill<TT>, dim3((unsigned)nwg), dim3(TT), (size_t)(2 * nb + 16) * 4, st, idx, w, val, rs_rows, rows, K, nb, p.rcp, \
                        p.T, p.totals, p.bstart, p.tmp, p.ainv, ahat)
@@ -1639,16 +1804,16 @@
     hipStream_t st = (hipStream_t)stream;
     PartP2 p;
     partp2_layout(p, const_cast<void *>(partp_ws), rows, K, ncols);
+    const int live = edge_live();
     const SoftkArgs sk{k, rs, dA, da, mode, normalized, nullptr, dk, ahat_rows, reinterpret_cast<float4 *>(rowinfo_ws),
-                       dA ? nullptr : p.recpos, dA_rec};
+                       dA ? nullptr : p.recpos, dA_rec, edge_ainv() ? p.ainv : nullptr, p.ainv_ok, live};
     const unsigned gr = (unsigned)((rows + 3) / 4);
     const bool grouped = node_groups(rows * K, ncols);
     const unsigned nmain = (unsigned)((ncols + 3) / 4);
     const bool split = node_split(ncols);
 #define DGG_EDGE_PARTP(HH)                                                                                                  \
     if (phase != 2)                                                                                                          \
-        hipLaunchKernelGGL((edge_bwd_rows<HH, true, true>), dim3(gr), dim3(256), 0, st, xp, rows, idx, val, nullptr, K, row0, t, perturb, nullptr, \
-                           nullptr, dxp, sk);                                                                                \
+        hipLaunchKernelGGL(edge_bwd_rows_pay<HH>, dim3(gr), dim3(256), 0, st, xp, rows, idx, val, K, row0, t, perturb, dxp, sk);               \
     if (phase == 1) {                                                                                                        \
     } else if (mode == 0 && grouped)                                                                                         \
         hipLaunchKernelGGL((edge_bwd_nodeg<HH, 4>), dim3((unsigned)((ncols + 4 * (256 / HH) - 1) / (4 * (256 / HH)))), dim3(256), 0, st, xp, \
@@ -1657,7 +1822,7 @@
     else if (mode == 0)                                                                                                      \
         hipLaunchKernelGGL(edge_bwd_node<HH>, dim3(split ? nmain + (unsigned)ncols : nmain), dim3(256), 0, st, xp, ncols, p.nodeptr, p.recs, \
                            dA_rec, reinterpret_cast<const float4 *>(rowinfo_ws), rs, normalized, row0, rows, t, perturb, dxp, out_act,  \
-                           split ? nmain : 0u)
+                           split ? nmain : 0u, 0, live)
     switch (h) {
         case 16: DGG_EDGE_PARTP(16); break;
         case 32: DGG_EDGE_PARTP(32); break;
@@ -1686,7 +1851,7 @@
     if (phase != 2) {
 #define DGG_PP_PASS(TT)                                                                                                      \
     hipLaunchKernelGGL(pp_count<TT>, dim3((unsigned)nwg), dim3(TT), (size_t)nb * 4, st, idx, w, chunks, K, nb, p.rcp, p.T, rs_all, ncols, \
-                       p.ainv);                                                                                              \
+                       p.ainv, p.ainv_ok);                                                                                   \
     hipLaunchKernelGGL(pp_scan, dim3((unsigned)((nb + 31) / 32)), dim3(1024), 0, st, p.T, nwg, nb, p.totals);                \
     hipLaunchKernelGGL(pp_fill<TT>, dim3((unsigned)nwg), dim3(TT), (size_t)(2 * nb + 16) * 4, st, idx, w, val, rs_nodes, chunks, K, nb, p.rcp, \
                        p.T, p.totals, p.bstart, p.tmp, p.ainv, ahat, cnode)
@@ -1750,6 +1915,7 @@
     hipStream_t st = (hipStream_t)stream;
     PartP2 p;
     partp2_layout(p, const_cast<void *>(partp_ws), chunks, K, ncols);
+    const int live = edge_live();
     const SoftkArgs sk{k, rs, dA, da, mode, normalized, nullptr, dk, ahat_rows, reinterpret_cast<float4 *>(rowinfo_ws), nullptr, dA_rec};
     const unsigned gr = (unsigned)((rows + 3) / 4);
     const unsigned nmain = (unsigned)((ncols + 3) / 4);
@@ -1760,7 +1926,7 @@
     if (phase != 1 && mode == 0)                                                                                             \
         hipLaunchKernelGGL(edge_bwd_node<HH>, dim3(split ? nmain + (unsigned)ncols : nmain), dim3(256), 0, st, xp, ncols, p.nodeptr, p.recs, \
                            dA_rec, reinterpret_cast<const float4 *>(rowinfo_ws), rs, normalized, row0, rows, t, perturb, dxp, out_act,  \
-                           split ? nmain : 0u, 1)
+                           split ? nmain : 0u, 1, live)
     switch (h) {
         case 16: DGG_EDGE_PARTC(16); break;
         case 32: DGG_EDGE_PARTC(32); break;
diff --git a/learning-adaptive-neighborhoods-for-gnns_amd/ops.py b/learning-adaptive-neighborhoods-for-gnns_amd/ops.py
--- a/learning-adaptive-neighborhoods-for-gnns_amd/ops.py
+++ b/learning-adaptive-neighborhoods-for-gnns_amd/ops.py
@@ -149,16 +149,28 @@
         return res + linear_fwd_multi(x, grp)
     if len(layers) > 8 or any(o % 32 for o in outs) or sum(outs) > 256 or sum(outs) == 224:
         return [linear_fwd(x, W, b, act, lay) for W, b, act, lay in layers]
+    Ws = [_chk(W) for W, *_ in layers]
+    bs = [None if b is None else _chk(b) for _, b, _, _ in layers]
+    lays = [lay for *_, lay in layers]
+    L = _lib.lib()
+    if L.dgg_linear_fwd_multi_unpacked_ok(_ptr(x), N, d, len(layers), _ptr_array(Ws), _int_array(outs), _int_array(lays)) == 1:
+        ys = [torch.empty((N, o), device=x.device, dtype=torch.float32) for o in outs]
+        _lib.check(L.dgg_linear_fwd_multi_unpacked(_ptr(x), N, d, len(layers), _ptr_array(Ws), _ptr_array(bs), _int_array(outs),
+                                                   _int_array(lays), _int_array([a for _, _, a, _ in layers]), _ptr_array(ys), _stream()),
+                   "linear_fwd_multi_unpacked")
+        return ys
     Wcat = torch.empty((sum(outs), d), device=x.device, dtype=torch.float32)
     bcat = torch.empty((sum(outs),), device=x.device, dtype=torch.float32)
-    _lib.check(_lib.lib().dgg_linear_pack_weights(len(layers), _ptr_array([_chk(W) for W, *_ in layers]),
-                                                  _ptr_array([None if b is None else _chk(b) for _, b, _, _ in layers]), _int_array(outs),
-                                                  _int_array([lay for *_, lay in layers]), d, _ptr(Wcat), _ptr(bcat), _stream()),
-               "linear_pack_weights")
+    _lib.check(L.dgg_linear_pack_weights(len(layers), _ptr_array(Ws), _ptr_array(bs), _int_array(outs), _int_array(lays), d, _ptr(Wcat),
+                                         _ptr(bcat), _stream()), "linear_pack_weights")
     ys = [torch.empty((N, o), device=x.device, dtype=torch.float32) for o in outs]
     _lib.check(_lib.lib().dgg_linear_fwd_multi(_ptr(x), N, d, _ptr(Wcat), _ptr(bcat), len(layers), _int_array(outs),
                                                _int_array([a for _, _, a, _ in layers]), _ptr_array(ys), _stream()), "linear_fwd_multi")
     return ys
+
+
+def tn_store():
+    return os.environ.get("DGG_TN_STORE", "1") != "0"
 
 
 def linear_bwd_multi(x, layers):
@@ -182,7 +194,9 @@
             res.append((dW, db))
         return res
     nW = [int(W.numel()) for W, *_ in layers]
-    zz = _zeros((sum(nW) + sum(o for o, l_ in zip(outs, layers) if l_[5]),), x.device)
+    store = tn_store()
+    nz = sum(nW) + sum(o for o, l_ in zip(outs, layers) if l_[5])
+    zz = torch.empty((nz,), device=x.device, dtype=torch.float32) if store else _zeros((nz,), x.device)
     dWs, dbs, o_ = [], [], 0
     for (W, *_), n_ in zip(layers, nW):
         dWs.append(zz[o_:o_ + n_].view(W.shape))
@@ -193,9 +207,9 @@
     ws = torch.empty((int(_lib.lib().dgg_gemm_tn_multi_ws_floats(N, sum(outs), d)),), device=x.device, dtype=torch.float32)
     dys = [_chk(l_[2]) for l_ in layers]
     ysv = [(_chk(l_[1]) if (l_[1] is not None and l_[3] != ACT_NONE) else None) for l_ in layers]
-    _lib.check(_lib.lib().dgg_gemm_tn_multi(len(layers), _ptr_array(dys), _int_array(outs), _ptr_array(ysv),
-                                            _int_array([l_[3] for l_ in layers]), _ptr(x), N, d, _ptr_array(dWs),
-                                            _int_array([0 if l_[4] == 0 else 1 for l_ in layers]), _ptr_array(dbs), _ptr(ws), _stream()),
+    fn = _lib.lib().dgg_gemm_tn_multi_store if store else _lib.lib().dgg_gemm_tn_multi
+    _lib.check(fn(len(layers), _ptr_array(dys), _int_array(outs), _ptr_array(ysv), _int_array([l_[3] for l_ in layers]), _ptr(x), N, d,
+                  _ptr_array(dWs), _int_array([0 if l_[4] == 0 else 1 for l_ in layers]), _ptr_array(dbs), _ptr(ws), _stream()),
                "gemm_tn_multi")
     return list(zip(dWs, dbs))
 
diff --git a/learning-adaptive-neighborhoods-for-gnns_amd/parallel.py b/learning-adaptive-neighborhoods-for-gnns_amd/parallel.py
--- a/learning-adaptive-neighborhoods-for-gnns_amd/parallel.py
+++ b/learning-adaptive-neighborhoods-for-gnns_amd/parallel.py
@@ -342,6 +342,9 @@
                 need += rows * self.K + ncols * (h + F + 2)
             if self.scorer is not None:
                 need += rows * self.K + ncols * (2 * self.scorer["Wcat"].shape[0] + h) + 4 * int(self.scorer["Wcat"].numel()) + 4096
+            if s.get("partp") is not None and self.scorer is None and self.mode == 0 and s["z"] is None and not self.x_grad and \
+                    hasattr(kern, "linear_bwd_multi") and getattr(kern, "tn_store", lambda: False)():
+                return self._backward(dZ, x_local, P, dA_ext)
             with kern.zero_pool(s["xp"].device, need):
                 return self._backward(dZ, x_local, P, dA_ext)
         return self._backward(dZ, x_local, P, dA_ext)
```

Result: no change. 2.672 billion edges/s (median of 6 runs) (+0.8%).
